# NOAA-OWP/T-Route

Hardware: AMD Instinct MI355X
Metric: segment-timesteps/sec, CONUS NHD 2.7M-seg MC (higher is better)
Workload: dtype f32

## Files before the change

include/trmc.h:

```cpp
#ifndef TRMC_H
#define TRMC_H

#include <stddef.h>
#include <stdint.h>

#ifdef __cplusplus
extern "C" {
#endif

#define TRMC_ABI_VERSION 19

typedef enum trmc_status {
    TRMC_OK = 0,
    TRMC_EINVAL = -1,
    TRMC_ECYCLE = -2,
    TRMC_ENODEVICE = -3,
    TRMC_EHIP = -4,
    TRMC_ENOMEM = -5,
    TRMC_ESTATE = -6,
    TRMC_EUNSUPPORTED = -7
} trmc_status;

enum { TRMC_P_DT = 0, TRMC_P_DX, TRMC_P_BW, TRMC_P_TW, TRMC_P_TWCC, TRMC_P_N,
       TRMC_P_NCC, TRMC_P_CS, TRMC_P_S0, TRMC_NPARAM };

typedef struct trmc_plan trmc_plan;

typedef struct trmc_stats {
    int64_t nseg;
    int64_t nseg_routed;
    int32_t nlevels;
    int32_t nsteps;
    int32_t assume_short_ts;
    int32_t main_launches;
    int64_t segment_steps;
    double ms_prep;
    double ms_main;
    double ms_emit;
    double ms_total;
    int32_t wide_levels, wide_k;
    int32_t wide_launches;
    int32_t mid_levels;
    int64_t wide_segment_steps;
    double ms_wide;
    int32_t mid_k, mid_launches;
    int32_t arithmetic;
    int32_t reserved0;
} trmc_stats;

const char *trmc_last_error(void);
int trmc_abi_version(void);
int trmc_device_count(int *count);

int trmc_plan_create(int64_t nseg, const int64_t *up_ptr, const int64_t *up_idx,
                     const float *params, const uint8_t *boundary, int precision,
                     int device, trmc_plan **out);
int trmc_plan_create_hinted(int64_t nseg, const int64_t *up_ptr, const int64_t *up_idx,
                            const float *params, const uint8_t *boundary, const uint8_t *cost_hint,
                            int precision, int device, trmc_plan **out);
enum { TRMC_ENGINE_AUTO = 0, TRMC_ENGINE_LEVELS = 1, TRMC_ENGINE_FLOW = 2, TRMC_ENGINE_MASK = 3,
       TRMC_PLAN_SHORT_TS = 4, TRMC_PLAN_FULL_TS = 8 };
int trmc_plan_create_ex(int64_t nseg, const int64_t *up_ptr, const int64_t *up_idx,
                        const float *params, const uint8_t *boundary, const uint8_t *cost_hint,
                        int precision, int device, int flags, trmc_plan **out);
enum { TRMC_ARITH_EXACT = 0, TRMC_ARITH_TOLERANCE = 1 };
typedef struct trmc_plan_options {
    int32_t struct_size;
    int32_t arithmetic;
    int64_t wide_min_rows;
    int32_t wide_levels, wide_k;
    int64_t mid_min_rows;
    int32_t mid_levels, mid_k;
    int32_t tile_perm_group;
    int32_t tail_sort;
    int32_t stem_min_rows;
    int32_t sequence_mode;
    int32_t flow_watchdog_ms;
    int32_t flow_overlap;
    int32_t flow_lean;
    int32_t flow_debug;
    int32_t hot_rows;
    int32_t cluster_rows;
    int32_t cluster_late_lag;
    int32_t stream_split;
    int32_t hot_wave_rows;
    int32_t velocity_on_demand;
    int32_t reserved[2];
} trmc_plan_options;
int trmc_plan_create_opt(int64_t nseg, const int64_t *up_ptr, const int64_t *up_idx,
                         const float *params, const uint8_t *boundary, const uint8_t *cost_hint,
                         int precision, int device, int flags, const trmc_plan_options *options, trmc_plan **out);
int trmc_stream_begin(trmc_plan *plan, int nsteps, int qts_subdivisions, int slots, int full_output, int output_stride);
int trmc_stream_push(trmc_plan *plan, const void *qlat, int64_t nq, const void *boundary_q_dev, int32_t rowset, void *hyd_host,
                     void *q0_host, void *fvd_host);
typedef struct trmc_stream_day {
    const void *qlat;
    int64_t nq;
    const void *boundary_q_dev;
    int32_t rowset;
    int32_t reserved0;
    void *hyd_host, *q0_host, *fvd_host;
    int64_t da_ngage;
    int32_t da_nsteps, res_nsteps;
    const uint8_t *da_mode;
    const void *da_a, *da_w;
    void *nudge_host;
    int64_t res_nres;
    void *res_inflow_host;
    const void *da_q0;
    const struct trmc_stream_reservoir_da *reservoir_da;
    void *res_da_state_host, *res_da_tsidx_host;
} trmc_stream_day;
int trmc_stream_set_gages(trmc_plan *plan, int64_t ngage, const int64_t *gage_rows);
int trmc_stream_push_day(trmc_plan *plan, const trmc_stream_day *day);
int trmc_stream_set_packed_forcing(trmc_plan *plan, int64_t nfeat, const int64_t *feat_of_row, const double *pack_a, const double *pack_b);
int trmc_stream_push_day_packed(trmc_plan *plan, const trmc_stream_day *day, const int32_t *raw_a, const int32_t *raw_b);
int trmc_stream_packed_forcing_kernel_ms(trmc_plan *plan, double *ms_out);
enum { TRMC_SUMMARY_PEAK = 1, TRMC_SUMMARY_MEAN = 2, TRMC_SUMMARY_PEAK_DEPTH = 4, TRMC_SUMMARY_TOTAL = 8 };
int trmc_stream_set_summary(trmc_plan *plan, int what);
int trmc_stream_summary_dest(trmc_plan *plan, void *peak_flow_host, int32_t *peak_step_host, void *mean_flow_host);
int trmc_stream_summary_depth_dest(trmc_plan *plan, void *peak_depth_host, int32_t *peak_depth_step_host);
int trmc_stream_summary_total(trmc_plan *plan, void *peak_flow, int64_t *peak_step, void *mean_flow, void *peak_depth,
                              int64_t *peak_depth_step, int64_t *days_out);
int trmc_stream_gather(trmc_plan *plan, int64_t day, int32_t rowset, void *dst_dev, void *stream);
int trmc_stream_boundary(trmc_plan *plan, int64_t day, const void *q_dev, int64_t src_row_stride, const int64_t *index_dev, void *stream);
int trmc_stream_advance(trmc_plan *plan, int ntiles);
int trmc_stream_flush(trmc_plan *plan);
int trmc_stream_wait(trmc_plan *plan, int64_t day);
int trmc_stream_info(const trmc_plan *plan, int32_t *slots, int32_t *tiles_per_day, int32_t *lag_max, int32_t *wide_levels,
                     int32_t *cluster_levels, int64_t *days_pushed, int64_t *days_complete, int64_t *launches);
int trmc_stream_day_ms(trmc_plan *plan, int64_t day, double *ms_out);
int trmc_stream_end(trmc_plan *plan);

int trmc_plan_set_sequence_mode(trmc_plan *plan, int on);
int trmc_plan_arithmetic(const trmc_plan *plan, int32_t *arithmetic);
int trmc_plan_engine(const trmc_plan *plan, int32_t *is_flow);
void trmc_plan_destroy(trmc_plan *plan);

int trmc_topology_levels(int64_t nseg, const int64_t *up_ptr, const int64_t *up_idx,
                         const uint8_t *boundary, int32_t *level_of_row,
                         int64_t *plan_pos_of_row, int32_t *nlevels);

int trmc_topology_levels_hinted(int64_t nseg, const int64_t *up_ptr, const int64_t *up_idx,
                                const uint8_t *boundary, const uint8_t *cost_hint, int32_t *level_of_row,
                                int64_t *plan_pos_of_row, int32_t *nlevels);

int trmc_topology_clusters(int64_t nseg, const int64_t *up_ptr, const int64_t *up_idx, const uint8_t *boundary,
                           const uint8_t *cost_hint, int64_t wide_min_rows, int32_t wide_max_levels, int32_t cluster_rows,
                           int64_t *plan_pos_of_row, int32_t *lag_of_row, int32_t *block_of_row, int32_t *wide_levels,
                           int32_t *cluster_levels, int32_t *cluster_blocks);

int trmc_topology_blocks(int64_t nseg, const int64_t *up_ptr, const int64_t *up_idx,
                         const uint8_t *boundary, const uint8_t *cost_hint, int cost_tiers,
                         int64_t *plan_pos_of_row, int32_t *rank_of_row, int32_t *block_rows, int32_t *nblocks);

int trmc_topology_blocks_general(int64_t nseg, const int64_t *up_ptr, const int64_t *up_idx, const uint8_t *boundary,
                                 int32_t stem_min_rows, int64_t *plan_pos_of_row, int32_t *rank_of_row, int32_t *block_rows,
                                 int32_t *nblocks, int32_t *early_blocks, int32_t early_cap, int32_t *nearly);

int trmc_plan_info(const trmc_plan *plan, int64_t *nseg, int64_t *nseg_routed,
                   int32_t *nlevels, int32_t *precision, int32_t *device);
int trmc_plan_lags(const trmc_plan *plan, int32_t *lag_of_row, int32_t *wide_levels, int32_t *cluster_levels);
int trmc_plan_cluster_blocks(const trmc_plan *plan, int32_t *block_of_row, int32_t *block_width, int32_t *cluster_blocks);
int trmc_plan_levels(const trmc_plan *plan, int32_t *level_of_row, int64_t *plan_pos_of_row);

int trmc_upload_forcing(trmc_plan *plan, int nsteps, const void *qlat, int64_t nq,
                        const void *q0, const void *boundary_fvd);

int trmc_upload_forcing_packed(trmc_plan *plan, int nsteps, int64_t nq, int64_t nfeat, const int32_t *raw_a,
                               const int32_t *raw_b, const double *pack_a, const double *pack_b,
                               const int64_t *feat_of_row, const void *q0, const void *boundary_fvd);

int trmc_set_boundary_flow_device(trmc_plan *plan, int nsteps, const void *q_dev);

int trmc_set_reservoirs(trmc_plan *plan, int64_t nres, const int64_t *res_rows, const void *par,
                        double routing_period);
int trmc_download_reservoir_inflow(trmc_plan *plan, void *inflow_out);

typedef struct trmc_reservoir_da_table {
    int64_t n, ncol;
    const float *obs, *time, *state;
    const int32_t *ipar;
} trmc_reservoir_da_table;
int trmc_set_reservoir_da(trmc_plan *plan, int64_t nres, const int32_t *kind, const int32_t *table_row,
                          const trmc_reservoir_da_table *usgs, const trmc_reservoir_da_table *usace,
                          const trmc_reservoir_da_table *rfc);
int trmc_download_reservoir_da(trmc_plan *plan, float *state_out, int32_t *timeseries_idx_out);
typedef struct trmc_stream_reservoir_da {
    trmc_reservoir_da_table usgs, usace, rfc;
    int32_t rfc_reset_idx;
    int32_t reserved0;
} trmc_stream_reservoir_da;
int trmc_stream_set_reservoir_da(trmc_plan *plan, int on, int64_t usgs_ncol, int64_t usace_ncol, int64_t rfc_ncol);
#define TRMC_RESERVOIR_DA_HYBRID 2
#define TRMC_RESERVOIR_DA_RFC 4
int trmc_reservoir_da_steps(int device, int kind, int64_t n, int64_t ncol, const float *obs, const float *time,
                            const float *fin, const int32_t *iin, float *fout, int32_t *iout);

int trmc_set_nudging(trmc_plan *plan, int nsteps, int64_t ngage, const int64_t *gage_rows,
                     const uint8_t *mode, const void *a, const void *w);
int trmc_set_nudging_successors(trmc_plan *plan, int64_t ngage, const int64_t *successor_rows);
int trmc_download_nudge(trmc_plan *plan, void *nudge_out);

int trmc_route_device(trmc_plan *plan, int nsteps, int qts_subdivisions, int assume_short_ts);

int trmc_route_begin(trmc_plan *plan, int nsteps, int qts_subdivisions, int assume_short_ts);
int trmc_route_advance(trmc_plan *plan, int t_end);
int trmc_route_end(trmc_plan *plan);
int trmc_plan_stream(trmc_plan *plan, void **stream_out);
int trmc_rowset_create(trmc_plan *plan, const int64_t *rows, int64_t nrows, int32_t *id_out);
int trmc_gather_flow_range(trmc_plan *plan, int32_t rowset, int t_begin, int t_end, void *dst_dev,
                           int64_t dst_stride);
int trmc_set_boundary_flow_range(trmc_plan *plan, int t_begin, int t_end, const void *q_dev, int64_t src_stride,
                                 void *stream );
int trmc_set_boundary_flow_range_indexed(trmc_plan *plan, int t_begin, int t_end, const void *q_dev,
// ... 115 lines not shown
```

t-route_amd/_lib.py:

```python
import ctypes as C
import os

import numpy as np

_HERE = os.path.dirname(os.path.abspath(__file__))
LIB_PATH = os.environ.get("TRMC_LIB_PATH") or os.path.join(_HERE, "libtrmc.so")

TRMC_OK, TRMC_EINVAL, TRMC_ECYCLE, TRMC_ENODEVICE, TRMC_EHIP, TRMC_ENOMEM, TRMC_ESTATE = 0, -1, -2, -3, -4, -5, -6
TRMC_EUNSUPPORTED = -7
ENGINE_AUTO, ENGINE_LEVELS, ENGINE_FLOW, PLAN_SHORT_TS, PLAN_FULL_TS = 0, 1, 2, 4, 8
NPARAM = 9
PARAM_COLS = ("dt", "dx", "bw", "tw", "twcc", "n", "ncc", "cs", "s0")


class Stats(C.Structure):
    _fields_ = [
        ("nseg", C.c_int64), ("nseg_routed", C.c_int64), ("nlevels", C.c_int32), ("nsteps", C.c_int32),
        ("assume_short_ts", C.c_int32), ("main_launches", C.c_int32), ("segment_steps", C.c_int64),
        ("ms_prep", C.c_double), ("ms_main", C.c_double), ("ms_emit", C.c_double), ("ms_total", C.c_double),
        ("wide_levels", C.c_int32), ("wide_k", C.c_int32), ("wide_launches", C.c_int32), ("mid_levels", C.c_int32),
        ("wide_segment_steps", C.c_int64), ("ms_wide", C.c_double), ("mid_k", C.c_int32), ("mid_launches", C.c_int32),
        ("arithmetic", C.c_int32), ("reserved0", C.c_int32),
    ]

    def as_dict(self):
        return {k: getattr(self, k) for k, _ in self._fields_}


class PlanOptions(C.Structure):
    _fields_ = [
        ("struct_size", C.c_int32), ("arithmetic", C.c_int32), ("wide_min_rows", C.c_int64), ("wide_levels", C.c_int32),
        ("wide_k", C.c_int32), ("mid_min_rows", C.c_int64), ("mid_levels", C.c_int32), ("mid_k", C.c_int32),
        ("tile_perm_group", C.c_int32), ("tail_sort", C.c_int32), ("stem_min_rows", C.c_int32), ("sequence_mode", C.c_int32),
        ("flow_watchdog_ms", C.c_int32), ("flow_overlap", C.c_int32), ("flow_lean", C.c_int32), ("flow_debug", C.c_int32), ("hot_rows", C.c_int32),
        ("cluster_rows", C.c_int32), ("cluster_late_lag", C.c_int32), ("stream_split", C.c_int32), ("hot_wave_rows", C.c_int32), ("velocity_on_demand", C.c_int32), ("reserved", C.c_int32 * 2),
    ]


ARITH_EXACT, ARITH_TOLERANCE = 0, 1
OPTION_ENV = {
    "TRMC_WIDE_MIN_ROWS": ("wide_min_rows", "off0"), "TRMC_WIDE_LEVELS": ("wide_levels", "int"), "TRMC_WIDE_K": ("wide_k", "int"),
    "TRMC_MID_MIN_ROWS": ("mid_min_rows", "off0"), "TRMC_MID_LEVELS": ("mid_levels", "int"), "TRMC_MID_K": ("mid_k", "int"),
    "TRMC_TILE_PERM": ("tile_perm_group", "off0"), "TRMC_HOT_ROWS": ("hot_rows", "off0"), "TRMC_CLUSTER_ROWS": ("cluster_rows", "int"), "TRMC_STREAM_SPLIT": ("stream_split", "int"), "TRMC_HOT_WAVE_ROWS": ("hot_wave_rows", "int"), "TRMC_VELOCITY_ON_DEMAND": ("velocity_on_demand", "int"), "TRMC_TAIL_SORT": ("tail_sort", "off0"),
    "TRMC_STEM_MIN_ROWS": ("stem_min_rows", "off0"), "TRMC_SETUP_ASIDE": ("sequence_mode", "flag"),
    "TRMC_FLOW_WATCHDOG_MS": ("flow_watchdog_ms", "int"), "TRMC_FLOW_OVERLAP": ("flow_overlap", "flag"),
    "TRMC_FLOW_LEAN": ("flow_lean", "lean"), "TRMC_FLOW_DEBUG": ("flow_debug", "flag"),
}


def plan_options(options=None):
    o = PlanOptions()
    o.struct_size = C.sizeof(PlanOptions)
    for name, (field, how) in OPTION_ENV.items():
        v = os.environ.get(name)
        if v is None or v == "":
            continue
        n = int(v)
        if how == "off0":
            n = -1 if n == 0 else n
        elif how == "flag":
            n = 1 if n == 1 else 0
        elif how == "lean":
            n = 1 if n == 1 else -1
        setattr(o, field, n)
    a = os.environ.get("TRMC_ARITHMETIC")
    if a:
        o.arithmetic = {"exact": ARITH_EXACT, "tolerance": ARITH_TOLERANCE}[a]
    for k, v in (options or {}).items():
        if k == "arithmetic" and isinstance(v, str):
            v = {"exact": ARITH_EXACT, "tolerance": ARITH_TOLERANCE}[v]
        if not hasattr(o, k) or k in ("struct_size", "reserved"):
            raise ValueError(f"unknown plan option {k!r}")
        setattr(o, k, int(v))
    return o


_vp, _i64, _i32, _int = C.c_void_p, C.c_int64, C.c_int32, C.c_int


class ReservoirDaTable(C.Structure):
    _fields_ = [("n", C.c_int64), ("ncol", C.c_int64), ("obs", C.c_void_p), ("time", C.c_void_p), ("state", C.c_void_p),
                ("ipar", C.c_void_p)]


class StreamReservoirDa(C.Structure):
    _fields_ = [("usgs", ReservoirDaTable), ("usace", ReservoirDaTable), ("rfc", ReservoirDaTable), ("rfc_reset_idx", C.c_int32),
                ("reserved0", C.c_int32)]


RESERVOIR_DA_HYBRID, RESERVOIR_DA_RFC = 2, 4
SUMMARY_PEAK, SUMMARY_MEAN = 1, 2
SUMMARY_PEAK_DEPTH, SUMMARY_TOTAL = 4, 8
SUMMARY_NAMES = {"peak": SUMMARY_PEAK, "mean": SUMMARY_MEAN, "peak_depth": SUMMARY_PEAK_DEPTH, "total": SUMMARY_TOTAL}
TRMC_X_FLOW, TRMC_X_VELOCITY, TRMC_X_DEPTH = 0, 1, 2
X_NAMES = {"flow": TRMC_X_FLOW, "velocity": TRMC_X_VELOCITY, "depth": TRMC_X_DEPTH}
_P = C.POINTER
SIGNATURES = {
    "trmc_last_error": (C.c_char_p, []),
    "trmc_abi_version": (_int, []),
    "trmc_device_count": (_int, [_P(_int)]),
    "trmc_plan_create": (_int, [_i64, _vp, _vp, _vp, _vp, _int, _int, _P(_vp)]),
    "trmc_plan_create_hinted": (_int, [_i64, _vp, _vp, _vp, _vp, _vp, _int, _int, _P(_vp)]),
    "trmc_plan_create_ex": (_int, [_i64, _vp, _vp, _vp, _vp, _vp, _int, _int, _int, _P(_vp)]),
    "trmc_plan_create_opt": (_int, [_i64, _vp, _vp, _vp, _vp, _vp, _int, _int, _int, _P(PlanOptions), _P(_vp)]),
    "trmc_plan_set_sequence_mode": (_int, [_vp, _int]),
    "trmc_stream_begin": (_int, [_vp, _int, _int, _int, _int, _int]),
    "trmc_stream_push": (_int, [_vp, _vp, _i64, _vp, _i32, _vp, _vp, _vp]),
    "trmc_stream_set_gages": (_int, [_vp, _i64, _vp]),
    "trmc_stream_push_day": (_int, [_vp, _vp]),
    "trmc_stream_set_reservoir_da": (_int, [_vp, _int, _i64, _i64, _i64]),
    "trmc_stream_set_summary": (_int, [_vp, _int]),
    "trmc_stream_summary_dest": (_int, [_vp, _vp, _vp, _vp]),
    "trmc_stream_summary_depth_dest": (_int, [_vp, _vp, _vp]),
    "trmc_stream_summary_total": (_int, [_vp, _vp, _vp, _vp, _vp, _vp, _vp]),
    "trmc_stream_gather": (_int, [_vp, _i64, _i32, _vp, _vp]),
    "trmc_stream_boundary": (_int, [_vp, _i64, _vp, _i64, _vp, _vp]),
    "trmc_stream_advance": (_int, [_vp, _int]),
    "trmc_stream_flush": (_int, [_vp]),
    "trmc_stream_wait": (_int, [_vp, _i64]),
    "trmc_stream_info": (_int, [_vp, _P(_i32), _P(_i32), _P(_i32), _P(_i32), _P(_i32), _P(_i64), _P(_i64), _P(_i64)]),
    "trmc_stream_day_ms": (_int, [_vp, _i64, _P(C.c_double)]),
    "trmc_stream_end": (_int, [_vp]),
    "trmc_plan_arithmetic": (_int, [_vp, _P(_i32)]),
    "trmc_plan_engine": (_int, [_vp, _P(_i32)]),
    "trmc_plan_destroy": (None, [_vp]),
    "trmc_topology_levels": (_int, [_i64, _vp, _vp, _vp, _vp, _vp, _P(_i32)]),
    "trmc_topology_levels_hinted": (_int, [_i64, _vp, _vp, _vp, _vp, _vp, _vp, _P(_i32)]),
    "trmc_topology_clusters": (_int, [_i64, _vp, _vp, _vp, _vp, _i64, _i32, _i32, _vp, _vp, _vp, _P(_i32), _P(_i32), _P(_i32)]),
    "trmc_topology_blocks": (_int, [_i64, _vp, _vp, _vp, _vp, _int, _vp, _vp, _P(_i32), _P(_i32)]),
    "trmc_topology_blocks_general": (_int, [_i64, _vp, _vp, _vp, _i32, _vp, _vp, _P(_i32), _P(_i32), _vp, _i32, _P(_i32)]),
    "trmc_plan_info": (_int, [_vp, _P(_i64), _P(_i64), _P(_i32), _P(_i32), _P(_i32)]),
    "trmc_plan_levels": (_int, [_vp, _vp, _vp]),
    "trmc_plan_lags": (_int, [_vp, _vp, _P(_i32), _P(_i32)]),
    "trmc_plan_cluster_blocks": (_int, [_vp, _vp, _P(_i32), _P(_i32)]),
    "trmc_upload_forcing": (_int, [_vp, _int, _vp, _i64, _vp, _vp]),
    "trmc_upload_forcing_packed": (_int, [_vp, _int, _i64, _i64, _vp, _vp, _vp, _vp, _vp, _vp, _vp]),
    "trmc_set_boundary_flow_device": (_int, [_vp, _int, _vp]),
    "trmc_set_reservoirs": (_int, [_vp, _i64, _vp, _vp, C.c_double]),
    "trmc_download_reservoir_inflow": (_int, [_vp, _vp]),
    "trmc_set_reservoir_da": (_int, [_vp, _i64, _vp, _vp, _P(ReservoirDaTable), _P(ReservoirDaTable), _P(ReservoirDaTable)]),
    "trmc_download_reservoir_da": (_int, [_vp, _vp, _vp]),
    "trmc_reservoir_da_steps": (_int, [_int, _int, _i64, _i64, _vp, _vp, _vp, _vp, _vp, _vp]),
    "trmc_set_nudging": (_int, [_vp, _int, _i64, _vp, _vp, _vp, _vp]),
    "trmc_set_nudging_successors": (_int, [_vp, C.c_int64, _vp]),
    "trmc_download_nudge": (_int, [_vp, _vp]),
    "trmc_route_device": (_int, [_vp, _int, _int, _int]),
    "trmc_route_begin": (_int, [_vp, _int, _int, _int]),
    "trmc_route_advance": (_int, [_vp, _int]),
    "trmc_route_end": (_int, [_vp]),
    "trmc_plan_stream": (_int, [_vp, _P(_vp)]),
    "trmc_rowset_create": (_int, [_vp, _vp, _i64, _P(_i32)]),
    "trmc_gather_flow_range": (_int, [_vp, _i32, _int, _int, _vp, _i64]),
    "trmc_set_boundary_flow_range": (_int, [_vp, _int, _int, _vp, _i64, _vp]),
    "trmc_set_boundary_flow_range_indexed": (_int, [_vp, _int, _int, _vp, _i64, _vp, _vp]),
    "trmc_plan_set_lag": (_int, [_vp, _vp]),
    "trmc_download_fvd": (_int, [_vp, _vp]),
    "trmc_download_fvd_strided": (_int, [_vp, _int, _vp]),
    "trmc_download_fvd_rowset": (_int, [_vp, _int, C.c_int32, _vp]),
    "trmc_window_summary": (_int, [_vp, _i32, _vp, _vp, _vp, _vp, _vp, _vp, _vp]),
    "trmc_window_summary_tile": (_int, [_int, _P(_i32), _P(_i32)]),
    "trmc_window_summary_kernel_ms": (_int, [_vp, _P(C.c_double)]),
    "trmc_window_courant": (_int, [_vp, _i32, _int, _vp]),
    "trmc_window_courant_summary": (_int, [_vp, _i32, C.c_double, _vp, _vp, _vp]),
    "trmc_window_courant_tile": (_int, [_int, _P(_i32), _P(_i32)]),
    "trmc_window_courant_kernel_ms": (_int, [_vp, _P(C.c_double)]),
    "trmc_plan_set_thresholds": (_int, [_vp, _i32, _vp]),
    "trmc_window_exceedance": (_int, [_vp, _i32, _int, _vp, _vp, _vp, _vp]),
    "trmc_window_exceedance_tile": (_int, [_int, _P(_i32), _P(_i32)]),
    "trmc_window_exceedance_kernel_ms": (_int, [_vp, _P(C.c_double)]),
    "trmc_plan_bankfull_depth": (_int, [_vp, _vp]),
    "trmc_stream_set_exceedance": (_int, [_vp, _int]),
    "trmc_stream_exceedance": (_int, [_vp, _vp, _vp, _vp, _vp, _P(_i64)]),
    "trmc_stream_set_courant": (_int, [_vp, _int, C.c_double]),
    "trmc_stream_courant": (_int, [_vp, _vp, _vp, _vp, _P(_i64)]),
    "trmc_stream_courant_kernel_ms": (_int, [_vp, _P(C.c_double)]),
    "trmc_stream_set_depth_exceedance": (_int, [_vp, _i32, _vp]),
    "trmc_stream_depth_exceedance": (_int, [_vp, _vp, _vp, _vp, _vp, _P(_i64)]),
    "trmc_stream_depth_exceedance_kernel_ms": (_int, [_vp, _P(C.c_double)]),
    "trmc_stream_set_stage": (_int, [_vp, _int]),
    "trmc_stream_stage_dest": (_int, [_vp, _vp]),
    "trmc_stream_set_packed_forcing": (_int, [_vp, _i64, _vp, _vp, _vp]),
    "trmc_stream_push_day_packed": (_int, [_vp, _vp, _vp, _vp]),
    "trmc_stream_packed_forcing_kernel_ms": (_int, [_vp, _P(C.c_double)]),
    "trmc_plan_set_nan_is_zero": (_int, [_vp, _int]),
    "trmc_host_alloc": (_int, [C.c_size_t, C.POINTER(C.c_void_p)]),
    "trmc_host_free": (_int, [_vp]),
    "trmc_download_final_state": (_int, [_vp, _vp]),
    "trmc_download_iterations": (_int, [_vp, _vp]),
    "trmc_plan_collect_cost": (_int, [_vp, _int]),
    "trmc_download_cost": (_int, [_vp, _vp, _P(_i32)]),
    "trmc_gather_flow_rows": (_int, [_vp, _vp, _i64, _vp, _int]),
    "trmc_download_gathered": (_int, [_vp, _vp]),
    "trmc_plan_set_stamps": (_int, [_vp, _vp, _i32]),
    "trmc_plan_set_output_stride": (_int, [_vp, _i32]),
    "trmc_plan_hot_rows": (_int, [_vp, _P(_i64)]),
    "trmc_plan_hot_state": (_int, [_vp, _P(_i32), _P(_i32), _P(_i32), _P(_i32), _P(_i32), _P(_i32)]),
    "trmc_fetch_begin": (_int, [_vp, _i32, _vp, _vp]),
    "trmc_fetch_begin_fvd": (_int, [_vp, _i32, _vp, _vp, _int, _vp]),
    "trmc_fetch_wait": (_int, [_vp]),
    "trmc_get_stats": (_int, [_vp, _P(Stats)]),
    "trmc_route": (_int, [_vp, _int, _int, _int, _vp, _i64, _vp, _vp, _vp]),
    "trmc_segments": (_int, [_int, _int, _i64, _vp, _vp]),
    "trmc_segments_ex": (_int, [_int, _int, _int, _i64, _vp, _vp, _vp]),
    "trmc_muskingcungenwm": (None, [_P(C.c_float)] * 21),
    "trmc_plan_chain_from": (_int, [_vp, _vp]),
# ... 244 lines not shown
```

t-route_amd/csrc/abi.inc:

```

static bool stream_active(const trmc_plan *pl);

const char *trmc_last_error(void) { return g_err.c_str(); }
int trmc_abi_version(void) { return TRMC_ABI_VERSION; }

int trmc_device_count(int *count)
{
    if (!count) return fail(TRMC_EINVAL, "count is NULL");
    int c = 0;
    hipError_t e = hipGetDeviceCount(&c);
    if (e != hipSuccess) {
        *count = 0;
        return fail(TRMC_ENODEVICE, std::string("hipGetDeviceCount: ") + hipGetErrorString(e));
    }
    *count = c;
    return 0;
}

int trmc_topology_levels(int64_t nseg, const int64_t *up_ptr, const int64_t *up_idx, const uint8_t *boundary,
                         int32_t *level_of_row, int64_t *plan_pos_of_row, int32_t *nlevels)
{
    return trmc_topology_levels_hinted(nseg, up_ptr, up_idx, boundary, nullptr, level_of_row, plan_pos_of_row, nlevels);
}

// ... 168 lines not shown

int trmc_plan_create_ex(int64_t nseg, const int64_t *up_ptr, const int64_t *up_idx, const float *params,
                        const uint8_t *boundary, const uint8_t *cost_hint, int precision, int device, int flags,
                        trmc_plan **out)
{
    return trmc_plan_create_opt(nseg, up_ptr, up_idx, params, boundary, cost_hint, precision, device, flags, nullptr, out);
}

static int plan_streams(trmc_plan *pl)
{
    HIP_TRY(hipSetDevice(pl->device));
    int prio_lo = 0, prio_hi = 0;
    HIP_TRY(hipDeviceGetStreamPriorityRange(&prio_lo, &prio_hi));
    if (int rc = pl->stream.ensure(hipStreamNonBlocking, prio_hi)) return rc;
    if (int rc = pl->stream2.ensure(hipStreamNonBlocking, prio_lo)) return rc;
    if (int rc = pl->ev_emit.ensure(false)) return rc;
    if (pl->flow) {
        if (int rc = pl->fstream.ensure(hipStreamNonBlocking, prio_hi)) return rc;
        for (DevEvent &e : pl->ev_chunk)
            if (int rc = e.ensure(false)) return rc;
        if (int rc = pl->ev_ctl.ensure(false)) return rc;
    }
    for (DevEvent &e : pl->ev)
        if (int rc = e.ensure(true)) return rc;
    return 0;
}

int trmc_plan_create_opt(int64_t nseg, const int64_t *up_ptr, const int64_t *up_idx, const float *params,
                         const uint8_t *boundary, const uint8_t *cost_hint, int precision, int device, int flags,
                         const trmc_plan_options *options, trmc_plan **out)
{
    if (!out) return fail(TRMC_EINVAL, "out is NULL");
    trmc_plan_options o{};
    if (options) {
        if (options->struct_size < 8 || options->struct_size > (int32_t)sizeof(trmc_plan_options))
            return fail(TRMC_EINVAL, "trmc_plan_options.struct_size is not the size of a trmc_plan_options this library knows");
        std::memcpy(&o, options, (size_t)options->struct_size);
    }
    if (o.arithmetic != TRMC_ARITH_EXACT && o.arithmetic != TRMC_ARITH_TOLERANCE) return fail(TRMC_EINVAL, "bad trmc_plan_options.arithmetic");
    if (o.arithmetic == TRMC_ARITH_TOLERANCE && precision != 32)
        return fail(TRMC_EINVAL, "TRMC_ARITH_TOLERANCE is an arithmetic of precision-32 plans");
    *out = nullptr;
    if (precision != 32 && precision != 64) return fail(TRMC_EINVAL, "precision must be 32 or 64");
    if (nseg > 0 && !params) return fail(TRMC_EINVAL, "params is NULL");
    if ((flags & ~(TRMC_ENGINE_MASK | TRMC_PLAN_SHORT_TS | TRMC_PLAN_FULL_TS)) || (flags & TRMC_ENGINE_MASK) == 3
        || ((flags & TRMC_PLAN_SHORT_TS) && (flags & TRMC_PLAN_FULL_TS)))
        return fail(TRMC_EINVAL, "bad plan flags");
    int engine = flags & TRMC_ENGINE_MASK;
    if (engine == TRMC_ENGINE_FLOW && precision != 32) return fail(TRMC_EINVAL, "the dataflow engine runs precision-32 plans only");
    if (int rc = check_device(device)) return rc;

    trmc_plan *pl = new (std::nothrow) trmc_plan();
    if (!pl) return fail(TRMC_ENOMEM, "out of host memory");
    pl->sh = std::make_shared<PlanShared>();
    if (engine == TRMC_ENGINE_AUTO) {
        if (precision != 32)
            engine = TRMC_ENGINE_LEVELS;
        else {
            int64_t nb = 0;
            for (int64_t r = 0; boundary && r < nseg; ++r) nb += boundary[r] == 1;
            engine = ((flags & TRMC_PLAN_SHORT_TS) && nseg - nb >= 1000000) ? TRMC_ENGINE_LEVELS : TRMC_ENGINE_FLOW;
        }
    }
    pl->flow = engine == TRMC_ENGINE_FLOW;
    pl->watchdog_ticks = (uint64_t)(o.flow_watchdog_ms > 0 ? o.flow_watchdog_ms : 30000) * 100000ull;
    {
        int ncu = 256;
        if (hipSetDevice(device) == hipSuccess) (void)hipDeviceGetAttribute(&ncu, hipDeviceAttributeMultiprocessorCount, device);
        trmc_plan::Opt &po = pl->opt;
        po.tol = o.arithmetic == TRMC_ARITH_TOLERANCE;
        po.wide_min_rows = o.wide_min_rows < 0 ? 0 : (o.wide_min_rows > 0 ? o.wide_min_rows : (po.tol ? 256L : 288L) * ncu);
        po.wide_levels = (int32_t)std::min<long>(o.wide_levels > 0 ? o.wide_levels : 16, kWideMaxLevels);
        po.wide_k = o.wide_k > 0 ? o.wide_k : 0;
        po.mid_min_rows = o.mid_min_rows < 0 ? 0 : (o.mid_min_rows > 0 ? o.mid_min_rows : kMidDefaultRowsPerCu * (int64_t)ncu);
        po.mid_levels = (int32_t)std::min<long>(o.mid_levels > 0 ? o.mid_levels : 12, kMidMaxLevels);
        po.mid_k = o.mid_k > 0 ? o.mid_k : 4;
        po.tile_perm_group = o.tile_perm_group < 0 ? 0 : (o.tile_perm_group > 0 ? 1 : -1);
        po.hot_rows = o.hot_rows < 0 ? 0 : (o.hot_rows > 0 ? 1 : -1);
        po.cluster_rows = o.cluster_rows > 0 ? std::min<int32_t>(o.cluster_rows, kClusterRowsMax) : 0;
        po.cluster_late_lag = std::max(0, o.cluster_late_lag);
        po.stream_split = std::max(0, o.stream_split);
        po.hot_wave_rows = std::max(0, std::min(64, o.hot_wave_rows));
        po.velocity_on_demand = o.velocity_on_demand;
        po.sequence = o.sequence_mode != 0;
        po.flow_overlap = o.flow_overlap != 0;
        po.flow_lean = o.flow_lean;
        po.flow_debug = o.flow_debug != 0;
    }
    const bool tiers = (flags & TRMC_PLAN_SHORT_TS) != 0;
    std::string err;
    int64_t wide_min_rows = 0, mid_min_rows = 0;
    int32_t wide_max_levels = 0, mid_max_levels = 0;
    if (tiers && !pl->flow && cost_hint && o.tail_sort >= 0) {
        wide_min_rows = pl->opt.wide_min_rows;
        wide_max_levels = pl->opt.wide_levels;
        mid_min_rows = pl->opt.mid_min_rows;
        mid_max_levels = pl->opt.mid_levels;
    }
    int32_t cluster_rows = 0;
    if (tiers && !pl->flow && pl->opt.cluster_rows > 0) {
        cluster_rows = pl->opt.cluster_rows;
        wide_min_rows = pl->opt.wide_min_rows;
        wide_max_levels = pl->opt.wide_levels;
        mid_min_rows = 0;
        mid_max_levels = 0;
        pl->opt.mid_min_rows = 0;
    }
    int32_t stem_min_rows = 0;
    if (pl->flow && (flags & TRMC_PLAN_FULL_TS)) stem_min_rows = o.stem_min_rows < 0 ? 0 : (o.stem_min_rows > 0 ? o.stem_min_rows : 1024);
    const int trc = trmc::build_topology(nseg, up_ptr, up_idx, boundary, pl->sh->topo, err, cost_hint, pl->flow ? kFlowBlock : 0, tiers,
                                         (tiers && !pl->flow) ? kWideMaxLevels : 0, wide_min_rows, wide_max_levels, stem_min_rows,
                                         mid_min_rows, mid_max_levels, cluster_rows, pl->opt.cluster_late_lag, kCtileBlock);
    if (trc) {
        delete pl;
        return fail(trc == -2 ? TRMC_ECYCLE : TRMC_EINVAL, err);
    }
    pl->device = device;
    pl->hinted = cost_hint != nullptr && (!pl->flow || tiers);
    pl->precision = precision;
    pl->esz = precision == 32 ? 4 : 8;
    pl->nseg = nseg;
    pl->nseg_pad = (nseg + 63) / 64 * 64;
    if (pl->nseg_pad == 0) pl->nseg_pad = 64;
    pl->nrouted = nseg - pl->sh->topo.nboundary;
    pl->dt_uniform = true;
    pl->dt = nseg ? params[TRMC_P_DT] : 0.0;
    for (int64_t r = 1; r < nseg; ++r)
        if (params[(size_t)r * TRMC_NPARAM + TRMC_P_DT] != params[TRMC_P_DT]) {
            pl->dt_uniform = false;
            break;
        }

    auto bail = [&](int rc) {
        trmc_plan_destroy(pl);
        return rc;
    };
    int rc = plan_streams(pl);
    if (rc) return bail(rc);
    rc = by_precision(pl, [&](auto t) { return upload_params<decltype(t)>(pl, params); });
    if (rc) return bail(rc);
    std::vector<int32_t> level_plan((size_t)pl->nseg_pad, 0);
    for (int64_t p = 0; p < nseg; ++p) level_plan[p] = pl->sh->topo.level_of_row[pl->sh->topo.row_of_pos[p]];
    if ((rc = upload_i32(pl->sh->level, level_plan, 1))) return bail(rc);
    if (pl->sh->topo.ncl > 0) {
        std::vector<int32_t> lagk(pl->sh->topo.lagk_of_pos);
        lagk.resize((size_t)pl->nseg_pad, 0);
        if ((rc = upload_i32(pl->sh->lagk, lagk, 1))) return bail(rc);
        if ((rc = upload_i32(pl->sh->cblk_ptr, pl->sh->topo.cblk_ptr, 1))) return bail(rc);
    }
    if ((rc = upload_i32(pl->sh->up_ptr, pl->sh->topo.up_ptr, 1))) return bail(rc);
    if ((rc = upload_i32(pl->sh->up_idx, pl->sh->topo.up_idx, 1))) return bail(rc);
    {
        if (nseg >= (int64_t)1 << 30) return bail(fail(TRMC_EINVAL, "more than 2**30 segments in one plan"));
        if ((uint64_t)pl->nseg_pad * pl->esz >= (1ull << 32))
            return bail(fail(TRMC_EINVAL, "too many segments for one plan at this precision (column size reaches 4 GiB)"));
        std::vector<int32_t> up2((size_t)pl->nseg_pad * 2, -1);
        for (int64_t p = 0; p < nseg; ++p) {
            const int32_t k0 = pl->sh->topo.up_ptr[p], k1 = pl->sh->topo.up_ptr[p + 1];
            if (k1 - k0 >= 1) up2[2 * p] = pl->sh->topo.up_idx[k0];
            if (k1 - k0 >= 2) up2[2 * p + 1] = pl->sh->topo.up_idx[k0 + 1] | (k1 - k0 > 2 ? 0x40000000 : 0);
        }
        if ((rc = upload_i32(pl->sh->up2, up2, 2))) return bail(rc);
    }
    if (pl->flow && (rc = upload_i32(pl->sh->rank, pl->sh->topo.rank_of_pos, 1))) return bail(rc);
    if (pl->flow) {
        if ((rc = pl->sh->prio.ensure(pl->sh->topo.prio_of_wave.size() + 1))) return bail(rc);
// ... 27 lines not shown
    *out = pl;
    return 0;
}

void trmc_plan_destroy(trmc_plan *pl)
{
    if (!pl) return;
    (void)hipSetDevice(pl->device);
    delete pl;
}

static int final_state_into(trmc_plan *pl, void *dst, int32_t nsteps_of_window = -1);
static int ensure_copy_stream(trmc_plan *pl);

int trmc_plan_clone(trmc_plan *src, trmc_plan **out)
{
    if (!out) return fail(TRMC_EINVAL, "out is NULL");
    *out = nullptr;
    if (!src) return fail(TRMC_EINVAL, "plan is NULL");
    if (int rc = use_device(src)) return rc;
    trmc_plan *pl = new (std::nothrow) trmc_plan();
    if (!pl) return fail(TRMC_ENOMEM, "out of host memory");
    pl->device = src->device;
    pl->precision = src->precision;
    pl->esz = src->esz;
    pl->nseg = src->nseg;
    pl->nseg_pad = src->nseg_pad;
    pl->nrouted = src->nrouted;
    pl->dt_uniform = src->dt_uniform;
    pl->dt = src->dt;
    pl->hinted = src->hinted;
    pl->params_sane = src->params_sane;
    pl->flow = src->flow;
    pl->watchdog_ticks = src->watchdog_ticks;
    pl->opt = src->opt;
    pl->ncuq = src->ncuq;
    pl->sh = src->sh;
    pl->is_clone = true;
    auto bail = [&](int rc) {
        trmc_plan_destroy(pl);
        return rc;
    };
    if (int rc = plan_streams(pl)) return bail(rc);
    if (src->maxlag > 0) {
        pl->lag_of_row = src->lag_of_row;
        pl->maxlag = src->maxlag;
    }
    if (int rc = pl->it_prev.ensure((size_t)pl->nseg_pad)) return bail(rc);
    if (pl->ncuq > 0)
        if (int rc = pl->cuq_head.ensure((size_t)pl->ncuq * 2 * sizeof(int32_t))) return bail(rc);
    *out = pl;
    return 0;
}

int trmc_stage_forcing(trmc_plan *pl, int nsteps, const void *qlat, int64_t nq)
{
    if (!pl) return fail(TRMC_EINVAL, "plan is NULL");
    const bool busy = pl->run.active;
    if (busy && pl->run.t_done < pl->run.nsteps + (pl->run.short_ts ? pl->maxlag : 0))
        return fail(TRMC_ESTATE, "the window in progress has not been queued to its end (trmc_route_advance)");
    if (busy && (pl->ngage > 0 || pl->nres > 0))
        return fail(TRMC_ESTATE, "a window with nudging tables or reservoirs is in progress: its series are read after trmc_route_end; "
                                 "stage the next forcing then");
    if (nsteps < 1) return fail(TRMC_EINVAL, "nsteps must be >= 1");
    if (nq < 1) return fail(TRMC_EINVAL, "qlat needs at least one column");
    if (pl->nseg > 0 && !qlat) return fail(TRMC_EINVAL, "qlat is NULL");
    if (int rc = use_device(pl)) return rc;
    if (int rc = ensure_copy_stream(pl)) return rc;
    const size_t bytes = (size_t)pl->nseg * nq * pl->esz;
    if (busy && bytes > pl->in_qlat.bytes)
        return fail(TRMC_ESTATE, "the staging area would have to grow while the window in progress may still read it");
    if (int rc = pl->in_qlat.ensure(bytes)) return rc;
    if (int rc = pl->in_q0.ensure((size_t)pl->nseg * 3 * pl->esz)) return rc;
    pl->state_missing = busy || (pl->routed_nsteps < 0 && !pl->q0_staged);
    if (pl->nseg > 0 && !pl->state_missing && pl->routed_nsteps >= 0)
        if (int rc = final_state_into(pl, pl->in_q0.p)) return rc;
    pl->q0_staged = !pl->state_missing;
    if (busy) HIP_TRY(hipStreamWaitEvent(pl->hstream, pl->ev[1], 0));
    if (pl->nseg > 0) HIP_TRY(hipMemcpyAsync(pl->in_qlat.p, qlat, bytes, hipMemcpyHostToDevice, pl->hstream));
    pl->qlat_alt_ready = false;
    if (pl->opt.sequence && !pl->flow && pl->nseg > 0) {
        if (int rc = pl->qlat_alt.ensure((size_t)nq * pl->nseg_pad * pl->esz)) return rc;
        const int32_t n = (int32_t)pl->nseg;
        const dim3 grid((n + 63) / 64, (unsigned)((nq + 31) / 32));
        const int rc = by_precision(pl, [&](auto t) {
            using T = decltype(t);
            hipLaunchKernelGGL((k_prep_qlat<T>), grid, dim3(kBlock), 0, pl->hstream, (const T *)pl->in_qlat.p,
                               (const int32_t *)pl->sh->row_of_pos.p, (T *)pl->qlat_alt.p, n, pl->nseg_pad, (int32_t)nq);
            return launched();
        });
        if (rc) return rc;
        pl->qlat_alt_ready = true;
    }
    if (int rc = pl->mk_forcing.record(pl->hstream)) return rc;
    pl->qlat_direct = false;
    pl->nq = nq;
    pl->have_boundary = pl->sh->topo.nboundary == 0;
    pl->ngage = 0;
    pl->nraw = 0;
    pl->staged_nsteps = nsteps;
    if (!busy) pl->routed_nsteps = -1;
    return 0;
}

int trmc_plan_info(const trmc_plan *pl, int64_t *nseg, int64_t *nseg_routed, int32_t *nlevels, int32_t *precision,
                   int32_t *device)
{
    if (!pl) return fail(TRMC_EINVAL, "plan is NULL");
    if (nseg) *nseg = pl->nseg;
    if (nseg_routed) *nseg_routed = pl->nrouted;
    if (nlevels) *nlevels = pl->sh->topo.nlevels;
    if (precision) *precision = pl->precision;
    if (device) *device = pl->device;
    return 0;
}

int trmc_plan_lags(const trmc_plan *pl, int32_t *lag_of_row, int32_t *wide_levels, int32_t *cluster_levels)
{
    if (!pl) return fail(TRMC_EINVAL, "plan is NULL");
    const trmc::Topology &t = pl->sh->topo;
    if (t.cl_rows <= 0) return fail(TRMC_EINVAL, "the plan is not in cluster order (trmc_plan_options.cluster_rows)");
    for (int64_t r = 0; lag_of_row && r < pl->nseg; ++r)
        lag_of_row[r] = t.level_of_row[r] < 0 ? -1 : t.lagk_of_pos[(size_t)t.pos_of_row[r]];
    if (wide_levels) *wide_levels = t.cl_from_level;
    if (cluster_levels) *cluster_levels = t.ncl;
    return 0;
}

int trmc_plan_cluster_blocks(const trmc_plan *pl, int32_t *block_of_row, int32_t *block_width, int32_t *cluster_blocks)
{
    if (!pl) return fail(TRMC_EINVAL, "plan is NULL");
    const trmc::Topology &t = pl->sh->topo;
    if (t.cl_rows <= 0) return fail(TRMC_EINVAL, "the plan is not in cluster order (trmc_plan_options.cluster_rows)");
    const int32_t nb = t.ncl > 0 ? (int32_t)t.cblk_ptr.size() - 1 : 0;
    if (block_of_row) {
        for (int64_t r = 0; r < pl->nseg; ++r) block_of_row[r] = -1;
        for (int32_t b = 0; b < nb; ++b)
            for (int32_t p = t.cblk_ptr[(size_t)b]; p < t.cblk_ptr[(size_t)b + 1]; ++p) block_of_row[t.row_of_pos[(size_t)p]] = b;
    }
    if (block_width) *block_width = kCtileBlock;
    if (cluster_blocks) *cluster_blocks = nb;
    return 0;
}

int trmc_plan_levels(const trmc_plan *pl, int32_t *level_of_row, int64_t *plan_pos_of_row)
{
    if (!pl) return fail(TRMC_EINVAL, "plan is NULL");
    for (int64_t r = 0; r < pl->nseg; ++r) {
        if (level_of_row) level_of_row[r] = pl->sh->topo.level_of_row[r];
        if (plan_pos_of_row) plan_pos_of_row[r] = pl->sh->topo.pos_of_row[r];
    }
    return 0;
}

static int final_state_into(trmc_plan *pl, void *dst, int32_t nsteps_of_window)
{
    const int32_t n = (int32_t)pl->nseg, T_ = nsteps_of_window >= 0 ? nsteps_of_window : pl->routed_nsteps;
    const size_t plane = (size_t)(T_ + 1) * pl->nseg_pad;
    const int32_t *rop = (const int32_t *)pl->sh->row_of_pos.p;
    int rc;
    if (pl->flow) {
        hipLaunchKernelGGL((k_final_state<float>), dim3(blocks_for(n)), dim3(kBlock), 0, pl->stream, (const float *)pl->tm.p,
                           (const float *)pl->d_state.p, rop, (float *)dst, n, pl->nseg_pad, T_, 2, 0);
        rc = launched();
    } else {
        rc = by_precision(pl, [&](auto t) {
            using T = decltype(t);
            const T *q = (const T *)pl->tm.p;
            hipLaunchKernelGGL((k_final_state<T>), dim3(blocks_for(n)), dim3(kBlock), 0, pl->stream, q, q + 2 * plane, rop, (T *)dst, n,
                               pl->nseg_pad, T_, 1, T_);
            return launched();
// ... 1297 lines not shown
```

t-route_amd/csrc/host_flow.inc:

```
int flow_place_blocks(trmc_plan *pl)
{
    pl->ncuq = 0;
    const int32_t nb = pl->sh->topo.nblocks;
    if (nb <= 0) return 0;
    constexpr int kKeys = 4096;
    DevBuf seen;
    if (int rc = seen.ensure(kKeys)) return rc;
    HIP_TRY(hipMemset(seen.p, 0, kKeys));
    int ncu = 256;
    (void)hipDeviceGetAttribute(&ncu, hipDeviceAttributeMultiprocessorCount, pl->device);
    hipLaunchKernelGGL(k_cu_probe, dim3((unsigned)(64 * ncu)), dim3(64), 0, nullptr, (uint8_t *)seen.p);
    std::vector<uint8_t> hs(kKeys);
    hipError_t e = hipMemcpy(hs.data(), seen.p, kKeys, hipMemcpyDeviceToHost);
    seen.release();
    if (e != hipSuccess) return fail(TRMC_EHIP, std::string("compute-unit probe: ") + hipGetErrorString(e));
    std::vector<int32_t> cu_index(kKeys, -1);
    int32_t Q = 0;
    for (int k = 0; k < kKeys; ++k)
        if (hs[k]) cu_index[k] = Q++;
    if (Q < 2) return 0;
    const std::vector<uint8_t> &wc = pl->sh->topo.cost_of_wave;
    int hi = 0;
    for (const uint8_t c : wc) hi = std::max(hi, (int)c);
    const bool sixteenths = hi > 7;
// ... 83 lines not shown
    a.gran = (unsigned long long *)pl->tm.p;
    a.d_state = (float *)pl->d_state.p;
    a.d_gran = (unsigned long long *)pl->d_gran.p;
    a.out = (float *)pl->out.p;
    a.row_of_pos = (const int32_t *)pl->sh->row_of_pos.p;
    a.it_prev = (uint8_t *)pl->it_prev.p;
    a.it_sum = pl->collect_cost ? (uint16_t *)pl->it_sum.p : nullptr;
    a.sane = pl->params_sane;
    a.out_vec = nsteps % 4 == 0;
    a.res_of_pos = pl->nres > 0 ? (const int32_t *)pl->res_of_pos.p : nullptr;
    a.res_par = (const float *)pl->res_par.p;
    a.res_inflow = (float *)pl->res_inflow.p;
    a.res_dt = (float)pl->res_dt;
    a.res_da = (pl->nres > 0 && pl->res_da_on) ? pl->res_da.p : nullptr;
    const bool da = pl->ngage > 0;
    a.gage_of_pos = da ? (const int32_t *)pl->gage_of_pos.p : nullptr;
    a.da_mode = (const uint8_t *)pl->da_mode.p;
    a.da_a = (const float *)pl->da_a.p;
    a.da_w = (const float *)pl->da_w.p;
    a.da_nudge = (float *)pl->da_nudge.p;
    a.nseg_pad = pl->nseg_pad;
    a.nsteps = nsteps;
    a.qts = qts;
    a.nseg = (int32_t)pl->nseg;
    a.first = (int32_t)pl->sh->topo.nboundary;
    a.tag_base = pl->tag_base;
    a.ticket = (int32_t *)pl->ticket.p;
    a.watchdog_ticks = pl->watchdog_ticks;
    a.dbg = pl->opt.flow_debug ? (unsigned long long *)pl->dbg.p : nullptr;
    a.nblocks_dbg = pl->sh->topo.nblocks;
    a.prio = (const uint8_t *)pl->sh->prio.p;
    a.cuq_ptr = a.cuq_blk = a.cu_index = nullptr;
    a.cuq_perm = nullptr;
    a.cuq_head = nullptr;
    a.ncuq = 0;
    return a;
}

int flow_route_begin(trmc_plan *pl, int nsteps, int qts, int short_ts)
{
    const trmc::Topology &tp = pl->sh->topo;
    const int32_t n = (int32_t)pl->nseg;
    const int64_t np = pl->nseg_pad;
    hipStream_t st = pl->stream;
    if (int rc = pl->tm.ensure((size_t)(nsteps + 1) * np * sizeof(unsigned long long), true)) return rc;
    if (int rc = pl->d_state.ensure((size_t)np * sizeof(float))) return rc;
    if (int rc = pl->d_gran.ensure((size_t)np * sizeof(unsigned long long), true)) return rc;
    if (int rc = pl->ticket.ensure(16 * sizeof(int32_t))) return rc;
    if (pl->opt.flow_debug) {
        if (int rc = pl->dbg.ensure((size_t)(tp.nblocks + 1) * 6 * sizeof(unsigned long long))) return rc;
        HIP_TRY(hipMemsetAsync(pl->dbg.p, 0, pl->dbg.bytes, st));
    }
    if (int rc = pl->qlat_tm.ensure((size_t)pl->nq * np * sizeof(float))) return rc;
    if (int rc = pl->out.ensure((size_t)pl->nseg * nsteps * 3 * sizeof(float))) return rc;
    if (pl->nres > 0)
        if (int rc = pl->res_inflow.ensure((size_t)pl->nres * nsteps * sizeof(float))) return rc;
    if (pl->collect_cost) {
        if (int rc = pl->it_sum.ensure((size_t)np * sizeof(uint16_t))) return rc;
        pl->cost_nsteps = nsteps;
    }
    if ((uint64_t)pl->tag_base + (uint64_t)pl->tag_span + (uint64_t)nsteps + 2 >= 0xffffffffull) {
        HIP_TRY(hipMemsetAsync(pl->tm.p, 0, pl->tm.bytes, st));
        HIP_TRY(hipMemsetAsync(pl->d_gran.p, 0, pl->d_gran.bytes, st));
        pl->tag_base = 1;
        pl->tag_span = 0;
    }
    pl->tag_base += (uint32_t)pl->tag_span;
    pl->tag_span = nsteps + 1;
    const int32_t *row_of_pos = (const int32_t *)pl->sh->row_of_pos.p;
    HIP_TRY(hipEventRecord(pl->ev[0], st));
    pl->q0_staged = false;
    if (int rc = pl->mk_dec.order(st)) return rc;
    if (pl->fstream)
        if (int rc = pl->mk_dec.order(pl->fstream)) return rc;
    pl->mk_dec.settle();
    if (int rc = pl->mk_forcing.order(st)) return rc;
    pl->mk_forcing.settle();
    HIP_TRY(hipMemsetAsync(pl->it_prev.p, 0, (size_t)np, st));
    HIP_TRY(hipMemsetAsync(pl->ticket.p, 0, 16 * sizeof(int32_t), st));
    pl->flow_next = pl->flow_last = 0;
    if (pl->collect_cost) HIP_TRY(hipMemsetAsync(pl->it_sum.p, 0, (size_t)np * sizeof(uint16_t), st));
    if (n > 0) {
        if (!pl->qlat_direct)
            hipLaunchKernelGGL((k_prep_qlat<float>), dim3((n + 63) / 64, (unsigned)((pl->nq + 31) / 32)), dim3(kBlock), 0, st,
                               (const float *)pl->in_qlat.p, row_of_pos, (float *)pl->qlat_tm.p, n, np, (int32_t)pl->nq);
        hipLaunchKernelGGL(k_flow_init, dim3(blocks_for(n)), dim3(kBlock), 0, st, (const float *)pl->in_q0.p, row_of_pos,
                           (unsigned long long *)pl->tm.p, (float *)pl->d_state.p, (unsigned long long *)pl->d_gran.p, n,
                           pl->tag_base);
    }
    RouteRun &r = pl->run;
    r = RouteRun{};
    r.active = true;
    r.nsteps = nsteps;
    r.qts = qts;
    r.short_ts = short_ts ? 1 : 0;
    r.boundary_through = tp.nboundary > 0 ? 0 : nsteps;
    if (tp.nboundary > 0 && pl->have_boundary) {
        hipLaunchKernelGGL(k_flow_boundary, dim3(blocks_for(tp.nboundary * (int64_t)nsteps)), dim3(kBlock), 0, st,
                           (const float *)pl->in_bfvd.p, (unsigned long long *)pl->tm.p, (float *)pl->out.p, row_of_pos,
                           (int32_t)tp.nboundary, nsteps, np, 0, nsteps, (int64_t)nsteps * 3, 3, 3, pl->tag_base, (const int64_t *)nullptr);
        r.boundary_through = nsteps;
    }
    HIP_TRY(hipEventRecord(pl->ev[1], st));
    HIP_TRY(hipStreamWaitEvent(pl->fstream, pl->ev[1], 0));
    HIP_TRY(hipGetLastError());
    pl->routed_nsteps = -1;
    return 0;
}

static bool flow_lean(const trmc_plan *pl, int nsteps)
{
    int ncu = 256;
    (void)hipDeviceGetAttribute(&ncu, hipDeviceAttributeMultiprocessorCount, pl->device);
    const int32_t force = pl->opt.flow_lean;
    return (uint64_t)pl->nseg * (uint64_t)nsteps * 3ull < (1ull << 32)
           && (force ? force > 0 : pl->sh->topo.nblocks <= TRMC_LEAN_WAVES * (256 / kFlowBlock) * ncu);
}
static bool flow_overlap(const trmc_plan *pl)
{
    return pl->opt.flow_overlap && pl->run.short_ts && flow_lean(pl, pl->run.nsteps);
}
static hipStream_t flow_stream(const trmc_plan *pl, int which) { return which ? pl->fstream : pl->stream; }

int flow_route_advance(trmc_plan *pl, int t_end)
{
    RouteRun &r = pl->run;
    if (pl->nrouted > 0 && t_end > r.t_done) {
        const bool lean = r.short_ts && flow_lean(pl, r.nsteps);
        const int which = flow_overlap(pl) ? pl->flow_next : 0;
        hipStream_t st = flow_stream(pl, which);
        FlowArgs a = flow_args(pl, r.nsteps, r.qts, r.short_ts != 0);
        a.ticket += 8 * which;
        HIP_TRY(hipMemsetAsync(a.ticket, 0, sizeof(int32_t), st));
        if (lean && pl->ncuq > 0) {
            a.cuq_ptr = (const int32_t *)pl->sh->cuq_ptr.p;
            a.cuq_blk = (const int32_t *)pl->sh->cuq_blk.p;
            a.cu_index = (const int32_t *)pl->sh->cu_index.p;
            a.cuq_perm = (const uint8_t *)pl->sh->cuq_perm.p;
            a.cuq_head = (int32_t *)pl->cuq_head.p + (size_t)pl->ncuq * which;
            a.ncuq = pl->ncuq;
            HIP_TRY(hipMemsetAsync(a.cuq_head, 0, (size_t)pl->ncuq * sizeof(int32_t), st));
        }
        const dim3 grid((unsigned)pl->sh->topo.nblocks), block(kFlowBlock);
        if (a.res_da) {
            if (lean && a.lag) hipLaunchKernelGGL((k_mc_flow_lean_rda<true>), grid, block, 0, st, a, r.t_done, t_end);
            else if (lean) hipLaunchKernelGGL((k_mc_flow_lean_rda<false>), grid, block, 0, st, a, r.t_done, t_end);
            else if (r.short_ts) hipLaunchKernelGGL((k_mc_flow_rda<true>), grid, block, 0, st, a, r.t_done, t_end);
            else hipLaunchKernelGGL((k_mc_flow_rda<false>), grid, block, 0, st, a, r.t_done, t_end);
        } else if (pl->opt.tol) {
            if (lean && a.lag)
                hipLaunchKernelGGL((k_mc_flow_lean<true, true>), grid, block, 0, st, a, r.t_done, t_end);
            else if (lean)
                hipLaunchKernelGGL((k_mc_flow_lean<false, true>), grid, block, 0, st, a, r.t_done, t_end);
            else if (r.short_ts)
                hipLaunchKernelGGL((k_mc_flow<true, true>), grid, block, 0, st, a, r.t_done, t_end);
            else
                hipLaunchKernelGGL((k_mc_flow<false, true>), grid, block, 0, st, a, r.t_done, t_end);
        } else if (lean && a.lag)
            hipLaunchKernelGGL((k_mc_flow_lean<true>), grid, block, 0, st, a, r.t_done, t_end);
        else if (lean)
            hipLaunchKernelGGL((k_mc_flow_lean<false>), grid, block, 0, st, a, r.t_done, t_end);
        else if (r.short_ts)
            hipLaunchKernelGGL((k_mc_flow<true>), grid, block, 0, st, a, r.t_done, t_end);
        else
            hipLaunchKernelGGL((k_mc_flow<false>), grid, block, 0, st, a, r.t_done, t_end);
        HIP_TRY(hipEventRecord(pl->ev_chunk[which], st));
        pl->flow_last = which;
        if (flow_overlap(pl)) pl->flow_next = 1 - which;
// ... 107 lines not shown
```

t-route_amd/csrc/host_levels.inc:

```

int quot_selfcheck(int device, bool *ok);

template <class T> T *col(trmc_plan *pl, int c) { return (T *)pl->sh->params.p + (size_t)c * pl->nseg_pad; }

template <class T> int upload_params(trmc_plan *pl, const float *params)
{
    const int64_t n = pl->nseg, np = pl->nseg_pad;
    std::vector<T> host((size_t)TRMC_NPARAM * np, T(0));
    const size_t all_cols = (size_t)kTotalCols * np;
    bool sane = true;
    auto in_range = [](float v) { return v >= 0x1p-14f && v <= 0x1p17f; };
    auto within = [](float v, float lo, float hi) { return v >= lo && v <= hi; };
    for (int64_t p = 0; p < n; ++p) {
        const float *src = params + (size_t)pl->sh->topo.row_of_pos[p] * TRMC_NPARAM;
        for (int c = 0; c < TRMC_NPARAM; ++c) host[(size_t)c * np + p] = (T)src[c];
        const float cs = src[TRMC_P_CS];
        sane = sane && in_range(src[TRMC_P_BW]) && in_range(src[TRMC_P_N]) && (cs == 0.0f || in_range(cs))
               && (src[TRMC_P_TWCC] == 0.0f || in_range(src[TRMC_P_TWCC])) && (src[TRMC_P_NCC] == 0.0f || in_range(src[TRMC_P_NCC]))
               && within(src[TRMC_P_DT], 0x1p-20f, 0x1p40f) && within(src[TRMC_P_DX], 0x1p-10f, 0x1p19f)
               && within(src[TRMC_P_S0], 0x1p-30f, 0x1p10f);
    }
    bool quot_ok = false;
    if (int rc = quot_selfcheck(pl->device, &quot_ok)) return rc;
    pl->params_sane = sane && quot_ok && sizeof(T) == 4;
// ... 261 lines not shown
        if constexpr (rda()) hipLaunchKernelGGL((k_mc_ctile_rda<dec()>), grid, block, 0, st, a, cblk_ptr, b0, tile, K);
        else if (dpl && tile_carries(a)) {
            if (pk_d) hipLaunchKernelGGL((k_mc_ctile_dpl<T, tl(), dec(), true>), grid, block, 0, st, a, cblk_ptr, b0, tile, K, pk_d, pk_at);
            else hipLaunchKernelGGL((k_mc_ctile_dpl<T, tl(), dec(), false>), grid, block, 0, st, a, cblk_ptr, b0, tile, K, pk_d, pk_at);
        } else if (pk_d && tile_carries(a)) hipLaunchKernelGGL((k_mc_ctile_pkd<T, tl(), dec()>), grid, block, 0, st, a, cblk_ptr, b0, tile, K, pk_d, pk_at);
        else hipLaunchKernelGGL((k_mc_ctile<T, tl(), dec(), lazy()>), grid, block, 0, st, a, cblk_ptr, b0, tile, K);
    });
}

template <class T> int emit_tiles_through(trmc_plan *pl, int32_t t_complete)
{
    constexpr int32_t kTile = TRMC_EMIT_TILE;
    RouteRun &r = pl->run;
    const int32_t n = (int32_t)pl->nseg, nsteps = r.nsteps;
    const int32_t ntiles = (nsteps + kTile - 1) / kTile;
    const size_t plane = (size_t)(nsteps + 1) * pl->nseg_pad;
    const T *q_tm = (const T *)pl->tm.p;
    while (r.tiles_done < ntiles && ((r.tiles_done + 1) * kTile <= t_complete || t_complete >= nsteps)) {
        HIP_TRY(hipEventRecord(pl->tile_ev[r.tiles_done], (r.wide > 0 && !r.tail_active) ? pl->wstream : pl->stream));
        HIP_TRY(hipStreamWaitEvent(pl->stream2, pl->tile_ev[r.tiles_done], 0));
        const int32_t skip_lo = (r.wide > 0 || r.cl) ? pl->sh->topo.lvl_ptr[0] : 0;
        const int32_t skip_hi = r.cl ? pl->sh->topo.lvl_ptr[pl->sh->topo.nlevels] : (r.wide > 0 ? pl->sh->topo.lvl_ptr[r.wide + r.mid] : 0);
        const int32_t shift_from = (skip_lo + 63) / 64 * 64, shift = std::max(0, (skip_hi - shift_from) / 64 * 64);
        const int32_t n_emit = n - shift;
        if (n_emit > 0) {
            const int32_t tb = r.tiles_done * kTile, te = min(nsteps, tb + kTile);
            hipLaunchKernelGGL((k_emit<T>), dim3((n_emit + 63) / 64, (unsigned)((te - tb + kEmitSteps - 1) / kEmitSteps)),
                               dim3(kBlock), 0, pl->stream2, q_tm, q_tm + plane, q_tm + 2 * plane,
                               (const int32_t *)pl->sh->row_of_pos.p, (T *)pl->out.p, n, pl->nseg_pad, nsteps, tb, te, shift_from, shift,
                               skip_lo, skip_hi);
        }
        ++r.tiles_done;
    }
    return 0;
}

template <class T> int route_begin_t(trmc_plan *pl, int nsteps, int qts, int short_ts)
{
    const trmc::Topology &tp = pl->sh->topo;
    const int32_t n = (int32_t)pl->nseg;
    const int64_t np = pl->nseg_pad;
    hipStream_t st = pl->stream;
    const size_t plane = (size_t)(nsteps + 1) * np;
    if (int rc = pl->tm.ensure(3 * plane * sizeof(T))) return rc;
    const bool qlat_early = pl->qlat_alt_ready;
    if (qlat_early) std::swap(pl->qlat_tm, pl->qlat_alt);
    pl->qlat_alt_ready = false;
    if (int rc = pl->qlat_tm.ensure((size_t)pl->nq * np * sizeof(T))) return rc;
    if (int rc = pl->out.ensure((size_t)pl->nseg * nsteps * 3 * sizeof(T))) return rc;
    if (pl->nres > 0)
        if (int rc = pl->res_inflow.ensure((size_t)pl->nres * nsteps * sizeof(T))) return rc;
    if (pl->collect_cost) {
        if (int rc = pl->it_sum.ensure((size_t)np * sizeof(uint16_t))) return rc;
        pl->cost_nsteps = nsteps;
    }
    StepArgs<T> a = step_args<T>(pl, nsteps, qts);
    const int32_t *row_of_pos = (const int32_t *)pl->sh->row_of_pos.p;
    constexpr int32_t kTile = TRMC_EMIT_TILE;
    const int32_t ntiles = (nsteps + kTile - 1) / kTile;
    if (int rc = ensure_events(pl->tile_ev, (size_t)std::max(0, ntiles), false)) return rc;

    for (DevMark &m : pl->mk_released) {
        if (int rc = m.order(st)) return rc;
        if (pl->wstream)
            if (int rc = m.order(pl->wstream)) return rc;
        m.settle();
    }
    HIP_TRY(hipEventRecord(pl->ev[0], st));
    const bool setup_aside = pl->opt.sequence && short_ts && pl->wstream != nullptr;
    hipStream_t const plan_st = st;
    if (setup_aside) {
        st = pl->wstream;
        if (int rc = pl->mk_gather.order(st)) return rc;
    }
    pl->mk_gather.settle();
    if (int rc = pl->mk_dec.order(st)) return rc;
    pl->mk_dec.settle();
    if (int rc = pl->mk_forcing.order(st)) return rc;
    pl->mk_forcing.settle();
    HIP_TRY(hipMemsetAsync(pl->it_prev.p, 0, (size_t)np, st));
    if (pl->collect_cost) HIP_TRY(hipMemsetAsync(pl->it_sum.p, 0, (size_t)np * sizeof(uint16_t), st));
    if (n > 0) {
        if (!pl->qlat_direct && !qlat_early)
            hipLaunchKernelGGL((k_prep_qlat<T>), dim3((n + 63) / 64, (unsigned)((pl->nq + 31) / 32)), dim3(kBlock), 0, st,
                               (const T *)pl->in_qlat.p, row_of_pos, (T *)pl->qlat_tm.p, n, np, (int32_t)pl->nq);
        if (!pl->chain_staged)
            hipLaunchKernelGGL((k_init_state<T>), dim3(blocks_for(n)), dim3(kBlock), 0, st, (const T *)pl->in_q0.p,
                               row_of_pos, a.q_tm, a.v_tm, a.d_tm, n);
    }
    pl->chain_staged = false;
    pl->q0_staged = false;
    pl->row0_replaced = false;
    RouteRun &r = pl->run;
    r = RouteRun{};
    r.active = true;
    r.nsteps = nsteps;
    r.qts = qts;
    r.short_ts = short_ts ? 1 : 0;
    if (pl->stamps) ++pl->stamp_seq;
    r.boundary_through = tp.nboundary > 0 ? 0 : nsteps;
    if (tp.nboundary > 0 && pl->have_boundary) {
        hipLaunchKernelGGL((k_fill_boundary<T>), dim3(blocks_for(tp.nboundary * (int64_t)nsteps)), dim3(kBlock), 0, st,
                           (const T *)pl->in_bfvd.p, a.q_tm, a.v_tm, a.d_tm, (int32_t)tp.nboundary, nsteps, np);
        r.boundary_through = nsteps;
    }
    HIP_TRY(hipEventRecord(pl->ev[1], st));
    if (setup_aside) {
        st = plan_st;
        HIP_TRY(hipStreamWaitEvent(st, pl->ev[1], 0));
    }
    if (pl->wide_safe_pos < 0) {
        int64_t first = pl->nseg;
        for (int64_t p = tp.nboundary; p < pl->nseg && first == pl->nseg; ++p) {
            bool unsafe = pl->maxlag > 0 && !pl->lag_of_row.empty() && pl->lag_of_row[(size_t)tp.row_of_pos[p]] != 0;
            for (int32_t k = tp.up_ptr[p]; !unsafe && k < tp.up_ptr[p + 1]; ++k) unsafe = tp.up_idx[k] < tp.nboundary;
            if (unsafe) first = p;
        }
        pl->wide_safe_pos = first;
    }
    if (short_ts && pl->nrouted > 0) {
        const int64_t min_rows = pl->opt.wide_min_rows;
        int32_t W = 0, M = 0;
        const bool all_in_place = pl->maxlag == 0 && r.boundary_through == nsteps;
        const int32_t level_cap = tp.ncl > 0 ? tp.cl_from_level : (tp.tail_from_level > 0 ? tp.tail_from_level : tp.nlevels);
        auto level_ok = [&](int32_t l, int64_t need) {
            return l < level_cap && tp.lvl_ptr[l + 1] - tp.lvl_ptr[l] >= need && (all_in_place || (int64_t)tp.lvl_ptr[l + 1] <= pl->wide_safe_pos);
        };
        if (min_rows > 0)
            while (W < std::min<int32_t>(pl->opt.wide_levels, kWideMaxLevels) && level_ok(W, min_rows)) ++W;
        if (W > 0 && pl->opt.mid_min_rows > 0)
            while (M < pl->opt.mid_levels && level_ok(W + M, pl->opt.mid_min_rows)) ++M;
        if (tp.ncl > 0 && all_in_place) {
            r.cl = true;
            W = tp.cl_from_level;
            M = 0;
        }
        if (W > 0 || r.cl) {
            r.wide = W;
            r.wide_k = std::max(1, std::min(nsteps, pl->opt.wide_k > 0 ? pl->opt.wide_k : std::max(1, std::min(16, nsteps / 8))));
            r.mid = M;
            r.mid_k = M > 0 ? std::max(1, std::min(r.wide_k, pl->opt.mid_k)) : 0;
            r.cl_next = W;
            if (int rc = ensure_tile_stream(pl)) return rc;
            HIP_TRY(hipStreamWaitEvent(pl->wstream, pl->ev[1], 0));
            const size_t ntile = (size_t)std::max(1, (nsteps + r.wide_k - 1) / r.wide_k + W - 1);
            if (int rc = ensure_events(pl->wide_t0, ntile, true)) return rc;
            if (int rc = ensure_events(pl->wide_t1, ntile, true)) return rc;
        }
    }
    HIP_TRY(hipGetLastError());
    pl->routed_nsteps = -1;
    return 0;
}

template <class T> int route_end_queue(trmc_plan *pl)
{
    RouteRun &r = pl->run;
    if (r.end_queued) return 0;
    hipStream_t st = pl->stream;
    stamp(pl, st, 3);
    HIP_TRY(hipEventRecord(pl->ev[2], st));
    if (int rc = emit_tiles_through<T>(pl, r.nsteps)) return rc;
    HIP_TRY(hipEventRecord(pl->ev_emit, pl->stream2));
    HIP_TRY(hipStreamWaitEvent(st, pl->ev_emit, 0));
    HIP_TRY(hipEventRecord(pl->ev[3], st));
    HIP_TRY(hipGetLastError());
    r.end_queued = true;
    return 0;
// ... 209 lines not shown
```

t-route_amd/csrc/k_mc_ctile.inc:

```
#ifndef TRMC_CTILE_BLOCK
#define TRMC_CTILE_BLOCK 512
#endif
constexpr int kCtileBlock = TRMC_CTILE_BLOCK;
constexpr int kClusterRowsMax = 128;
static_assert(kCtileBlock % 64 == 0 && kCtileBlock >= kClusterRowsMax && kCtileBlock <= 1024,
              "TRMC_CTILE_BLOCK: whole wavefronts, at least one cluster, at most one workgroup");
constexpr int kCtileStage = kCtileBlock > 512 ? kTileStage / 2 : kTileStage;
template <class T, bool TOL, bool DEC, bool LAZYV, bool RDA, bool PKD = false, bool DPL = false>
__device__ __forceinline__ void mc_ctile_rows(const StepArgs<T> &a, const int32_t *__restrict__ cblk_ptr, int32_t cb0, int32_t tile, int32_t K,
                                              T *pk_d = nullptr, int32_t *pk_at = nullptr);
template <class T, bool TOL = false, bool DEC = false, bool LAZYV = false>
__global__ void __launch_bounds__(kCtileBlock, sizeof(T) == 4 ? (LAZYV ? TRMC_TILE_WAVES_LAZY : TRMC_TILE_WAVES) : 1)
k_mc_ctile(const StepArgs<T> a, const int32_t *__restrict__ cblk_ptr, const int32_t cb0, const int32_t tile, const int32_t K)
{
    mc_ctile_rows<T, TOL, DEC, LAZYV, false>(a, cblk_ptr, cb0, tile, K);
}
template <bool DEC>
__global__ void __launch_bounds__(kCtileBlock, TRMC_TILE_WAVES)
k_mc_ctile_rda(const StepArgs<float> a, const int32_t *__restrict__ cblk_ptr, const int32_t cb0, const int32_t tile, const int32_t K)
{
    mc_ctile_rows<float, false, DEC, false, true>(a, cblk_ptr, cb0, tile, K);
}
template <class T, bool TOL = false, bool DEC = false>
__global__ void __launch_bounds__(kCtileBlock, sizeof(T) == 4 ? TRMC_TILE_WAVES_LAZY : 1)
k_mc_ctile_pkd(const StepArgs<T> a, const int32_t *__restrict__ cblk_ptr, const int32_t cb0, const int32_t tile, const int32_t K,
               T *const pk_d, int32_t *const pk_at)
{
    mc_ctile_rows<T, TOL, DEC, true, false, true>(a, cblk_ptr, cb0, tile, K, pk_d, pk_at);
}
template <class T, bool TOL = false, bool DEC = false, bool PKD = false>
__global__ void __launch_bounds__(kCtileBlock, sizeof(T) == 4 ? TRMC_TILE_WAVES_LAZY : 1)
k_mc_ctile_dpl(const StepArgs<T> a, const int32_t *__restrict__ cblk_ptr, const int32_t cb0, const int32_t tile, const int32_t K,
               T *const pk_d, int32_t *const pk_at)
{
    mc_ctile_rows<T, TOL, DEC, true, false, PKD, true>(a, cblk_ptr, cb0, tile, K, pk_d, pk_at);
}
template <class T, bool TOL, bool DEC, bool LAZYV, bool RDA, bool PKD, bool DPL>
__device__ __forceinline__ void mc_ctile_rows(const StepArgs<T> &a, const int32_t *__restrict__ cblk_ptr, const int32_t cb0,
                                              const int32_t tile, const int32_t K, T *const pk_d, int32_t *const pk_at)
{
    using M = typename DevMath<T, TOL>::type;
    const ColdArgs<StepArgs<T>> cold = cold_args<StepArgs<T>>();
    __shared__ uint64_t s_tab[TRMC_POW_TAB_WORDS];
    __shared__ T s_out[(DEC || !LAZYV) ? 3 * kCtileStage * kCtileBlock : 1];
    __shared__ T s_x[2 * kCtileBlock];
    M m{stage_pow_tables(s_tab), false};
    m.sane = a.sane;

    const int32_t cb = cb0 + (int32_t)blockIdx.x;
    const int32_t lo = cblk_ptr[cb], hi = cblk_ptr[cb + 1];
    int32_t behind, slot, slot_next;
    const bool in_range = seq_locate(a, tile, a.level[lo], behind, slot, slot_next);
    const int32_t t_lo = behind * K + 1, t_hi = min(behind * K + K, a.nsteps);
    if (!in_range || t_lo > t_hi) return;

    int32_t s = lo + (int32_t)threadIdx.x;
    bool active = s < hi;
    if (a.cls_last) {
        const int32_t c = active ? (int32_t)(a.cls_last[s] & 0x7f) : 0x80;
        const int32_t key = (c & 0x80) ? 8 : 7 - min(c, 7);
        bool none;
        s = lo + block_partition_by_class<kCtileBlock>(key, none);
        active = !none;
    }
    if (a.cls_last) {
        const int32_t cp = active ? (int32_t)(a.cls_last[s] & 0x7f) : 0;
        if (__any(cp >= 3)) __builtin_amdgcn_s_setprio(3);
        else if (__any(cp == 2)) __builtin_amdgcn_s_setprio(2);
        else __builtin_amdgcn_s_setprio(1);
    } else
        __builtin_amdgcn_s_setprio(2);
    const uint32_t su = (uint32_t)(active ? s : lo);
    const uint32_t sl = su - (uint32_t)lo;
    uint32_t ob = su * (uint32_t)sizeof(T);
    const size_t np = (size_t)a.nseg_pad;
    trmc::ChannelParams<T> p;
    trmc::ChannelConst<T> c;
    load_row_params(a, ob, p, c);
    int2 u = a.up2[su];
    if (!active) u.x = u.y = -1;
    const int32_t uy = u.y >= 0 ? (u.y & 0x3fffffff) : -1;
    const int32_t in0 = (u.x >= lo && u.x < hi) ? (u.x - lo) * (int32_t)sizeof(T) : -1;
    const int32_t in1 = (uy >= lo && uy < hi) ? (uy - lo) * (int32_t)sizeof(T) : -1;
    const int32_t ri = (active && a.res_of_pos) ? a.res_of_pos[su] : -1;
    const int32_t gi = (active && a.gage_of_pos) ? a.gage_of_pos[su] : -1;

    T *const q_tm = a.q_tm + (size_t)slot * (size_t)a.slot_tm;
    const size_t ql_base = (size_t)slot * (size_t)a.slot_qlat;
    T q_prev = at(q_tm + (size_t)(t_lo - 1) * np, ob);
    T d_prev = at(a.d_tm + (size_t)slot * (size_t)a.slot_tm + (size_t)(t_lo - 1) * np, ob);
    T *const out_row = a.out + (size_t)slot * (size_t)a.slot_out + (size_t)a.row_of_pos[su] * (size_t)a.nsteps * 3;
    int32_t ql_col = (t_lo - 1) / a.qts, ql_left = a.qts - (t_lo - 1) % a.qts;
    T ql = at(a.qlat_tm + ql_base + (size_t)ql_col * np, ob);
    m.coef_ok = coef_guard(p.dt, ql);
    const bool count_cost = a.it_sum != nullptr;
    int32_t it_acc = 0, it_last = 0, staged = 0;
    bool over_last = false;
    if (active) s_x[(size_t)((t_lo - 1) & 1) * kCtileBlock + sl] = q_prev;
    __syncthreads();
    T *q_up = q_tm + (size_t)(t_lo - 1) * np;
    const ptrdiff_t d_of_q = DPL ? a.d_tm - a.q_tm : 0;
    const int32_t v_every = (LAZYV && DEC) ? cold->v_every : 0;
    int32_t v_left = v_every > 0 ? (v_every - 1) - ((t_lo - 1) % v_every) : 0;
    T dmax = T(0);
    int32_t dmax_at = 1;
    if constexpr (PKD) {
        if (t_lo != 1) {
            const size_t col = (size_t)slot * np + (size_t)su;
            dmax = pk_d[col];
            dmax_at = pk_at[col];
        }
    }
    for (int32_t t = t_lo; t <= t_hi; ++t, q_up += np) {
        bool want_v = false;
        if constexpr (LAZYV && DEC) {
            want_v = v_every > 0 && v_left == 0;
            if (v_every > 0) v_left = v_left == 0 ? v_every - 1 : v_left - 1;
        }
        if (active) {
            if (ql_left == 0) {
                ++ql_col;
                ql = at(cold->qlat_tm + ql_base + (size_t)ql_col * np, ob);
                m.coef_ok = coef_guard(p.dt, ql);
                ql_left = cold->qts;
            }
            --ql_left;
            const T *const sx = s_x + (size_t)((t - 1) & 1) * kCtileBlock;
            T qup = T(0);
            if (u.x >= 0) qup += in0 >= 0 ? at(sx, (uint32_t)in0) : at(q_up, (uint32_t)u.x * (uint32_t)sizeof(T));
            if (uy >= 0) qup += in1 >= 0 ? at(sx, (uint32_t)in1) : at(q_up, (uint32_t)uy * (uint32_t)sizeof(T));
            if (uy >= 0) {
                if (u.y & 0x40000000) {
                    const int32_t *const up_ptr = cold->up_ptr, *const up_idx = cold->up_idx;
                    const int32_t k1 = up_ptr[su + 1];
                    for (int32_t k = up_ptr[su] + 2; k < k1; ++k) {
                        const int32_t uk = up_idx[k];
                        qup += (uk >= lo && uk < hi) ? sx[uk - lo] : at(q_up, (uint32_t)uk * (uint32_t)sizeof(T));
                    }
                }
            }
            T q_new, v_new, d_new;
            if (ri >= 0) {
                reservoir_row<T, M, RDA>(cold, m, slot, ri, t, qup, d_prev, q_new, v_new, d_new);
                it_last = 0;
            } else {
                trmc::Inflow<T> f;
                f.qup = qup;
                f.quc = qup;
                f.qdp = q_prev;
                f.ql = ql;
                const trmc::StepResult<T> r = trmc::mc_segment_step<T, M>(p, c, f, d_prev, m, !LAZYV);
                q_new = r.qdc;
                v_new = r.velc;
                d_new = r.depthc;
                it_last = r.iters;
                over_last = r.over;
                if (count_cost) it_acc += min(r.iters, 3) + (r.over ? 4 : 0);
                if (gi >= 0) nudge_row<T>(cold, slot, gi, t, q_new);
            }
            asm volatile("" : "+v"(ob));
            at(q_up + np, ob) = q_new;
            if constexpr (DPL) {
                if (t != t_hi) at(q_up + np + d_of_q, ob) = d_new;
            }
            s_x[(size_t)(t & 1) * kCtileBlock + sl] = q_new;
            hand_on_row<T>(cold, slot, slot_next, ob, np, t, t_hi, q_new, d_new);
            q_prev = q_new;
            d_prev = d_new;
            if constexpr (PKD) {
                if (t == 1 || d_new > dmax) {
                    dmax = d_new;
                    dmax_at = t;
                }
            }
            if (LAZYV && want_v && it_last > 0) v_new = trmc::step_velocity<T, M>(p, c, d_new, m);
// ... 50 lines not shown
```

t-route_amd/csrc/k_tile_row.inc:

```

template <class T>
__device__ __forceinline__ void load_row_params(const StepArgs<T> &a, uint32_t &ob, trmc::ChannelParams<T> &p, trmc::ChannelConst<T> &c)
{
    p.dt = a.dt_col ? at(a.dt_col, ob) : a.dt;
    asm volatile("" : "+v"(ob));
    p.dx = at(a.dx, ob);
    p.bw = at(a.bw, ob);
    p.twcc = at(a.twcc, ob);
    p.n = at(a.n, ob);
    p.ncc = at(a.ncc, ob);
    p.s0 = at(a.s0, ob);
    p.tw = p.cs = T(0);
    c.z = at(a.z, ob);
    c.bfd = at(a.bfd, ob);
    c.sqrt_s0 = at(a.sqrt_s0, ob);
    c.sq1pz2 = at(a.sq1pz2, ob);
    c.s0_n = at(a.s0_n, ob);
    c.s0_ncc = at(a.s0_ncc, ob);
    c.inv_n = at(a.inv_n, ob);
    trmc::derive_const(c, p);
}

template <class T, class M, bool RDA>
__device__ __forceinline__ void reservoir_row(ColdArgs<StepArgs<T>> cold, const M &m, int32_t slot, int32_t ri, int32_t t, T qup, T d_prev, T &q_new, T &v_new, T &d_new)
{
    const T *rp = cold->res_par + (size_t)ri * 9;
    const trmc::LevelPoolParams<T> lp{rp[0], rp[1], rp[2], rp[3], rp[4], rp[5], rp[6], rp[7], rp[8]};
    T H = d_prev;
    q_new = trmc::levelpool_step<T, M>(qup, T(0), cold->res_dt, H, lp, m);
    if constexpr (RDA) {
        void *const da = cold->res_da;
        trmc::ResDaState *const carry = (trmc::ResDaState *)cold->res_da_carry;
        const trmc::ResDaResult r =
            carry ? trmc::reservoir_da_row_day((char *)da + (size_t)slot * (size_t)cold->slot_rda, carry, ri, t, cold->nsteps, cold->res_t_end,
                                               qup, d_prev, cold->res_dt, rp, q_new, H)
                  : trmc::reservoir_da_row(da, ri, t, qup, d_prev, cold->res_dt, rp, q_new, H);
        q_new = r.outflow;
        H = r.water_elevation;
    }
    v_new = T(0);
    d_new = H;
    cold->res_inflow[(size_t)slot * (size_t)cold->slot_res + (size_t)ri * (size_t)cold->nsteps + (size_t)(t - 1)] = qup;
}

template <class T>
__device__ __forceinline__ void nudge_row(ColdArgs<StepArgs<T>> cold, int32_t slot, int32_t gi, int32_t t, T &q_new)
{
    const size_t e = (size_t)slot * (size_t)cold->slot_da + (size_t)gi * (size_t)cold->nsteps + (size_t)(t - 1);
    const T *const da_a = cold->da_a;
    const uint8_t mode = cold->da_mode[e];
    T nudge = T(0);
    if (mode == 1) {
        nudge = da_a[e] - q_new;
        q_new = da_a[e];
    } else if (mode == 2) {
        nudge = (da_a[e] - q_new) * cold->da_w[e];
        q_new = q_new + nudge;
    }
    cold->da_nudge[e] = nudge;
}

template <class T>
__device__ __forceinline__ void hand_on_row(ColdArgs<StepArgs<T>> cold, int32_t slot, int32_t slot_next, uint32_t ob, size_t np, int32_t t, int32_t t_hi, T q_new, T d_new)
{
    if (t == t_hi) {
        at(cold->d_tm + (size_t)slot * (size_t)cold->slot_tm + (size_t)t * np, ob) = d_new;
        if (cold->seq_slots > 1 && t == cold->nsteps) {
            at(cold->q_tm + (size_t)slot_next * (size_t)cold->slot_tm, ob) = q_new;
            at(cold->d_tm + (size_t)slot_next * (size_t)cold->slot_tm, ob) = d_new;
        }
    }
}
```

t-route_amd/csrc/kernels_levels.inc:

```
template <class A> using ColdArgs = const __attribute__((address_space(4))) A *;
template <class A> __device__ __forceinline__ ColdArgs<A> cold_args()
{
    ColdArgs<A> p = (ColdArgs<A>)__builtin_amdgcn_kernarg_segment_ptr();
    asm volatile("" : "+s"(p));
    return p;
}
template <class T> struct StepArgs {
    const T *dx, *bw, *twcc, *n, *ncc, *s0;
    const T *z, *bfd, *sqrt_s0, *sq1pz2, *s0_n, *s0_ncc, *inv_n;
    const T *dt_col;
    T dt;
    const int32_t *up_ptr, *up_idx, *level;
    const int2 *up2;
    const int32_t *lag;
    const T *qlat_tm;
    T *q_tm, *v_tm, *d_tm;
    uint8_t *it_prev;
    uint16_t *it_sum;
    bool sane;
    const int32_t *res_of_pos;
    const T *res_par;
    T *res_inflow;
    T res_dt;
    void *res_da;
// ... 215 lines not shown
}
template <class T, bool TOL = false, bool DEC = false>
__global__ void __launch_bounds__(kTileBlock, sizeof(T) == 4 ? TRMC_TILE_WAVES_LAZY : 1)
k_mc_tile_pkd(const StepArgs<T> a, const int32_t s_begin, const int32_t s_end, const int32_t tile, const int32_t K, T *const pk_d,
              int32_t *const pk_at)
{
    mc_tile_rows<T, TOL, DEC, true, false, true>(a, s_begin, s_end, tile, K, pk_d, pk_at);
}
template <class T, bool TOL = false, bool DEC = false, bool PKD = false>
__global__ void __launch_bounds__(kTileBlock, sizeof(T) == 4 ? TRMC_TILE_WAVES_LAZY : 1)
k_mc_tile_dpl(const StepArgs<T> a, const int32_t s_begin, const int32_t s_end, const int32_t tile, const int32_t K, T *const pk_d,
              int32_t *const pk_at)
{
    mc_tile_rows<T, TOL, DEC, true, false, PKD, true>(a, s_begin, s_end, tile, K, pk_d, pk_at);
}
template <class T, bool TOL, bool DEC, bool LAZYV, bool RDA, bool PKD, bool DPL>
__device__ __forceinline__ void mc_tile_rows(const StepArgs<T> &a, const int32_t s_begin, const int32_t s_end, const int32_t tile,
                                             const int32_t K, T *const pk_d, int32_t *const pk_at)
{
    using M = typename DevMath<T, TOL>::type;
    const ColdArgs<StepArgs<T>> cold = cold_args<StepArgs<T>>();
    __shared__ uint64_t s_tab[TRMC_POW_TAB_WORDS];
    __shared__ T s_out[(DEC || !LAZYV) ? 3 * kTileStage * kTileBlock : 1];
    M m{stage_pow_tables(s_tab), false};
    m.sane = a.sane;

    int32_t s;
    bool from_hot = false;
    int32_t *const hot_list = a.cls_last ? cold->hot_list : nullptr;
    const int32_t hot_blocks = hot_list ? cold->hot_home : 0;
    if ((int32_t)blockIdx.x < hot_blocks) {
        const int32_t cur = cold->hot_cur, cap = cold->hot_cap, H = cold->hot_wave_rows;
        const int32_t lane = (int32_t)(threadIdx.x & 63u), wave = (int32_t)blockIdx.x * (kTileBlock / 64) + (int32_t)(threadIdx.x >> 6);
        const int32_t i = wave * H + lane;
        const int32_t nlist = min(cold->hot_cnt[cur], cap);
        if (lane >= H || i >= nlist) return;
        if (lane == 0) atomicAdd(&cold->hot_cnt[3], min(nlist - i, H));
        s = hot_list[(size_t)cur * (size_t)cap + (size_t)i];
        from_hot = true;
        if (s < s_begin || s >= s_end) return;
    } else {
        const int32_t home = (int32_t)blockIdx.x - hot_blocks;
        const int32_t s_mine = s_begin + home * kTileBlock + (int32_t)threadIdx.x;
        s = s_mine;
        if (a.cls_last) {
            if (hot_list && home == 0 && threadIdx.x == 0) cold->hot_cnt[(cold->hot_cur + 2) % 3] = 0;
            int32_t c = s_mine < s_end ? (int32_t)(a.cls_last[s_mine] & 0x7f) : 0x80;
            if (hot_list && s_mine < s_end) {
                const int32_t n = cold->hot_seq;
                if (hot_list[(size_t)3 * (size_t)cold->hot_cap + (size_t)(n & 1) * (size_t)a.nseg_pad + (size_t)s_mine] == n) c = 0x80;
            }
            const int32_t key = (c & 0x80) ? 8 : 7 - min(c, 7);
            bool none;
            s = s_begin + home * kTileBlock + block_partition_by_class<kTileBlock>(key, none);
            if (none) return;
        }
        if (s >= s_end) return;
    }
    int32_t behind, slot, slot_next;
    const bool in_range = seq_locate(a, tile, a.level[s], behind, slot, slot_next);
    const int32_t t_lo = behind * K + 1, t_hi = min(behind * K + K, a.nsteps);
    if (!in_range || t_lo > t_hi) return;
    if (a.cls_last) {
        const int32_t cp = from_hot ? 7 : (int32_t)(a.cls_last[s] & 0x7f);
        if (__any(cp >= 3)) __builtin_amdgcn_s_setprio(3);
        else if (__any(cp == 2)) __builtin_amdgcn_s_setprio(1);
    }

    const uint32_t su = (uint32_t)s;
    uint32_t ob = su * (uint32_t)sizeof(T);
    const size_t np = (size_t)a.nseg_pad;
    trmc::ChannelParams<T> p;
    trmc::ChannelConst<T> c;
    load_row_params(a, ob, p, c);
    const int2 u = a.up2[su];
    const int32_t ri = a.res_of_pos ? a.res_of_pos[s] : -1;
    const int32_t gi = a.gage_of_pos ? a.gage_of_pos[s] : -1;

    T *const q_tm = a.q_tm + (size_t)slot * (size_t)a.slot_tm;
    const size_t ql_base = (size_t)slot * (size_t)a.slot_qlat;
    T q_prev = at(q_tm + (size_t)(t_lo - 1) * np, ob);
    T d_prev = at(a.d_tm + (size_t)slot * (size_t)a.slot_tm + (size_t)(t_lo - 1) * np, ob);
    T *const out_row = a.out + (size_t)slot * (size_t)a.slot_out + (size_t)a.row_of_pos[su] * (size_t)a.nsteps * 3;
    int32_t ql_col = (t_lo - 1) / a.qts, ql_left = a.qts - (t_lo - 1) % a.qts;
    T ql = at(a.qlat_tm + ql_base + (size_t)ql_col * np, ob);
    m.coef_ok = coef_guard(p.dt, ql);
    const bool count_cost = a.it_sum != nullptr;
    int32_t it_acc = 0, it_last = 0, staged = 0;
    bool over_last = false;
    T *q_up = q_tm + (size_t)(t_lo - 1) * np;
    const ptrdiff_t d_of_q = DPL ? a.d_tm - a.q_tm : 0;
    const int32_t v_every = (LAZYV && DEC) ? cold->v_every : 0;
    int32_t v_left = v_every > 0 ? (v_every - 1) - ((t_lo - 1) % v_every) : 0;
    T dmax = T(0);
    int32_t dmax_at = 1;
    if constexpr (PKD) {
        if (t_lo != 1) {
            const size_t col = (size_t)slot * np + (size_t)su;
            dmax = pk_d[col];
            dmax_at = pk_at[col];
        }
    }
    for (int32_t t = t_lo; t <= t_hi; ++t, q_up += np) {
        bool want_v = false;
        if constexpr (LAZYV && DEC) {
            want_v = v_every > 0 && v_left == 0;
            if (v_every > 0) v_left = v_left == 0 ? v_every - 1 : v_left - 1;
        }
        if (ql_left == 0) {
            ++ql_col;
            ql = at(cold->qlat_tm + ql_base + (size_t)ql_col * np, ob);
            m.coef_ok = coef_guard(p.dt, ql);
            ql_left = cold->qts;
        }
        --ql_left;
        T qup = T(0);
        if (u.x >= 0) qup += at(q_up, (uint32_t)u.x * (uint32_t)sizeof(T));
        if (u.y >= 0) {
            qup += at(q_up, (uint32_t)(u.y & 0x3fffffff) * (uint32_t)sizeof(T));
            if (u.y & 0x40000000) {
                const int32_t *const up_ptr = cold->up_ptr, *const up_idx = cold->up_idx;
                const int32_t k1 = up_ptr[su + 1];
                for (int32_t k = up_ptr[su] + 2; k < k1; ++k) qup += at(q_up, (uint32_t)up_idx[k] * (uint32_t)sizeof(T));
            }
        }
        T q_new, v_new, d_new;
        if (ri >= 0) {
            reservoir_row<T, M, RDA>(cold, m, slot, ri, t, qup, d_prev, q_new, v_new, d_new);
            it_last = 0;
        } else {
            trmc::Inflow<T> f;
            f.qup = qup;
            f.quc = qup;
            f.qdp = q_prev;
            f.ql = ql;
            const trmc::StepResult<T> r = trmc::mc_segment_step<T, M>(p, c, f, d_prev, m, !LAZYV);
            q_new = r.qdc;
            v_new = r.velc;
            d_new = r.depthc;
            it_last = r.iters;
            over_last = r.over;
            if (count_cost) it_acc += min(r.iters, 3) + (r.over ? 4 : 0);
            if (gi >= 0) nudge_row<T>(cold, slot, gi, t, q_new);
        }
        asm volatile("" : "+v"(ob));
        at(q_up + np, ob) = q_new;
        if constexpr (DPL) {
            if (t != t_hi) at(q_up + np + d_of_q, ob) = d_new;
        }
        hand_on_row<T>(cold, slot, slot_next, ob, np, t, t_hi, q_new, d_new);
        q_prev = q_new;
        d_prev = d_new;
        if constexpr (PKD) {
            if (t == 1 || d_new > dmax) {
                dmax = d_new;
                dmax_at = t;
            }
        }
        if (LAZYV && want_v && it_last > 0) v_new = trmc::step_velocity<T, M>(p, c, d_new, m);
        if (DEC || (!LAZYV && a.out)) {
            T *so = s_out + (size_t)(staged * 3) * kTileBlock + threadIdx.x;
            so[0] = q_new;
            so[kTileBlock] = v_new;
            so[2 * kTileBlock] = d_new;
            ++staged;
            if (staged == kTileStage || t == t_hi) {
                T *dst = out_row + (size_t)(t - staged) * 3;
// ... 1 lines not shown
                if (LAZYV || !a.out) {
                } else if (a.out_vec && (staged & 3) == 0) {
                    for (int j = 0; j < 3 * staged / 4; ++j) {
                        float4 v;
                        v.x = (float)si[(4 * j + 0) * kTileBlock];
                        v.y = (float)si[(4 * j + 1) * kTileBlock];
                        v.z = (float)si[(4 * j + 2) * kTileBlock];
                        v.w = (float)si[(4 * j + 3) * kTileBlock];
                        reinterpret_cast<float4 *>(dst)[j] = v;
                    }
                } else {
                    for (int32_t e = 0; e < 3 * staged; ++e) dst[e] = si[e * kTileBlock];
                }
                if constexpr (DEC) {
                    const int32_t ds = cold->dec_stride;
                    for (int32_t k = t / ds; k >= 1 && k * ds > t - staged; --k) {
                        if (k > cold->dec_keep) continue;
                        const int32_t kslot = k * ds - (t - staged) - 1;
                        T *dd = cold->dec + (size_t)slot * (size_t)cold->slot_dec + ((size_t)cold->row_of_pos[su] * (size_t)cold->dec_keep + (size_t)(k - 1)) * 3;
                        dd[0] = si[(kslot * 3 + 0) * kTileBlock];
                        dd[1] = si[(kslot * 3 + 1) * kTileBlock];
                        dd[2] = si[(kslot * 3 + 2) * kTileBlock];
                    }
                }
                staged = 0;
            }
        }
    }
    if constexpr (PKD) {
        const size_t col = (size_t)slot * np + (size_t)su;
        pk_d[col] = dmax;
        pk_at[col] = dmax_at;
    }
    if (t_hi == cold->nsteps) cold->it_prev[su] = (uint8_t)min(it_last, 255);
    if (uint8_t *const cls = cold->cls_last) {
        uint8_t c = (uint8_t)(min(it_last, 3) + (over_last ? 4 : 0));
        const bool hot = hot_list && c >= 3 && (t_hi < cold->nsteps || cold->seq_slots > 1);
        if (hot && (from_hot || __builtin_popcountll(__ballot(hot)) < TRMC_HOT_WAVE_MAX)) {
            const int32_t nxt = (cold->hot_cur + 1) % 3, cap = cold->hot_cap;
            const int32_t i = atomicAdd(&cold->hot_cnt[nxt], 1);
            if (i < cap) {
                hot_list[(size_t)nxt * (size_t)cap + (size_t)i] = s;
                const int32_t n = cold->hot_seq + 1;
                hot_list[(size_t)3 * (size_t)cap + (size_t)(n & 1) * (size_t)a.nseg_pad + (size_t)su] = n;
            }
        }
        cls[su] = c;
    }
    if (uint16_t *const it_sum = cold->it_sum) it_sum[su] = (uint16_t)min(65535, (int)it_sum[su] + it_acc);
}

#include "k_mc_ctile.inc"

constexpr int kConstCols = 7, kTotalCols = TRMC_NPARAM + kConstCols;
template <class T>
__global__ void __launch_bounds__(kBlock)
k_make_const(T *cols, int32_t nseg, int64_t nseg_pad)
{
    using M = typename DevMath<T>::type;
    const int32_t s = blockIdx.x * kBlock + threadIdx.x;
    if (s >= nseg) return;
    const M m{nullptr, false};
    trmc::ChannelParams<T> p;
    p.dt = cols[(size_t)TRMC_P_DT * nseg_pad + s];
    p.dx = cols[(size_t)TRMC_P_DX * nseg_pad + s];
    p.bw = cols[(size_t)TRMC_P_BW * nseg_pad + s];
    p.tw = cols[(size_t)TRMC_P_TW * nseg_pad + s];
    p.twcc = cols[(size_t)TRMC_P_TWCC * nseg_pad + s];
    p.n = cols[(size_t)TRMC_P_N * nseg_pad + s];
    p.ncc = cols[(size_t)TRMC_P_NCC * nseg_pad + s];
    p.cs = cols[(size_t)TRMC_P_CS * nseg_pad + s];
    p.s0 = cols[(size_t)TRMC_P_S0 * nseg_pad + s];
    const trmc::ChannelConst<T> c = trmc::make_const<T, M>(p, m);
    T *o = cols + (size_t)TRMC_NPARAM * nseg_pad + s;
    o[0 * nseg_pad] = c.z;
    o[1 * nseg_pad] = c.bfd;
    o[2 * nseg_pad] = c.sqrt_s0;
    o[3 * nseg_pad] = c.sq1pz2;
    o[4 * nseg_pad] = c.s0_n;
    o[5 * nseg_pad] = c.s0_ncc;
    o[6 * nseg_pad] = c.inv_n;
}

template <class T>
__global__ void __launch_bounds__(kBlock)
k_prep_qlat(const T *__restrict__ in, const int32_t *__restrict__ row_of_pos, T *__restrict__ qlat_tm,
            int32_t nseg, int64_t nseg_pad, int32_t nq)
{
    __shared__ T tile[32][65];
    const int32_t p0 = blockIdx.x * 64;
    const int32_t j0 = blockIdx.y * 32;
    const int32_t nj = min(32, nq - j0);
    for (int32_t i = threadIdx.x; i < 64 * 32; i += kBlock) {
        const int32_t pl = i / 32, jl = i % 32;
        const int32_t p = p0 + pl;
        if (p < nseg && jl < nj) tile[jl][pl] = in[(size_t)row_of_pos[p] * nq + j0 + jl];
    }
    __syncthreads();
    for (int32_t i = threadIdx.x; i < 64 * 32; i += kBlock) {
        const int32_t jl = i / 64, pl = i % 64;
        const int32_t p = p0 + pl;
        if (p < nseg && jl < nj) qlat_tm[(size_t)(j0 + jl) * nseg_pad + p] = tile[jl][pl];
    }
}

struct PackSpec {
    double scale, offset;
    int32_t fill1, fill2, vmin, vmax;
    int32_t use1, use2;
};
__device__ __forceinline__ double unpack_cf(int32_t raw, const PackSpec &k)
{
    if ((k.use1 && raw == k.fill1) || (k.use2 && raw == k.fill2) || raw < k.vmin || raw > k.vmax) return 0.0;
    return (double)raw * k.scale + k.offset;
}
template <class T>
__device__ __forceinline__ T ingest_packed_at(const int32_t *__restrict__ raw_a, const int32_t *__restrict__ raw_b, const PackSpec &ka,
                                              const PackSpec &kb, int32_t f, size_t col)
{
    double v = 0.0;
    if (f >= 0) {
        v = unpack_cf(raw_a[col + (size_t)f], ka);
        if (raw_b) v = v + unpack_cf(raw_b[col + (size_t)f], kb);
    }
    return (T)(float)v;
}
template <class T>
__global__ void __launch_bounds__(kBlock)
k_ingest_packed(const int32_t *__restrict__ raw_a, const int32_t *__restrict__ raw_b, const PackSpec ka, const PackSpec kb,
                const int32_t *__restrict__ feat_of_pos, T *__restrict__ qlat_tm, int32_t nseg, int64_t nseg_pad, int32_t nq,
                int64_t nfeat)
{
    const int32_t p = blockIdx.x * kBlock + threadIdx.x;
    if (p >= nseg) return;
    const int32_t f = feat_of_pos[p];
    for (int32_t j = 0; j < nq; ++j)
        qlat_tm[(size_t)j * nseg_pad + p] = ingest_packed_at<T>(raw_a, raw_b, ka, kb, f, (size_t)j * (size_t)nfeat);
}
constexpr int32_t kIngestCols = 4;
template <class T>
__global__ void __launch_bounds__(kBlock)
k_ingest_packed_day(const int32_t *__restrict__ raw_a, const int32_t *__restrict__ raw_b, const PackSpec ka, const PackSpec kb,
                    const int32_t *__restrict__ feat_of_pos, T *__restrict__ qlat_tm, int32_t nseg, int64_t nseg_pad, int32_t nq,
                    int64_t nfeat)
{
    const int32_t p = blockIdx.x * kBlock + threadIdx.x;
    if (p >= nseg) return;
    const int32_t f = feat_of_pos[p];
    const int32_t j0 = (int32_t)blockIdx.y * kIngestCols;
    T v[kIngestCols];
#pragma unroll
    for (int32_t k = 0; k < kIngestCols; ++k)
        v[k] = j0 + k < nq ? ingest_packed_at<T>(raw_a, raw_b, ka, kb, f, (size_t)(j0 + k) * (size_t)nfeat) : T(0);
#pragma unroll
    for (int32_t k = 0; k < kIngestCols; ++k)
        if (j0 + k < nq) qlat_tm[(size_t)(j0 + k) * nseg_pad + p] = v[k];
}

template <class T>
__global__ void __launch_bounds__(kBlock)
k_init_state(const T *__restrict__ q0, const int32_t *__restrict__ row_of_pos, T *q_tm, T *v_tm, T *d_tm,
             int32_t nseg)
{
    const int32_t p = blockIdx.x * kBlock + threadIdx.x;
    if (p >= nseg) return;
    const size_t r = (size_t)row_of_pos[p] * 3;
    q_tm[p] = q0[r + 0];
    v_tm[p] = q0[r + 1];
    d_tm[p] = q0[r + 2];
}

template <class T>
__global__ void __launch_bounds__(kBlock)
k_fill_boundary(const T *__restrict__ bfvd, T *q_tm, T *v_tm, T *d_tm, int32_t nboundary, int32_t nsteps,
                int64_t nseg_pad)
{
    const int64_t i = (int64_t)blockIdx.x * kBlock + threadIdx.x;
    if (i >= (int64_t)nboundary * nsteps) return;
    const int32_t b = (int32_t)(i / nsteps), t = (int32_t)(i % nsteps) + 1;
    const size_t src = ((size_t)b * nsteps + (t - 1)) * 3;
    const size_t dst = (size_t)t * nseg_pad + b;
    q_tm[dst] = bfvd[src + 0];
    v_tm[dst] = bfvd[src + 1];
    d_tm[dst] = bfvd[src + 2];
}

// ... 251 lines not shown
```

t-route_amd/csrc/stream.inc:

```
extern "C++" {
enum : int {
    P_HYD,
    P_Q0,
    P_FVD,
    P_NUDGE,
    P_RES,
    P_RDA,
    P_RDA_IDX,
    P_PEAK,
    P_STEP,
    P_MEAN,
    P_PD,
    P_PDS,
    P_N
};
enum : int {
    P_STAGE = P_N,
    P_ALL
};
struct StreamProdRow {
    bool on = false;
    size_t bytes = 0;
    size_t stride = 0;
    char *base = nullptr;
    DevBuf buf;
    void *next = nullptr;
};
struct StreamProd {
    int64_t day = -1;
    void *host[P_ALL] = {};
    int32_t rowset = -1;
    bool queued = false;
    DevEvent ev_done;
};
struct StreamRun {
    DevStream fst;
    DevEvent ev_begin, ev_gat;
    DevMark mk_bnd;
    DevEvent ev_total;
    DevEvent ev_exc;
    DevEvent ev_cou0, ev_cou;
    DevEvent ev_dex0, ev_dex;
    DevEvent ev_pk0, ev_pk1;
    std::vector<DevEvent> ev_slab;
    std::vector<DevEvent> ev_free;
    std::vector<DevEvent> ev_ready;
    std::vector<DevEvent> ev_forcing;
    std::vector<DevEvent> ev_t0, ev_t1;
    std::vector<StreamProd> prod;
    HostBlock rda_stage;
    bool active = false;
    int32_t nsteps = 0, qts = 1, K = 0, tpd = 0, slots = 0, W = 0, C = 0, lmax = 0;
    int64_t nq = 0;
    int64_t days_pushed = 0, day_min = 0, days_complete = 0, g_done = -1, launches = 0;
    size_t plane = 0, slot_tm = 0, slot_qlat = 0, slot_out = 0, slot_dec = 0;
    bool want_out = false;
    int32_t dec_stride = 0, dec_keep = 0;
    int32_t rowset = -1;
    DevBuf tm, qlat, out, dec;
    StreamProdRow tab[P_ALL];
    size_t slot_res = 0, slot_da = 0;
    DevBuf da_mode, da_a, da_w;
    DevBuf da_q0;
    DevBuf gage_of_pos, gage_pos_dev;
    std::vector<int32_t> gage_pos;
    int64_t ngage = 0;
    bool rda_want = false, rda = false;
    int64_t rda_cap_want[3] = {0, 0, 0}, rda_cap[3] = {0, 0, 0};
    int64_t rda_off[3] = {0, 0, 0}, rda_time_off[3] = {0, 0, 0};
    size_t slot_rda = 0;
    float t_end = 0.0f;
    DevBuf rda_tab, rda_carry;
    int32_t sum_want = 0, sum = 0;
    bool carry = false;
    DevBuf pkd_d, pkd_at;
    bool stage_want = false, stage = false, dpl = false;
    bool cou_want = false, cou = false, cou_ms_ok = false;
    double cou_limit_want = 0.0, cou_limit = 0.0;
    DevBuf cou_peak, cou_step, cou_count, cou_rows;
    int64_t cou_days = 0;
    DevBuf tot[P_N - P_PEAK];
    int64_t tot_days = 0;
    int32_t exc_want = -1, exc = -1, exc_K = 0, exc_KP = 0;
    DevBuf exc_acc, exc_rows;
    int64_t exc_days = 0;
    int32_t dex_K_want = 0, dex_KP_want = 0, dex_K = 0, dex_KP = 0;
    bool dex_ms_ok = false;
    DevBuf dex_th, dex_acc, dex_rows;
    int64_t dex_days = 0;
    int64_t pk_nfeat = 0;
    bool pk_two = false, pk_ms_ok = false;
    PackSpec pk_a{}, pk_b{};
    DevBuf pk_feat_of_pos;
};

}
trmc_plan::trmc_plan() = default;
trmc_plan::~trmc_plan() = default;

extern "C++" {
namespace {

constexpr int kSlabEvents = 8;

inline size_t stream_raw_bytes(const StreamRun &S, bool two) { return (two ? 2 : 1) * (size_t)S.nq * (size_t)S.pk_nfeat * sizeof(int32_t); }

template <class T>
__global__ void __launch_bounds__(kBlock)
k_stream_boundary(const T *__restrict__ q_dev, T *__restrict__ q_plane, int32_t nboundary, int32_t nsteps, int64_t nseg_pad)
{
    const int64_t i = (int64_t)blockIdx.x * kBlock + threadIdx.x;
    if (i >= (int64_t)nboundary * nsteps) return;
    const int32_t b = (int32_t)(i / nsteps), t = (int32_t)(i % nsteps) + 1;
    q_plane[(size_t)t * nseg_pad + b] = q_dev[i];
}
template <class T>
__global__ void __launch_bounds__(kBlock)
k_stream_boundary_idx(const T *__restrict__ q_dev, int64_t src_stride, const int64_t *__restrict__ index, T *__restrict__ q_plane,
                      int32_t nboundary, int32_t nsteps, int64_t nseg_pad)
{
    const int64_t i = (int64_t)blockIdx.x * kBlock + threadIdx.x;
    if (i >= (int64_t)nboundary * nsteps) return;
    const int32_t b = (int32_t)(i / nsteps), t = (int32_t)(i % nsteps) + 1;
    const int64_t r = index ? index[b] : b;
    q_plane[(size_t)t * nseg_pad + b] = q_dev[(size_t)r * (size_t)src_stride + (size_t)(t - 1)];
}

template <class T>
__global__ void __launch_bounds__(kBlock)
k_stream_first_obs(const int32_t *__restrict__ gage_pos, const int32_t *__restrict__ gage_of_pos, const int32_t *__restrict__ lagk,
                   const T *__restrict__ da_q0, T *__restrict__ q_tm, int32_t ngage, int32_t p0, int32_t p1, int64_t g, int32_t tpd,
                   int32_t slots, int64_t day_min, int64_t days, int64_t slot_tm)
{
    const int32_t gi = (int32_t)blockIdx.x * kBlock + (int32_t)threadIdx.x;
    if (gi >= ngage) return;
    const int32_t p = gage_pos[gi];
    if (p < p0 || p >= p1 || gage_of_pos[p] != gi) return;
    const int64_t i = g - lagk[p];
    if (i < 0 || i % tpd != 0) return;
    const int64_t day = i / tpd;
    if (day < day_min || day >= days) return;
    const int32_t slot = (int32_t)(day % slots);
    const T v = da_q0[(size_t)slot * (size_t)ngage + (size_t)gi];
    if (v == v) q_tm[(size_t)slot * (size_t)slot_tm + (size_t)p] = v;
}

__global__ void __launch_bounds__(kBlock) k_stream_rda_state(const trmc::ResDaRec *__restrict__ rec, float *__restrict__ state,
                                                             int32_t *__restrict__ tsidx, int32_t nres)
{
    const int32_t i = (int32_t)blockIdx.x * kBlock + (int32_t)threadIdx.x;
    if (i >= nres) return;
    const trmc::ResDaState s = rec[i].st;
    state[4 * i + 0] = s.update_time;
    state[4 * i + 1] = s.prev_persisted;
    state[4 * i + 2] = s.persistence_index;
    state[4 * i + 3] = s.persistence_update_time;
    tsidx[i] = s.timeseries_idx;
}

inline void stream_rda_image(const trmc_plan *pl, const StreamRun &S, const trmc_stream_reservoir_da &d, float *img)
{
    std::memset(img, 0, S.slot_rda);
    const trmc_reservoir_da_table *tab[3] = {&d.usgs, &d.usace, &d.rfc};
    for (int k = 0; k < 3; ++k) {
        if (tab[k]->n <= 0) continue;
        std::memcpy(img + S.rda_off[k], tab[k]->obs, (size_t)(tab[k]->n * tab[k]->ncol) * sizeof(float));
        if (k < 2) std::memcpy(img + S.rda_time_off[k], tab[k]->time, (size_t)tab[k]->ncol * sizeof(float));
    }
    trmc::ResDaRec *rec = reinterpret_cast<trmc::ResDaRec *>(img);
    for (int64_t i = 0; i < pl->nres; ++i) {
        trmc::ResDaRec r{};
        r.kind = pl->res_da_kind[(size_t)i];
        if (r.kind != 0) {
            const int k = r.kind == 2 ? 0 : (r.kind == 3 ? 1 : 2);
            const trmc_reservoir_da_table &t = *tab[k];
            const int64_t j = pl->res_da_trow[(size_t)i];
            r.ncol = (int32_t)t.ncol;
            r.obs_off = S.rda_off[k] + j * t.ncol;
            r.time_off = S.rda_time_off[k];
            if (k == 2) {
                const int32_t *ip = t.ipar + 5 * j;
                r.st.timeseries_idx = ip[0];
                r.total_counts = ip[1];
                r.use_forecast = ip[2];
                r.da_timestep = ip[3];
                r.persist_days = ip[4];
                r.reset_idx = d.rfc_reset_idx != 0;
// ... 129 lines not shown
        }
        HIP_TRY(hipEventRecord(S.ev_exc, pst));
        S.exc_days = e + 1;
    }
    if (S.cou && pl->nseg > 0) {
        StreamCourantArgs<T> c;
        c.par = (const T *)pl->sh->params.p;
        c.nseg_pad = pl->nseg_pad;
        c.up_ptr = (const int32_t *)pl->sh->up_ptr.p;
        c.up_idx = (const int32_t *)pl->sh->up_idx.p;
        c.res_of_pos = pl->nres > 0 ? (const int32_t *)pl->res_of_pos.p : nullptr;
        c.q_tm = q;
        c.d0 = d;
        if (S.dpl) {
            c.row_of_pos = nullptr;
            c.d1 = d + (size_t)pl->nseg_pad;
            c.d_row = 1;
            c.d_step = pl->nseg_pad;
        } else {
            c.row_of_pos = (const int32_t *)pl->sh->row_of_pos.p;
            c.d1 = (const T *)S.out.p + (size_t)slot * S.slot_out + 2;
            c.d_row = 3 * (int64_t)S.nsteps;
            c.d_step = 3;
        }
        c.qlat = (const T *)S.qlat.p + (size_t)slot * S.slot_qlat;
        c.peak = (T *)S.cou_peak.p;
        c.step = (int32_t *)S.cou_step.p;
        c.count = (int32_t *)S.cou_count.p;
        c.nseg = (int32_t)pl->nseg;
        c.nboundary = (int32_t)pl->sh->topo.nboundary;
        c.nsteps = S.nsteps;
        c.qts = S.qts;
        c.t0 = (int32_t)(e * S.nsteps);
        c.sane = pl->params_sane ? 1 : 0;
        c.limit = (T)S.cou_limit;
        HIP_TRY(hipEventRecord(S.ev_cou0, pst));
        bool tol = false;
        if constexpr (std::is_same<T, float>::value) {
            tol = pl->opt.tol;
            if (tol) hipLaunchKernelGGL((k_stream_courant<float, true>), dim3(blocks_for(pl->nseg)), dim3(kBlock), 0, pst, c);
        }
        if (!tol) hipLaunchKernelGGL((k_stream_courant<T, false>), dim3(blocks_for(pl->nseg)), dim3(kBlock), 0, pst, c);
        HIP_TRY(hipEventRecord(S.ev_cou, pst));
        S.cou_days = e + 1;
        S.cou_ms_ok = true;
    }
    if (S.dex_K > 0 && pl->nseg > 0) {
        const int32_t t0 = (int32_t)(e * S.nsteps);
        const T *const d1 = S.dpl ? d + (size_t)pl->nseg_pad : (const T *)S.out.p + (size_t)slot * S.slot_out + 2;
        const int64_t d_row = S.dpl ? 1 : 3 * (int64_t)S.nsteps, d_step = S.dpl ? pl->nseg_pad : 3;
        auto fold = [&](auto kp) {
            hipLaunchKernelGGL((k_stream_exceed_depth<T, decltype(kp)::value>), dim3(blocks_for(pl->nseg)), dim3(kBlock), 0, pst, d1,
                               (const int32_t *)pl->sh->row_of_pos.p, (const T *)S.dex_th.p, (int32_t *)S.dex_acc.p, (int32_t)pl->nseg,
                               pl->nseg_pad, S.nsteps, t0, S.dpl ? 0 : 1, d_row, d_step);
        };
        HIP_TRY(hipEventRecord(S.ev_dex0, pst));
        switch (S.dex_KP) {
        case 1: fold(std::integral_constant<int, 1>{}); break;
        case 2: fold(std::integral_constant<int, 2>{}); break;
        case 4: fold(std::integral_constant<int, 4>{}); break;
        default: return fail(TRMC_ESTATE, "internal: the stream's depth exceedance has no threshold table");
        }
        HIP_TRY(hipEventRecord(S.ev_dex, pst));
        S.dex_days = e + 1;
        S.dex_ms_ok = true;
    }
    HIP_TRY(hipGetLastError());
    if (!any) {
        HIP_TRY(hipEventRecord(S.ev_free[(size_t)slot], pst));
        HIP_TRY(hipEventRecord(p.ev_done, pst));
        p.queued = true;
        return 0;
    }
    HIP_TRY(hipEventRecord(S.ev_ready[(size_t)slot], pst));
    HIP_TRY(hipStreamWaitEvent(pl->cstream, S.ev_ready[(size_t)slot], 0));
    for (int k = 0; k < P_ALL; ++k)
        if (bytes[k]) HIP_TRY(hipMemcpyAsync(p.host[k], at(k), bytes[k], hipMemcpyDeviceToHost, pl->cstream));
    HIP_TRY(hipEventRecord(S.ev_free[(size_t)slot], pl->cstream));
    HIP_TRY(hipEventRecord(p.ev_done, pl->cstream));
    p.queued = true;
    return 0;
}

template <class T> int stream_launch(trmc_plan *pl, StreamRun &S, int64_t g_from, int64_t g_to, int64_t days)
{
    const trmc::Topology &tp = pl->sh->topo;
    const bool tol = pl->opt.tol;
    const int32_t split = (pl->opt.stream_split > 0 && pl->opt.stream_split < S.W) ? pl->opt.stream_split : S.W;
    const int32_t w0 = tp.lvl_ptr[0], w1 = tp.lvl_ptr[split], w2 = tp.lvl_ptr[S.W];
    hipStream_t wst = pl->wstream, cst = pl->stream;
    hipStream_t pst = stream_last(pl, S);
    const int32_t ncblk = S.C > 0 ? (int32_t)tp.cblk_ptr.size() - 1 : 0;
    StepArgs<T> as = stream_args<T>(pl, S, days);
    tile_args(pl, S.W, as);
    StepArgs<T> a = as;
    a.hot_list = a.hot_cnt = nullptr;
    T *const pk_d = S.carry ? (T *)S.pkd_d.p : nullptr;
    int32_t *const pk_at = S.carry ? (int32_t *)S.pkd_at.p : nullptr;
    for (int64_t g = g_from + 1; g <= g_to; ++g) {
        a.seq_day = as.seq_day = (int32_t)(g / S.tpd);
        const int32_t tile = (int32_t)(g % S.tpd);
        auto first_obs = [&](hipStream_t st, int32_t p0, int32_t p1) {
            if (S.ngage > 0 && p1 > p0)
                hipLaunchKernelGGL((k_stream_first_obs<T>), dim3(blocks_for(S.ngage)), dim3(kBlock), 0, st, (const int32_t *)S.gage_pos_dev.p,
                                   (const int32_t *)S.gage_of_pos.p, a.level, (const T *)S.da_q0.p, (T *)S.tm.p, (int32_t)S.ngage, p0, p1, g, S.tpd,
                                   S.slots, S.day_min, days, (int64_t)S.slot_tm);
        };
        if (S.W > 0 && w1 > w0) {
            first_obs(wst, w0, w1);
            if (as.hot_list) tile_turn(pl, as);
            launch_tile<T>(wst, as, w0, w1, tile, S.K, tol, pk_d, pk_at, S.dpl);
            HIP_TRY(hipEventRecord(S.ev_slab[(size_t)(g % kSlabEvents)], wst));
            ++S.launches;
        }
        if (ncblk > 0 || w2 > w1) {
            if (S.W > 0 && g >= 1) HIP_TRY(hipStreamWaitEvent(cst, S.ev_slab[(size_t)((g - 1) % kSlabEvents)], 0));
            first_obs(cst, w1, (int32_t)pl->nseg_pad);
            if (w2 > w1) {
                launch_tile<T>(cst, a, w1, w2, tile, S.K, tol, pk_d, pk_at, S.dpl);
                ++S.launches;
            }
            if (ncblk > 0) {
                launch_ctile<T>(cst, a, (const int32_t *)pl->sh->cblk_ptr.p, 0, ncblk, tile, S.K, tol, pk_d, pk_at, S.dpl);
                ++S.launches;
            }
        }
        HIP_TRY(hipGetLastError());
        S.g_done = g;
        const int64_t i_last = g - S.lmax;
        if (i_last >= 0 && (i_last + 1) % S.tpd == 0) {
            const int64_t e = (i_last + 1) / S.tpd - 1;
            if (e >= S.days_complete && e < days)
                if (int rc = stream_complete_day<T>(pl, S, e, pst)) return rc;
        }
    }
    return 0;
}

template <class T> int stream_begin_t(trmc_plan *pl, int nsteps, int qts, int slots, int full_output, int output_stride)
{
    const trmc::Topology &tp = pl->sh->topo;
    if (!pl->seq) pl->seq = std::make_unique<StreamRun>();
    StreamRun &S = *pl->seq;
    const int32_t K = pl->opt.wide_k > 0 ? pl->opt.wide_k : 16;
    if (nsteps % K != 0) return fail(TRMC_EINVAL, "a stream of windows needs nsteps to be a multiple of the plan's wide_k (" + std::to_string(K) + ")");
    S.nsteps = nsteps;
    S.qts = qts;
    S.K = K;
    S.tpd = nsteps / K;
    S.W = tp.ncl > 0 ? tp.cl_from_level : tp.nlevels;
    S.C = tp.ncl;
    S.lmax = std::max(0, S.W + S.C - 1);
    const int32_t need = 2 + (S.lmax + 1 + S.tpd - 1) / S.tpd;
    S.slots = std::max(need, slots);
    S.nq = pl->nq;
    const size_t np = (size_t)pl->nseg_pad;
    S.plane = (size_t)(nsteps + 1) * np;
    S.slot_tm = 2 * S.plane;
    S.slot_qlat = (size_t)S.nq * np;
    S.want_out = full_output != 0;
    S.slot_out = S.want_out ? (size_t)pl->nseg * nsteps * 3 : 0;
    S.dec_stride = output_stride > 0 ? output_stride : 0;
    S.dec_keep = S.dec_stride > 0 ? nsteps / S.dec_stride : 0;
    if (S.dec_stride > 0 && S.dec_keep < 1) return fail(TRMC_EINVAL, "output_stride exceeds nsteps");
    S.slot_dec = (size_t)pl->nseg * S.dec_keep * 3;
    if (int rc = S.tm.ensure((size_t)S.slots * S.slot_tm * sizeof(T))) return rc;
    if (int rc = S.qlat.ensure((size_t)S.slots * S.slot_qlat * sizeof(T))) return rc;
    if (int rc = pl->in_qlat.ensure(std::max((size_t)pl->nseg * (size_t)S.nq * sizeof(T), stream_raw_bytes(S, S.pk_two)))) return rc;
    S.pk_ms_ok = false;
    if (S.pk_nfeat > 0)
        for (DevEvent *e : {&S.ev_pk0, &S.ev_pk1})
            if (int rc = e->ensure(true)) return rc;
    if (S.want_out)
        if (int rc = S.out.ensure((size_t)S.slots * S.slot_out * sizeof(T))) return rc;
    if (S.dec_stride > 0)
        if (int rc = S.dec.ensure((size_t)S.slots * S.slot_dec * sizeof(T))) return rc;
    S.slot_res = (size_t)pl->nres * (size_t)nsteps;
    S.slot_da = (size_t)S.ngage * (size_t)nsteps;
    if (S.slot_da > 0) {
        if (int rc = S.da_mode.ensure((size_t)S.slots * S.slot_da)) return rc;
        for (DevBuf *b : {&S.da_a, &S.da_w})
            if (int rc = b->ensure((size_t)S.slots * S.slot_da * sizeof(T))) return rc;
        if (int rc = S.da_q0.ensure((size_t)S.slots * (size_t)S.ngage * sizeof(T))) return rc;
    }
    S.sum = S.sum_want;
    const bool pd = (S.sum & TRMC_SUMMARY_PEAK_DEPTH) != 0;
    S.carry = pd && !S.want_out;
    if (S.carry && pl->opt.velocity_on_demand < 0)
        return fail(TRMC_EUNSUPPORTED, "the peak depth of a stream without full_output is carried by the tile kernels' on-demand-velocity instances: "
                                       "not with trmc_plan_options.velocity_on_demand < 0");
    S.rda = pl->nres > 0 && pl->res_da_on && S.rda_want;
    if (S.rda && pd)
        return fail(TRMC_EUNSUPPORTED, "the peak depth of the day (TRMC_SUMMARY_PEAK_DEPTH) is not supported in a stream with reservoir data "
                                       "assimilation: the _rda tile instances do not carry it");
    for (DevBuf *b : {&S.pkd_d, &S.pkd_at})
        if (!S.carry) b->release();
    if (S.carry) {
        if (int rc = S.pkd_d.ensure((size_t)S.slots * np * sizeof(T))) return rc;
        if (int rc = S.pkd_at.ensure((size_t)S.slots * np * sizeof(int32_t))) return rc;
    }
    S.stage = S.stage_want;
    S.cou = S.cou_want;
    S.cou_limit = S.cou_limit_want;
    S.cou_days = 0;
    S.cou_ms_ok = false;
    S.dex_K = S.dex_K_want;
    S.dex_KP = S.dex_KP_want;
    S.dex_days = 0;
    S.dex_ms_ok = false;
    S.dpl = (S.stage || S.cou || S.dex_K > 0) && !S.want_out;
    if (S.dpl && pl->opt.velocity_on_demand < 0)
        return fail(TRMC_EUNSUPPORTED, "the stage, and the depths the Courant number and the depth exceedance are formed from, of a stream without "
                                       "full_output are written by the tile kernels' on-demand-velocity instances: not with "
                                       "trmc_plan_options.velocity_on_demand < 0");
    if (S.rda && S.stage)
        return fail(TRMC_EUNSUPPORTED, "stage hydrographs (trmc_stream_set_stage) are not supported in a stream with reservoir data "
                                       "assimilation: the _rda tile instances do not write the depth plane");
    if (S.rda && S.cou)
        return fail(TRMC_EUNSUPPORTED, "the Courant number over the days (trmc_stream_set_courant) is not supported in a stream with reservoir "
                                       "data assimilation: the _rda tile instances do not write the depth plane");
    if (S.rda && S.dex_K > 0)
        return fail(TRMC_EUNSUPPORTED, "the depth exceedance over the days (trmc_stream_set_depth_exceedance) is not supported in a stream with "
                                       "reservoir data assimilation: the _rda tile instances do not write the depth plane");
    if (S.dpl && tp.nboundary > 0)
        HIP_TRY(hipMemset2DAsync((T *)S.tm.p + S.plane, S.slot_tm * sizeof(T), 0, S.plane * sizeof(T), (size_t)S.slots, pl->stream));
    if ((pd || S.stage || S.dex_K > 0) && S.want_out && tp.nboundary > 0) HIP_TRY(hipMemsetAsync(S.out.p, 0, (size_t)S.slots * S.slot_out * sizeof(T), pl->stream));
    const size_t row = (size_t)pl->nseg * sizeof(T), irow = (size_t)pl->nseg * sizeof(int32_t), lrow = (size_t)pl->nseg * sizeof(int64_t);
    const size_t fvd = (S.dec_stride > 0 ? S.slot_dec : S.slot_out) * sizeof(T), da = S.slot_da * sizeof(T), res = S.slot_res * sizeof(T);
    const size_t rda4 = (size_t)pl->nres * 4 * sizeof(float), rda1 = (size_t)pl->nres * sizeof(int32_t);
    const bool peak = (S.sum & TRMC_SUMMARY_PEAK) != 0, mean = (S.sum & TRMC_SUMMARY_MEAN) != 0;
    const struct { bool on; size_t bytes, stride; bool own; size_t total; } rows[] = {
         {true, 0, 0, true, 0},
         {true, 3 * row, 3 * row, true, 0},
         {S.dec_stride > 0 || S.want_out, fvd, fvd, false, 0},
         {S.slot_da > 0, da, da, true, 0},
         {S.slot_res > 0, res, res, true, 0},
         {S.rda, rda4, rda4 + rda1, true, 0},
         {S.rda, rda1, rda4 + rda1, false, 0},
// ... 13 lines not shown
        t.bytes = rows[k].bytes;
        t.stride = rows[k].stride;
        t.next = nullptr;
        if (k >= P_PEAK && !t.on) t.buf.release();
        if (rows[k].own && t.on)
            if (int rc = t.buf.ensure((size_t)S.slots * t.stride)) return rc;
        t.base = (char *)t.buf.p;
        if (k < P_PEAK || k >= P_N) continue;
        DevBuf &b = S.tot[k - P_PEAK];
        if (!(tot && t.on)) b.release();
        else if (int rc = b.ensure(rows[k].total)) return rc;
    }
    S.tab[P_FVD].base = (char *)(S.dec_stride > 0 ? S.dec.p : S.out.p);
    if (S.rda) S.tab[P_RDA_IDX].base = S.tab[P_RDA].base + rda4;
    if (tot)
        if (int rc = S.ev_total.ensure(false)) return rc;
    S.exc = S.exc_want;
    S.exc_days = 0;
    if (S.exc >= 0 && pl->th_levels < 1)
        return fail(TRMC_ESTATE, "the streams of this plan were told to form an exceedance (trmc_stream_set_exceedance), but its thresholds have been "
                                 "cleared since (trmc_plan_set_thresholds)");
    S.exc_K = S.exc >= 0 ? pl->th_levels : 0;
    S.exc_KP = S.exc >= 0 ? pl->th_pad : 0;
    const size_t exc_bytes = (size_t)kStreamExceedFields * (size_t)S.exc_KP * np * sizeof(int32_t);
    if (S.exc < 0) {
        S.exc_acc.release();
        S.exc_rows.release();
    } else {
        if (int rc = S.exc_acc.ensure(exc_bytes)) return rc;
        if (int rc = S.exc_rows.ensure(4 * (size_t)pl->nseg * (size_t)S.exc_K * sizeof(int64_t))) return rc;
        if (int rc = S.ev_exc.ensure(false)) return rc;
    }
    const size_t cou_off = ((size_t)pl->nseg * sizeof(T) + 255) / 256 * 256;
    if (!S.cou) {
        for (DevBuf *b : {&S.cou_peak, &S.cou_step, &S.cou_count, &S.cou_rows}) b->release();
    } else {
        if (int rc = S.cou_peak.ensure(np * sizeof(T))) return rc;
        if (int rc = S.cou_step.ensure(np * sizeof(int32_t))) return rc;
        if (int rc = S.cou_count.ensure(np * sizeof(int32_t))) return rc;
        if (int rc = S.cou_rows.ensure(cou_off + 2 * (size_t)pl->nseg * sizeof(int64_t))) return rc;
        for (DevEvent *e : {&S.ev_cou0, &S.ev_cou})
            if (int rc = e->ensure(true)) return rc;
    }
    const size_t dex_bytes = (size_t)kStreamExceedFields * (size_t)S.dex_KP * np * sizeof(int32_t);
    if (S.dex_K < 1) {
        S.dex_acc.release();
        S.dex_rows.release();
    } else {
        if (int rc = S.dex_acc.ensure(dex_bytes)) return rc;
        if (int rc = S.dex_rows.ensure(4 * (size_t)pl->nseg * (size_t)S.dex_K * sizeof(int64_t))) return rc;
        for (DevEvent *e : {&S.ev_dex0, &S.ev_dex})
            if (int rc = e->ensure(true)) return rc;
    }
    S.slot_rda = 0;
    if (S.rda) {
        int64_t floats = pl->nres * (int64_t)(sizeof(trmc::ResDaRec) / sizeof(float));
        for (int k = 0; k < 3; ++k) {
            const int64_t n = pl->res_da_n[k];
            S.rda_cap[k] = n > 0 ? std::max(S.rda_cap_want[k], pl->res_da_ncol[k]) : 0;
            S.rda_off[k] = floats;
            floats += n * S.rda_cap[k];
            S.rda_time_off[k] = floats;
            if (k < 2) floats += S.rda_cap[k];
        }
        S.slot_rda = ((size_t)floats * sizeof(float) + 63) / 64 * 64;
        S.t_end = (float)nsteps * (float)pl->res_dt;
        if (int rc = S.rda_tab.ensure((size_t)S.slots * S.slot_rda)) return rc;
        if (int rc = S.rda_carry.ensure((size_t)pl->nres * sizeof(trmc::ResDaState))) return rc;
        if (int rc = S.rda_stage.ensure((size_t)S.slots * S.slot_rda)) return rc;
        HIP_TRY(hipStreamSynchronize(pl->stream));
        std::vector<trmc::ResDaRec> rec((size_t)pl->nres);
        HIP_TRY(hipMemcpy(rec.data(), pl->res_da.p, rec.size() * sizeof(trmc::ResDaRec), hipMemcpyDeviceToHost));
        std::vector<trmc::ResDaState> carry((size_t)pl->nres);
        for (size_t i = 0; i < rec.size(); ++i) carry[i] = rec[i].st;
        HIP_TRY(hipMemcpy(S.rda_carry.p, carry.data(), carry.size() * sizeof(trmc::ResDaState), hipMemcpyHostToDevice));
    }
    if (int rc = ensure_copy_stream(pl)) return rc;
    if (int rc = ensure_tile_stream(pl)) return rc;
    if (int rc = ensure_events(S.ev_slab, kSlabEvents, false)) return rc;
    for (auto *v : {&S.ev_free, &S.ev_ready, &S.ev_forcing})
        if (int rc = ensure_events(*v, (size_t)S.slots, false)) return rc;
    for (auto *v : {&S.ev_t0, &S.ev_t1})
        if (int rc = ensure_events(*v, (size_t)S.slots, true)) return rc;
    S.prod.resize((size_t)S.slots);
    for (StreamProd &p : S.prod) {
        if (int rc = p.ev_done.ensure(false)) return rc;
        p.day = -1;
        p.queued = false;
    }
    for (DevEvent *e : {&S.ev_begin, &S.ev_gat})
        if (int rc = e->ensure(false)) return rc;
    S.mk_bnd.settle();
    S.days_pushed = S.day_min = S.days_complete = 0;
    S.g_done = -1;
    S.launches = 0;
    hipStream_t st = pl->stream;
    if (int rc = pl->mk_forcing.order(st)) return rc;
    pl->mk_forcing.settle();
    HIP_TRY(hipMemsetAsync(pl->it_prev.p, 0, (size_t)np, st));
    if (S.exc >= 0 && exc_bytes > 0) HIP_TRY(hipMemsetAsync(S.exc_acc.p, 0, exc_bytes, st));
    if (S.dex_K > 0 && dex_bytes > 0) HIP_TRY(hipMemsetAsync(S.dex_acc.p, 0, dex_bytes, st));
    if (S.cou && np > 0) {
        HIP_TRY(hipMemsetAsync(S.cou_peak.p, 0, np * sizeof(T), st));
        HIP_TRY(hipMemsetAsync(S.cou_step.p, 0, np * sizeof(int32_t), st));
        HIP_TRY(hipMemsetAsync(S.cou_count.p, 0, np * sizeof(int32_t), st));
    }
    if (pl->collect_cost) {
        if (int rc = pl->it_sum.ensure(np * sizeof(uint16_t))) return rc;
        HIP_TRY(hipMemsetAsync(pl->it_sum.p, 0, np * sizeof(uint16_t), st));
        pl->cost_nsteps = 0;
    }
    if (pl->nseg > 0) {
        T *q = (T *)S.tm.p;
        hipLaunchKernelGGL((k_init_state<T>), dim3(blocks_for(pl->nseg)), dim3(kBlock), 0, st, (const T *)pl->in_q0.p,
                           (const int32_t *)pl->sh->row_of_pos.p, q, q + S.plane ,
                           q + S.plane, (int32_t)pl->nseg);
    }
    if (int rc = tile_setup(pl, st, S.W)) return rc;
    if (!tile_partition_on(pl)) pl->cls_last.release();
    HIP_TRY(hipEventRecord(S.ev_begin, st));
    HIP_TRY(hipStreamWaitEvent(pl->wstream, S.ev_begin, 0));
    if (int rc = S.fst.ensure(hipStreamNonBlocking)) return rc;
    HIP_TRY(hipStreamWaitEvent(S.fst, S.ev_begin, 0));
    HIP_TRY(hipStreamWaitEvent(pl->hstream, S.ev_begin, 0));
    HIP_TRY(hipGetLastError());
    pl->q0_staged = false;
    pl->routed_nsteps = -1;
    S.active = true;
    return 0;
}

template <class T> int stream_push_t(trmc_plan *pl, const trmc_stream_day &day, const int32_t *raw_a, const int32_t *raw_b)
{
    StreamRun &S = *pl->seq;
    const void *const qlat = day.qlat, *const boundary_q_dev = day.boundary_q_dev;
    const int32_t rowset = day.rowset;
    const trmc::Topology &tp = pl->sh->topo;
    const int64_t d = S.days_pushed;
    const int32_t slot = (int32_t)(d % S.slots);
    const size_t np = (size_t)pl->nseg_pad;
    hipStream_t hst = S.fst;
    if (d >= S.slots && S.days_complete <= d - S.slots)
        return fail(TRMC_ESTATE, "internal: the slot of the new day still belongs to a day that has not been queued to its end");
    if ((S.exc >= 0 || S.cou || S.dex_K > 0) && (d + 1) * (int64_t)S.nsteps > (int64_t)INT32_MAX)
        return fail(TRMC_EUNSUPPORTED, "the exceedance and the Courant number over the days of a stream count its steps in 32 bits on the device: this "
                                       "day would take the stream past 2^31 - 1 steps -- begin a new stream");
    StreamProd &p = S.prod[(size_t)slot];
    if (S.rda && p.day >= 0) HIP_TRY(hipEventSynchronize(S.ev_forcing[(size_t)slot]));
    if (p.day >= 0 && p.queued) HIP_TRY(hipStreamWaitEvent(hst, S.ev_free[(size_t)slot], 0));
    for (const int k : {(int)P_HYD, (int)P_STAGE}) {
        if (!(k == P_HYD ? day.hyd_host != nullptr : S.tab[P_STAGE].next != nullptr) || rowset < 0) continue;
        StreamProdRow &h = S.tab[k];
        const size_t hb = (size_t)pl->rowset_n[(size_t)rowset] * S.nsteps * sizeof(T);
        if (hb > h.stride) {
            if (d > S.day_min || S.days_complete < d) {
                if (h.stride > 0) return fail(TRMC_ESTATE, "a larger row set than the stream's first one: begin a new stream");
            }
            h.stride = hb;
            if (int rc = h.buf.ensure((size_t)S.slots * hb)) return rc;
            h.base = (char *)h.buf.p;
        }
    }
    p.day = d;
    p.queued = false;
    p.rowset = rowset;
    void *const from_day[P_PEAK] = {day.hyd_host, day.q0_host, day.fvd_host, day.nudge_host, day.res_inflow_host, day.res_da_state_host,
                                    day.res_da_tsidx_host};
    for (int k = 0; k < P_ALL; ++k) {
        p.host[k] = k < P_PEAK ? from_day[k] : S.tab[k].next;
        S.tab[k].next = nullptr;
    }
    const size_t bytes = raw_a ? stream_raw_bytes(S, raw_b != nullptr) : (size_t)pl->nseg * S.nq * sizeof(T);
    if (int rc = pl->in_qlat.ensure(bytes)) return rc;
    if (pl->nseg > 0 && raw_a) {
        const size_t one = stream_raw_bytes(S, false);
        int32_t *const da = (int32_t *)pl->in_qlat.p, *const db = raw_b ? da + (size_t)S.nq * (size_t)S.pk_nfeat : nullptr;
        if (one > 0) HIP_TRY(hipMemcpyAsync(da, raw_a, one, hipMemcpyHostToDevice, hst));
        if (one > 0 && raw_b) HIP_TRY(hipMemcpyAsync(db, raw_b, one, hipMemcpyHostToDevice, hst));
        const int32_t n = (int32_t)pl->nseg;
        HIP_TRY(hipEventRecord(S.ev_pk0, hst));
        hipLaunchKernelGGL((k_ingest_packed_day<T>), dim3(blocks_for(n), (unsigned)((S.nq + kIngestCols - 1) / kIngestCols)), dim3(kBlock), 0, hst,
                           (const int32_t *)da, (const int32_t *)db, S.pk_a, S.pk_b, (const int32_t *)S.pk_feat_of_pos.p,
                           (T *)S.qlat.p + (size_t)slot * S.slot_qlat, n, pl->nseg_pad, (int32_t)S.nq, S.pk_nfeat);
        HIP_TRY(hipEventRecord(S.ev_pk1, hst));
        S.pk_ms_ok = true;
    } else if (pl->nseg > 0) {
        HIP_TRY(hipMemcpyAsync(pl->in_qlat.p, qlat, bytes, hipMemcpyHostToDevice, hst));
        const int32_t n = (int32_t)pl->nseg;
        hipLaunchKernelGGL((k_prep_qlat<T>), dim3((n + 63) / 64, (unsigned)((S.nq + 31) / 32)), dim3(kBlock), 0, hst, (const T *)pl->in_qlat.p,
                           (const int32_t *)pl->sh->row_of_pos.p, (T *)S.qlat.p + (size_t)slot * S.slot_qlat, n, pl->nseg_pad, (int32_t)S.nq);
    }
    if (S.slot_da > 0) {
        const size_t n = S.slot_da, o = (size_t)slot * S.slot_da;
        HIP_TRY(hipMemcpyAsync((uint8_t *)S.da_mode.p + o, day.da_mode, n, hipMemcpyHostToDevice, hst));
        HIP_TRY(hipMemcpyAsync((T *)S.da_a.p + o, day.da_a, n * sizeof(T), hipMemcpyHostToDevice, hst));
        HIP_TRY(hipMemcpyAsync((T *)S.da_w.p + o, day.da_w, n * sizeof(T), hipMemcpyHostToDevice, hst));
        HIP_TRY(hipMemsetAsync((T *)S.tab[P_NUDGE].base + o, 0, n * sizeof(T), hst));
        T *const q0o = (T *)S.da_q0.p + (size_t)slot * (size_t)S.ngage;
        if (day.da_q0) HIP_TRY(hipMemcpyAsync(q0o, day.da_q0, (size_t)S.ngage * sizeof(T), hipMemcpyHostToDevice, hst));
        else HIP_TRY(hipMemsetAsync(q0o, 0xff, (size_t)S.ngage * sizeof(T), hst));
    }
    if (S.rda) {
        float *const img = (float *)((char *)S.rda_stage.p + (size_t)slot * S.slot_rda);
        stream_rda_image(pl, S, *day.reservoir_da, img);
        HIP_TRY(hipMemcpyAsync((char *)S.rda_tab.p + (size_t)slot * S.slot_rda, img, S.slot_rda, hipMemcpyHostToDevice, hst));
    }
    if (int rc = S.mk_bnd.order(hst)) return rc;
    S.mk_bnd.settle();
    if (tp.nboundary > 0 && boundary_q_dev) {
        T *q = (T *)S.tm.p + (size_t)slot * S.slot_tm;
        if (d > 0) {
            const T *qp = (const T *)S.tm.p + (size_t)((d - 1) % S.slots) * S.slot_tm + (size_t)S.nsteps * np;
            HIP_TRY(hipMemcpyAsync(q, qp, (size_t)tp.nboundary * sizeof(T), hipMemcpyDeviceToDevice, hst));
        }
        hipLaunchKernelGGL((k_stream_boundary<T>), dim3(blocks_for(tp.nboundary * (int64_t)S.nsteps)), dim3(kBlock), 0, hst,
                           (const T *)boundary_q_dev, q, (int32_t)tp.nboundary, S.nsteps, pl->nseg_pad);
    }
    HIP_TRY(hipGetLastError());
    HIP_TRY(hipEventRecord(S.ev_forcing[(size_t)slot], hst));
    HIP_TRY(hipStreamWaitEvent(pl->wstream, S.ev_forcing[(size_t)slot], 0));
    HIP_TRY(hipStreamWaitEvent(pl->stream, S.ev_forcing[(size_t)slot], 0));
    if (S.cou && S.cou_days > 0) HIP_TRY(hipStreamWaitEvent(pl->wstream, S.ev_cou, 0));
    if (S.dex_K > 0 && S.dex_days > 0) HIP_TRY(hipStreamWaitEvent(pl->wstream, S.ev_dex, 0));
    S.days_pushed = d + 1;
    hipStream_t tst = S.W > 0 ? pl->wstream : pl->stream;
    HIP_TRY(hipEventRecord(S.ev_t0[(size_t)slot], tst));
    const int rc = stream_launch<T>(pl, S, d * S.tpd - 1, (d + 1) * S.tpd - 1, d + 1);
    if (!rc) HIP_TRY(hipEventRecord(S.ev_t1[(size_t)slot], tst));
    return rc;
}

}
}

static bool stream_active(const trmc_plan *pl) { return pl && pl->seq && pl->seq->active; }

static int stream_gages_check(trmc_plan *pl, const std::vector<int32_t> &gage_pos)
{
    if (pl->nres == 0 || gage_pos.empty()) return 0;
    if (int rc = use_device(pl)) return rc;
    std::vector<int32_t> res_of_pos((size_t)pl->nseg_pad);
    HIP_TRY(hipMemcpy(res_of_pos.data(), pl->res_of_pos.p, res_of_pos.size() * sizeof(int32_t), hipMemcpyDeviceToHost));
    for (const int32_t p : gage_pos)
        if (res_of_pos[(size_t)p] >= 0)
            return fail(TRMC_EINVAL, "a gage on a reservoir row is not supported (row " + std::to_string(pl->sh->topo.row_of_pos[(size_t)p]) + ")");
    return 0;
}

static int stream_check(trmc_plan *pl, bool want_active)
{
    if (!pl) return fail(TRMC_EINVAL, "plan is NULL");
    const bool act = pl->seq && pl->seq->active;
    if (want_active && !act) return fail(TRMC_ESTATE, "no stream of windows in progress (trmc_stream_begin)");
    if (!want_active && act) return fail(TRMC_ESTATE, "a stream of windows is in progress (trmc_stream_end it first)");
    return use_device(pl);
}

int trmc_stream_begin(trmc_plan *pl, int nsteps, int qts_subdivisions, int slots, int full_output, int output_stride)
{
    if (int rc = stream_check(pl, false)) return rc;
    if (pl->flow) return fail(TRMC_EINVAL, "a stream of windows runs on the level engine");
    if (pl->run.active) return fail(TRMC_ESTATE, "a routing window is in progress");
    const trmc::Topology &tp = pl->sh->topo;
    if (!(tp.ncl > 0 || (tp.cl_rows > 0 && tp.cl_from_level == tp.nlevels)))
        return fail(TRMC_EINVAL, "a stream of windows needs a plan in cluster order (TRMC_PLAN_SHORT_TS on the level engine, "
                                 "trmc_plan_options.cluster_rows >= 0): every row is then routed in tiles");
    if (pl->maxlag > 0) return fail(TRMC_EINVAL, "rows with a lag (trmc_plan_set_lag) have no place in a stream of windows: every row has its tile lag");
    if (pl->nres > 0 && pl->res_da_on) {
        if (!(pl->seq && pl->seq->rda_want))
            return fail(TRMC_EINVAL, "reservoir data assimilation (reservoir types 2-5, trmc_set_reservoir_da) is routed window by window "
                                     "unless the plan's streams were told to carry it (trmc_stream_set_reservoir_da)");
        if (int rc = reservoir_da_plan_check(pl)) return rc;
    }
    if (pl->ngage > 0 && !(pl->seq && pl->seq->ngage > 0))
        return fail(TRMC_EINVAL, "the nudging tables of trmc_set_nudging belong to one window: declare a stream's gage rows with "
                                 "trmc_stream_set_gages, its tables arrive with every day (trmc_stream_push_day)");
    if (pl->seq && pl->seq->ngage > 0)
        if (int rc = stream_gages_check(pl, pl->seq->gage_pos)) return rc;
    if (settle_deferred_state(pl)) return TRMC_ESTATE;
    if (pl->staged_nsteps < 0) return fail(TRMC_ESTATE, "trmc_upload_forcing (the state, and the shape of the forcing) must precede trmc_stream_begin");
    if (nsteps < 1 || qts_subdivisions < 1) return fail(TRMC_EINVAL, "nsteps and qts_subdivisions must be >= 1");
    if ((int64_t)(nsteps - 1) / qts_subdivisions >= pl->nq)
        return fail(TRMC_EINVAL, "Number of columns (timesteps) in Qlat is incorrect: need " + std::to_string((nsteps - 1) / qts_subdivisions + 1)
                                     + ", got " + std::to_string(pl->nq));
    if (output_stride < 0 || slots < 0) return fail(TRMC_EINVAL, "slots and output_stride must be >= 0");
    const int rc = by_precision(pl, [&](auto t) { return stream_begin_t<decltype(t)>(pl, nsteps, qts_subdivisions, slots, full_output, output_stride); });
    if (rc && pl->seq) pl->seq->active = false;
    return rc;
}

int trmc_stream_set_gages(trmc_plan *pl, int64_t ngage, const int64_t *gage_rows)
{
    if (int rc = stream_check(pl, false)) return rc;
    if (pl->flow) return fail(TRMC_EINVAL, "a stream of windows runs on the level engine");
    if (ngage < 0) return fail(TRMC_EINVAL, "ngage < 0");
    if (ngage > 0 && !gage_rows) return fail(TRMC_EINVAL, "gage_rows is NULL");
    if (!pl->seq) pl->seq = std::make_unique<StreamRun>();
    StreamRun &S = *pl->seq;
    S.ngage = 0;
    S.gage_pos.clear();
    if (ngage == 0) return 0;
    std::vector<int32_t> g_of_pos((size_t)pl->nseg_pad, -1), pos((size_t)ngage);
    for (int64_t g = 0; g < ngage; ++g) {
        const int64_t r = gage_rows[g];
// ... 470 lines not shown

int trmc_stream_gather(trmc_plan *pl, int64_t day, int32_t rowset, void *dst_dev, void *stream)
{
    if (int rc = stream_check(pl, true)) return rc;
    StreamRun &S = *pl->seq;
    if (rowset < 0 || rowset >= (int32_t)pl->rowsets.size()) return fail(TRMC_EINVAL, "unknown row set");
    if (!dst_dev) return fail(TRMC_EINVAL, "dst_dev is NULL");
    if (day < 0 || day >= S.days_pushed) return fail(TRMC_EINVAL, "the day has not been pushed");
    if (S.prod[(size_t)(day % S.slots)].day != day) return fail(TRMC_ESTATE, "the day's slot has been reused");
    if (S.g_done < (day + 1) * S.tpd - 1 + pl->rowset_lagk[(size_t)rowset])
        return fail(TRMC_ESTATE, "the rows of the set have not been queued through day " + std::to_string(day) + " yet (they run up to "
                                     + std::to_string(pl->rowset_lagk[(size_t)rowset]) + " tiles behind)");
    const int64_t nrows = pl->rowset_n[(size_t)rowset];
    if (nrows == 0) return 0;
    hipStream_t pst = stream_last(pl, S);
    hipStream_t st = stream ? (hipStream_t)stream : pst;
    if (st != pst) {
        HIP_TRY(hipEventRecord(S.ev_gat, pst));
        HIP_TRY(hipStreamWaitEvent(st, S.ev_gat, 0));
    }
    if (S.W > 0 && st != pl->wstream) {
        HIP_TRY(hipEventRecord(S.ev_gat, pl->wstream));
        HIP_TRY(hipStreamWaitEvent(st, S.ev_gat, 0));
    }
    const int32_t slot = (int32_t)(day % S.slots);
    return by_precision(pl, [&](auto t) -> int {
        using T = decltype(t);
        hipLaunchKernelGGL((k_gather_rows<T>), dim3(blocks_for(nrows * S.nsteps)), dim3(kBlock), 0, st, (const T *)S.tm.p + (size_t)slot * S.slot_tm,
                           (const int32_t *)pl->rowsets[(size_t)rowset].p, (T *)dst_dev, nrows, pl->nseg_pad, S.nsteps, 1);
        HIP_TRY(hipGetLastError());
        return 0;
    });
}

int trmc_stream_advance(trmc_plan *pl, int ntiles)
{
    if (int rc = stream_check(pl, true)) return rc;
    StreamRun &S = *pl->seq;
    if (ntiles < 0) return fail(TRMC_EINVAL, "ntiles < 0");
    const int64_t g_last = S.days_pushed * S.tpd - 1 + S.lmax;
    const int64_t g_from = std::max<int64_t>(S.g_done, S.days_pushed * S.tpd - 1);
    const int64_t g_to = std::min<int64_t>(g_last, g_from + ntiles);
    int rc = 0;
    if (S.days_complete < S.days_pushed && g_to > g_from) {
        if (int rc = S.mk_bnd.order(pl->wstream)) return rc;
        if (int rc = S.mk_bnd.order(pl->stream)) return rc;
        S.mk_bnd.settle();
        rc = by_precision(pl, [&](auto t) { return stream_launch<decltype(t)>(pl, S, g_from, g_to, S.days_pushed); });
    }
    if (!rc && S.days_complete >= S.days_pushed) S.day_min = S.days_pushed;
    return rc;
}

int trmc_stream_flush(trmc_plan *pl) { return trmc_stream_advance(pl, 1 << 30); }

int trmc_stream_wait(trmc_plan *pl, int64_t day)
{
    if (int rc = stream_check(pl, true)) return rc;
    StreamRun &S = *pl->seq;
    if (day < 0 || day >= S.days_pushed) return fail(TRMC_EINVAL, "no such day in the stream");
    StreamProd &p = S.prod[(size_t)(day % S.slots)];
    if (p.day != day) return fail(TRMC_ESTATE, "the day's slot has been reused: its products were handed over long ago");
    if (!p.queued)
        return fail(TRMC_ESTATE, "day " + std::to_string(day) + " has not been queued to its end: its last rows run " + std::to_string(S.lmax)
                                     + " tiles behind its first -- push further days or trmc_stream_flush");
    HIP_TRY(hipEventSynchronize(p.ev_done));
    return 0;
}

int trmc_stream_day_ms(trmc_plan *pl, int64_t day, double *ms_out)
{
    if (int rc = stream_check(pl, true)) return rc;
    StreamRun &S = *pl->seq;
    if (!ms_out) return fail(TRMC_EINVAL, "ms_out is NULL");
    if (day < 0 || day >= S.days_pushed || S.prod[(size_t)(day % S.slots)].day != day) return fail(TRMC_EINVAL, "no such day in the ring");
    const size_t slot = (size_t)(day % S.slots);
    HIP_TRY(hipEventSynchronize(S.ev_t1[slot]));
    float ms = 0;
    HIP_TRY(hipEventElapsedTime(&ms, S.ev_t0[slot], S.ev_t1[slot]));
    *ms_out = ms;
    return 0;
}

int trmc_stream_info(const trmc_plan *pl, int32_t *slots, int32_t *tiles_per_day, int32_t *lag_max, int32_t *wide_levels,
                     int32_t *cluster_levels, int64_t *days_pushed, int64_t *days_complete, int64_t *launches)
{
    if (!pl || !pl->seq) return fail(TRMC_ESTATE, "no stream of windows was begun on this plan");
    const StreamRun &S = *pl->seq;
    if (slots) *slots = S.slots;
    if (tiles_per_day) *tiles_per_day = S.tpd;
    if (lag_max) *lag_max = S.lmax;
    if (wide_levels) *wide_levels = S.W;
    if (cluster_levels) *cluster_levels = S.C;
    if (days_pushed) *days_pushed = S.days_pushed;
    if (days_complete) *days_complete = S.days_complete;
    if (launches) *launches = S.launches;
    return 0;
}

int trmc_stream_end(trmc_plan *pl)
{
    if (int rc = stream_check(pl, true)) return rc;
    StreamRun &S = *pl->seq;
    if (int rc = trmc_stream_flush(pl)) return rc;
    if (S.days_pushed > 0 && pl->nseg > 0) {
        const int32_t slot = (int32_t)((S.days_pushed - 1) % S.slots);
        if (int rc = pl->in_q0.ensure((size_t)pl->nseg * 3 * pl->esz)) return rc;
        hipStream_t pst = stream_last(pl, S);
        const int rc = by_precision(pl, [&](auto t) -> int {
            using T = decltype(t);
            const T *q = (const T *)S.tm.p + (size_t)slot * S.slot_tm;
            hipLaunchKernelGGL((k_final_state<T>), dim3(blocks_for(pl->nseg)), dim3(kBlock), 0, pst, q, q + S.plane, (const int32_t *)pl->sh->row_of_pos.p,
                               (T *)pl->in_q0.p, (int32_t)pl->nseg, pl->nseg_pad, S.nsteps, 1, S.nsteps);
            HIP_TRY(hipGetLastError());
            return 0;
        });
        if (rc) return rc;
        pl->q0_staged = true;
        pl->state_missing = false;
    }
    HIP_TRY(hipStreamSynchronize(pl->wstream));
    HIP_TRY(hipStreamSynchronize(pl->stream));
    HIP_TRY(hipStreamSynchronize(pl->hstream));
    if (S.fst) HIP_TRY(hipStreamSynchronize(S.fst));
    HIP_TRY(hipStreamSynchronize(pl->cstream));
    if (pl->collect_cost) pl->cost_nsteps = (int32_t)std::min<int64_t>(S.days_pushed * S.nsteps, 1 << 30);
    for (StreamProdRow &t : S.tab) t.next = nullptr;
    S.active = false;
    return 0;
}
```

t-route_amd/csrc/trmc.hip:

```cpp
#include <hip/hip_runtime.h>

#include <cmath>
#include <cstdint>
#include <cstdio>
#include <cstdlib>
#include <cstring>
#include <algorithm>
#include <limits>
#include <memory>
#include <mutex>
#include <new>
#include <string>
#include <type_traits>
#include <utility>
#include <vector>

#include "../../include/trmc.h"
#include "det_pow.h"
#include "det_pow64.h"
#include "mc_segment.hpp"
#include "levelpool.hpp"
#include "reservoir_da.hpp"
#include "topology.hpp"
#include "internal.hpp"
// ... 100 lines not shown
    std::vector<DevEvent> wide_t0, wide_t1;
    std::vector<DevEvent> tile_ev;
    DevEvent ev_emit;
    DevEvent ev_chain[4];
    DevMark mk_released[2];
    DevStream fstream;
    DevEvent ev_chunk[2];
    DevEvent ev_ctl;
    DevMark mk_dec;
    DevStream cstream;
    DevStream hstream;
    DevEvent ev_fetch_ready;
    DevMark mk_fetch_done;
    DevMark mk_gather;
    KernelTimer t_wsum;
    KernelTimer t_cour;
    KernelTimer t_wexc;
    DevMark mk_forcing;
    std::shared_ptr<PlanShared> sh;
    bool is_clone = false;
    int device = 0;
    int precision = 32;
    size_t esz = 4;
    int64_t nseg = 0, nseg_pad = 0, nrouted = 0;
    bool dt_uniform = true;
    double dt = 0.0;
    DevBuf it_prev;
    DevBuf it_sum;
    bool collect_cost = false;
    bool hinted = false;
    bool params_sane = false;
    int32_t cost_nsteps = -1;
    int32_t maxlag = 0;
    int64_t wide_safe_pos = -1;
    bool chain_staged = false;
    std::vector<int32_t> lag_of_row;
    DevBuf gage_of_pos, da_mode, da_a, da_w, da_nudge;
    DevBuf res_of_pos, res_par, res_inflow;
    int64_t nres = 0;
    double res_dt = 0.0;
    std::vector<int64_t> res_rows;
    DevBuf thresholds;
    int32_t th_levels = 0, th_pad = 0;
    DevBuf res_da;
    bool res_da_on = false;
    std::vector<int32_t> res_da_kind, res_da_trow;
    int64_t res_da_n[3] = {0, 0, 0}, res_da_ncol[3] = {0, 0, 0};
    int64_t ngage = 0;
    int64_t nraw = 0;
    DevBuf raw_of_pos, da_raw;
    int32_t da_nsteps = -1;
    DevBuf in_qlat, in_q0, in_bfvd, qlat_tm, tm, out, scratch, gathered;
    size_t gathered_bytes = 0;
    int64_t nq = 0;
    bool qlat_direct = false;
    DevBuf qlat_alt;
    bool qlat_alt_ready = false;
    bool have_boundary = true;
    int32_t staged_nsteps = -1;
    int32_t routed_nsteps = -1;
    bool flow = false;
    uint32_t tag_base = 1;
    int32_t tag_span = 0;
    DevBuf d_gran;
    int flow_next = 0;
    int flow_last = 0;
    DevBuf d_state, ticket, dbg;
    DevBuf cuq_head;
    int32_t ncuq = 0;
    uint64_t watchdog_ticks = 3000000000ull;
    struct Opt {
        bool tol = false;
        int64_t wide_min_rows = 0;
        int32_t wide_levels = 16, wide_k = 16;
        int64_t mid_min_rows = 0;
        int32_t mid_levels = 12, mid_k = 4;
        int32_t tile_perm_group = -1;
        int32_t hot_rows = -1;
        int32_t cluster_rows = 0;
        int32_t cluster_late_lag = 0;
        int32_t stream_split = 0;
        int32_t hot_wave_rows = 0;
        int32_t velocity_on_demand = 0;
        bool sequence = false;
        bool flow_overlap = false;
        int32_t flow_lean = 0;
        bool flow_debug = false;
    } opt;
    trmc_stats stats{};
    RouteRun run;
    int32_t out_stride = 0;
    DevBuf dec;
    int32_t dec_stride_done = 0, dec_keep_done = 0, dec_nsteps_done = 0, dec_lo_done = 0, dec_hi_done = 0;
    unsigned long long *stamps = nullptr;
    int32_t nstamp_windows = 0;
    int64_t stamp_seq = -1;
    DevBuf fetch_hyd, fetch_q0, fetch_fvd;
    bool row0_replaced = false;
    bool state_missing = false;
    bool q0_staged = false;
    DevBuf hot_list, hot_cnt;
    int32_t hot_cap = 0;
    bool nan_is_zero = false;
    int64_t tile_seq = 0;
    DevBuf cls_last;
    std::vector<DevBuf> rowsets;
    std::vector<int64_t> rowset_n;
    std::vector<int32_t> rowset_lag;
    std::vector<int32_t> rowset_lagk;
    std::unique_ptr<StreamRun> seq;
};

namespace {
#include "host_levels.inc"
#include "host_flow.inc"
#include "host_misc.inc"
}

extern "C" {
#include "abi.inc"
#include "stream.inc"

}
```

Before: 71.19 billion.

## Split lateral-inflow forcing upload into column groups with per-tile event waits

Adds an optional forcing_groups setting that splits each day's host-to-device qlat copy and transpose into column groups, recording an event per group, so routing tiles wait only for the forcing columns they need instead of the whole day. The prep_qlat transpose kernel is generalized to a variable column-width tile with pitch and column offset. Some DA, reservoir and boundary uploads are moved ahead of the forcing copy. The default group count is 1, so the grouped path is off unless the option is set, but the reworked transpose kernel with different tile shapes runs by default.

After: 71.16 billion. No clear change (-0.0%).

```diff
diff --git a/include/trmc.h b/include/trmc.h
--- a/include/trmc.h
+++ b/include/trmc.h
@@ -85,7 +85,8 @@
     int32_t stream_split;
     int32_t hot_wave_rows;
     int32_t velocity_on_demand;
-    int32_t reserved[2];
+    int32_t forcing_groups;
+    int32_t reserved[1];
 } trmc_plan_options;
 int trmc_plan_create_opt(int64_t nseg, const int64_t *up_ptr, const int64_t *up_idx,
                          const float *params, const uint8_t *boundary, const uint8_t *cost_hint,
@@ -131,6 +132,7 @@
                      int32_t *cluster_levels, int64_t *days_pushed, int64_t *days_complete, int64_t *launches);
 int trmc_stream_day_ms(trmc_plan *plan, int64_t day, double *ms_out);
 int trmc_stream_end(trmc_plan *plan);
+int trmc_stream_forcing_group(int nsteps, int64_t nq, int tile_steps, int groups, int tile);
 
 int trmc_plan_set_sequence_mode(trmc_plan *plan, int on);
 int trmc_plan_arithmetic(const trmc_plan *plan, int32_t *arithmetic);
diff --git a/t-route_amd/_lib.py b/t-route_amd/_lib.py
--- a/t-route_amd/_lib.py
+++ b/t-route_amd/_lib.py
@@ -33,7 +33,7 @@
         ("wide_k", C.c_int32), ("mid_min_rows", C.c_int64), ("mid_levels", C.c_int32), ("mid_k", C.c_int32),
         ("tile_perm_group", C.c_int32), ("tail_sort", C.c_int32), ("stem_min_rows", C.c_int32), ("sequence_mode", C.c_int32),
         ("flow_watchdog_ms", C.c_int32), ("flow_overlap", C.c_int32), ("flow_lean", C.c_int32), ("flow_debug", C.c_int32), ("hot_rows", C.c_int32),
-        ("cluster_rows", C.c_int32), ("cluster_late_lag", C.c_int32), ("stream_split", C.c_int32), ("hot_wave_rows", C.c_int32), ("velocity_on_demand", C.c_int32), ("reserved", C.c_int32 * 2),
+        ("cluster_rows", C.c_int32), ("cluster_late_lag", C.c_int32), ("stream_split", C.c_int32), ("hot_wave_rows", C.c_int32), ("velocity_on_demand", C.c_int32), ("forcing_groups", C.c_int32), ("reserved", C.c_int32 * 1),
     ]
 
 
@@ -41,7 +41,7 @@
 OPTION_ENV = {
     "TRMC_WIDE_MIN_ROWS": ("wide_min_rows", "off0"), "TRMC_WIDE_LEVELS": ("wide_levels", "int"), "TRMC_WIDE_K": ("wide_k", "int"),
     "TRMC_MID_MIN_ROWS": ("mid_min_rows", "off0"), "TRMC_MID_LEVELS": ("mid_levels", "int"), "TRMC_MID_K": ("mid_k", "int"),
-    "TRMC_TILE_PERM": ("tile_perm_group", "off0"), "TRMC_HOT_ROWS": ("hot_rows", "off0"), "TRMC_CLUSTER_ROWS": ("cluster_rows", "int"), "TRMC_STREAM_SPLIT": ("stream_split", "int"), "TRMC_HOT_WAVE_ROWS": ("hot_wave_rows", "int"), "TRMC_VELOCITY_ON_DEMAND": ("velocity_on_demand", "int"), "TRMC_TAIL_SORT": ("tail_sort", "off0"),
+    "TRMC_TILE_PERM": ("tile_perm_group", "off0"), "TRMC_HOT_ROWS": ("hot_rows", "off0"), "TRMC_CLUSTER_ROWS": ("cluster_rows", "int"), "TRMC_STREAM_SPLIT": ("stream_split", "int"), "TRMC_HOT_WAVE_ROWS": ("hot_wave_rows", "int"), "TRMC_VELOCITY_ON_DEMAND": ("velocity_on_demand", "int"), "TRMC_FORCING_GROUPS": ("forcing_groups", "int"), "TRMC_TAIL_SORT": ("tail_sort", "off0"),
     "TRMC_STEM_MIN_ROWS": ("stem_min_rows", "off0"), "TRMC_SETUP_ASIDE": ("sequence_mode", "flag"),
     "TRMC_FLOW_WATCHDOG_MS": ("flow_watchdog_ms", "int"), "TRMC_FLOW_OVERLAP": ("flow_overlap", "flag"),
     "TRMC_FLOW_LEAN": ("flow_lean", "lean"), "TRMC_FLOW_DEBUG": ("flow_debug", "flag"),
@@ -121,6 +121,7 @@
     "trmc_stream_info": (_int, [_vp, _P(_i32), _P(_i32), _P(_i32), _P(_i32), _P(_i32), _P(_i64), _P(_i64), _P(_i64)]),
     "trmc_stream_day_ms": (_int, [_vp, _i64, _P(C.c_double)]),
     "trmc_stream_end": (_int, [_vp]),
+    "trmc_stream_forcing_group": (_int, [_int, _i64, _int, _int, _int]),
     "trmc_plan_arithmetic": (_int, [_vp, _P(_i32)]),
     "trmc_plan_engine": (_int, [_vp, _P(_i32)]),
     "trmc_plan_destroy": (None, [_vp]),
diff --git a/t-route_amd/csrc/abi.inc b/t-route_amd/csrc/abi.inc
--- a/t-route_amd/csrc/abi.inc
+++ b/t-route_amd/csrc/abi.inc
@@ -274,6 +274,7 @@
         po.stream_split = std::max(0, o.stream_split);
         po.hot_wave_rows = std::max(0, std::min(64, o.hot_wave_rows));
         po.velocity_on_demand = o.velocity_on_demand;
+        po.forcing_groups = std::max(0, o.forcing_groups);
         po.sequence = o.sequence_mode != 0;
         po.flow_overlap = o.flow_overlap != 0;
         po.flow_lean = o.flow_lean;
@@ -467,11 +468,10 @@
     if (pl->opt.sequence && !pl->flow && pl->nseg > 0) {
         if (int rc = pl->qlat_alt.ensure((size_t)nq * pl->nseg_pad * pl->esz)) return rc;
         const int32_t n = (int32_t)pl->nseg;
-        const dim3 grid((n + 63) / 64, (unsigned)((nq + 31) / 32));
         const int rc = by_precision(pl, [&](auto t) {
             using T = decltype(t);
-            hipLaunchKernelGGL((k_prep_qlat<T>), grid, dim3(kBlock), 0, pl->hstream, (const T *)pl->in_qlat.p,
-                               (const int32_t *)pl->sh->row_of_pos.p, (T *)pl->qlat_alt.p, n, pl->nseg_pad, (int32_t)nq);
+            prep_qlat_launch<T>(pl->hstream, (const T *)pl->in_qlat.p, (const int32_t *)pl->sh->row_of_pos.p, (T *)pl->qlat_alt.p, n, pl->nseg_pad,
+                                (int32_t)nq, 0, (int32_t)nq);
             return launched();
         });
         if (rc) return rc;
diff --git a/t-route_amd/csrc/host_flow.inc b/t-route_amd/csrc/host_flow.inc
--- a/t-route_amd/csrc/host_flow.inc
+++ b/t-route_amd/csrc/host_flow.inc
@@ -189,8 +189,7 @@
     if (pl->collect_cost) HIP_TRY(hipMemsetAsync(pl->it_sum.p, 0, (size_t)np * sizeof(uint16_t), st));
     if (n > 0) {
         if (!pl->qlat_direct)
-            hipLaunchKernelGGL((k_prep_qlat<float>), dim3((n + 63) / 64, (unsigned)((pl->nq + 31) / 32)), dim3(kBlock), 0, st,
-                               (const float *)pl->in_qlat.p, row_of_pos, (float *)pl->qlat_tm.p, n, np, (int32_t)pl->nq);
+            prep_qlat_launch<float>(st, (const float *)pl->in_qlat.p, row_of_pos, (float *)pl->qlat_tm.p, n, np, (int32_t)pl->nq, 0, (int32_t)pl->nq);
         hipLaunchKernelGGL(k_flow_init, dim3(blocks_for(n)), dim3(kBlock), 0, st, (const float *)pl->in_q0.p, row_of_pos,
                            (unsigned long long *)pl->tm.p, (float *)pl->d_state.p, (unsigned long long *)pl->d_gran.p, n,
                            pl->tag_base);
diff --git a/t-route_amd/csrc/host_levels.inc b/t-route_amd/csrc/host_levels.inc
--- a/t-route_amd/csrc/host_levels.inc
+++ b/t-route_amd/csrc/host_levels.inc
@@ -367,8 +367,7 @@
     if (pl->collect_cost) HIP_TRY(hipMemsetAsync(pl->it_sum.p, 0, (size_t)np * sizeof(uint16_t), st));
     if (n > 0) {
         if (!pl->qlat_direct && !qlat_early)
-            hipLaunchKernelGGL((k_prep_qlat<T>), dim3((n + 63) / 64, (unsigned)((pl->nq + 31) / 32)), dim3(kBlock), 0, st,
-                               (const T *)pl->in_qlat.p, row_of_pos, (T *)pl->qlat_tm.p, n, np, (int32_t)pl->nq);
+            prep_qlat_launch<T>(st, (const T *)pl->in_qlat.p, row_of_pos, (T *)pl->qlat_tm.p, n, np, (int32_t)pl->nq, 0, (int32_t)pl->nq);
         if (!pl->chain_staged)
             hipLaunchKernelGGL((k_init_state<T>), dim3(blocks_for(n)), dim3(kBlock), 0, st, (const T *)pl->in_q0.p,
                                row_of_pos, a.q_tm, a.v_tm, a.d_tm, n);
diff --git a/t-route_amd/csrc/k_mc_ctile.inc b/t-route_amd/csrc/k_mc_ctile.inc
--- a/t-route_amd/csrc/k_mc_ctile.inc
+++ b/t-route_amd/csrc/k_mc_ctile.inc
@@ -90,7 +90,7 @@
     T q_prev = at(q_tm + (size_t)(t_lo - 1) * np, ob);
     T d_prev = at(a.d_tm + (size_t)slot * (size_t)a.slot_tm + (size_t)(t_lo - 1) * np, ob);
     T *const out_row = a.out + (size_t)slot * (size_t)a.slot_out + (size_t)a.row_of_pos[su] * (size_t)a.nsteps * 3;
-    int32_t ql_col = (t_lo - 1) / a.qts, ql_left = a.qts - (t_lo - 1) % a.qts;
+    int32_t ql_col = TRMC_FORCING_COL_OF_STEP(t_lo, a.qts), ql_left = a.qts - (t_lo - 1) % a.qts;
     T ql = at(a.qlat_tm + ql_base + (size_t)ql_col * np, ob);
     m.coef_ok = coef_guard(p.dt, ql);
     const bool count_cost = a.it_sum != nullptr;
diff --git a/t-route_amd/csrc/k_tile_row.inc b/t-route_amd/csrc/k_tile_row.inc
--- a/t-route_amd/csrc/k_tile_row.inc
+++ b/t-route_amd/csrc/k_tile_row.inc
@@ -1,3 +1,6 @@
+
+#define TRMC_FORCING_COL_OF_STEP(t, qts) (((t) - 1) / (qts))
+__host__ __device__ constexpr int32_t forcing_col_of_step(int32_t t, int32_t qts) { return TRMC_FORCING_COL_OF_STEP(t, qts); }
 
 template <class T>
 __device__ __forceinline__ void load_row_params(const StepArgs<T> &a, uint32_t &ob, trmc::ChannelParams<T> &p, trmc::ChannelConst<T> &c)
diff --git a/t-route_amd/csrc/kernels_levels.inc b/t-route_amd/csrc/kernels_levels.inc
--- a/t-route_amd/csrc/kernels_levels.inc
+++ b/t-route_amd/csrc/kernels_levels.inc
@@ -321,7 +321,7 @@
     T q_prev = at(q_tm + (size_t)(t_lo - 1) * np, ob);
     T d_prev = at(a.d_tm + (size_t)slot * (size_t)a.slot_tm + (size_t)(t_lo - 1) * np, ob);
     T *const out_row = a.out + (size_t)slot * (size_t)a.slot_out + (size_t)a.row_of_pos[su] * (size_t)a.nsteps * 3;
-    int32_t ql_col = (t_lo - 1) / a.qts, ql_left = a.qts - (t_lo - 1) % a.qts;
+    int32_t ql_col = TRMC_FORCING_COL_OF_STEP(t_lo, a.qts), ql_left = a.qts - (t_lo - 1) % a.qts;
     T ql = at(a.qlat_tm + ql_base + (size_t)ql_col * np, ob);
     m.coef_ok = coef_guard(p.dt, ql);
     const bool count_cost = a.it_sum != nullptr;
@@ -489,26 +489,38 @@
     o[6 * nseg_pad] = c.inv_n;
 }
 
+constexpr int32_t kPrepTile = 2048;
 template <class T>
 __global__ void __launch_bounds__(kBlock)
 k_prep_qlat(const T *__restrict__ in, const int32_t *__restrict__ row_of_pos, T *__restrict__ qlat_tm,
-            int32_t nseg, int64_t nseg_pad, int32_t nq)
-{
-    __shared__ T tile[32][65];
-    const int32_t p0 = blockIdx.x * 64;
-    const int32_t j0 = blockIdx.y * 32;
-    const int32_t nj = min(32, nq - j0);
-    for (int32_t i = threadIdx.x; i < 64 * 32; i += kBlock) {
-        const int32_t pl = i / 32, jl = i % 32;
+            int32_t nseg, int64_t nseg_pad, int32_t pitch, int32_t c0, int32_t cnt, int32_t cs)
+{
+    __shared__ T tile[kPrepTile + 32];
+    const int32_t cw = 1 << cs, np = kPrepTile >> cs;
+    const int32_t p0 = blockIdx.x * np;
+    const int32_t j0 = blockIdx.y * cw;
+    const int32_t nj = min(cw, cnt - j0);
+    for (int32_t i = threadIdx.x; i < kPrepTile; i += kBlock) {
+        const int32_t pl = i >> cs, jl = i & (cw - 1);
         const int32_t p = p0 + pl;
-        if (p < nseg && jl < nj) tile[jl][pl] = in[(size_t)row_of_pos[p] * nq + j0 + jl];
+        if (p < nseg && jl < nj) tile[jl * (np + 1) + pl] = in[(size_t)row_of_pos[p] * pitch + j0 + jl];
     }
     __syncthreads();
-    for (int32_t i = threadIdx.x; i < 64 * 32; i += kBlock) {
-        const int32_t jl = i / 64, pl = i % 64;
+    for (int32_t i = threadIdx.x; i < kPrepTile; i += kBlock) {
+        const int32_t jl = i >> (11 - cs), pl = i & (np - 1);
         const int32_t p = p0 + pl;
-        if (p < nseg && jl < nj) qlat_tm[(size_t)(j0 + jl) * nseg_pad + p] = tile[jl][pl];
-    }
+        if (p < nseg && jl < nj) qlat_tm[(size_t)(c0 + j0 + jl) * nseg_pad + p] = tile[jl * (np + 1) + pl];
+    }
+}
+template <class T>
+inline void prep_qlat_launch(hipStream_t st, const T *in, const int32_t *row_of_pos, T *qlat_tm, int32_t n, int64_t nseg_pad, int32_t pitch,
+                             int32_t c0, int32_t cnt)
+{
+    int32_t cs = 0;
+    while (cs < 5 && (1 << cs) < cnt) ++cs;
+    const int32_t np = kPrepTile >> cs;
+    hipLaunchKernelGGL((k_prep_qlat<T>), dim3((unsigned)((n + np - 1) / np), (unsigned)((cnt + (1 << cs) - 1) >> cs)), dim3(kBlock), 0, st, in,
+                       row_of_pos, qlat_tm, n, nseg_pad, pitch, c0, cnt, cs);
 }
 
 struct PackSpec {
diff --git a/t-route_amd/csrc/stream.inc b/t-route_amd/csrc/stream.inc
--- a/t-route_amd/csrc/stream.inc
+++ b/t-route_amd/csrc/stream.inc
@@ -46,12 +46,16 @@
     std::vector<DevEvent> ev_free;
     std::vector<DevEvent> ev_ready;
     std::vector<DevEvent> ev_forcing;
+    std::vector<DevEvent> ev_fgroup;
     std::vector<DevEvent> ev_t0, ev_t1;
     std::vector<StreamProd> prod;
     HostBlock rda_stage;
     bool active = false;
     int32_t nsteps = 0, qts = 1, K = 0, tpd = 0, slots = 0, W = 0, C = 0, lmax = 0;
     int64_t nq = 0;
+    int32_t fgroups = 1, fg_done = -1;
+    std::vector<int32_t> fg_n;
+    int64_t fg_day = -1;
     int64_t days_pushed = 0, day_min = 0, days_complete = 0, g_done = -1, launches = 0;
     size_t plane = 0, slot_tm = 0, slot_qlat = 0, slot_out = 0, slot_dec = 0;
     bool want_out = false;
@@ -103,6 +107,25 @@
 
 constexpr int kSlabEvents = 8;
 
+constexpr int32_t kForcingGroupsDefault = 1;
+
+inline int32_t forcing_groups_of(int64_t nq, int32_t G) { return (int32_t)std::max<int64_t>(1, std::min<int64_t>(G, nq)); }
+inline void forcing_group_cols(int64_t nq, int32_t n, int32_t i, int32_t &first, int32_t &count)
+{
+    const int32_t w = (int32_t)(nq / n);
+    first = i * w;
+    count = i == n - 1 ? (int32_t)nq - first : w;
+}
+inline int stream_forcing_group(int nsteps, int64_t nq, int K, int groups, int tile)
+{
+    if (nsteps < 1 || nq < 1 || K < 1 || tile < 0 || (int64_t)tile * K >= nsteps) return -1;
+    const int32_t qts = (int32_t)((nsteps - 1) / nq) + 1;
+    const int32_t t_last = (int32_t)std::min<int64_t>((int64_t)K * (tile + 1), nsteps);
+    const int64_t col = std::min<int64_t>(forcing_col_of_step(t_last, qts), nq - 1);
+    const int32_t n = forcing_groups_of(nq, groups);
+    return (int)std::min<int64_t>(col / (nq / n), n - 1);
+}
+
 inline size_t stream_raw_bytes(const StreamRun &S, bool two) { return (two ? 2 : 1) * (size_t)S.nq * (size_t)S.pk_nfeat * sizeof(int32_t); }
 
 template <class T>
@@ -398,6 +421,23 @@
     return 0;
 }
 
+inline int stream_forcing_wait(trmc_plan *pl, StreamRun &S, int64_t day, int32_t tile, int64_t days)
+{
+    if (day >= days) return 0;
+    const size_t slot = (size_t)(day % S.slots);
+    const int32_t n = S.fg_n[slot];
+    if (n <= 1) return 0;
+    const int need = stream_forcing_group(S.nsteps, S.nq, S.K, n, tile);
+    if (need < 0) return fail(TRMC_ESTATE, "internal: a tile launch outside its day");
+    if (day == S.fg_day && need <= S.fg_done) return 0;
+    hipEvent_t ev = S.ev_fgroup[slot * (size_t)S.fgroups + (size_t)need];
+    HIP_TRY(hipStreamWaitEvent(pl->wstream, ev, 0));
+    HIP_TRY(hipStreamWaitEvent(pl->stream, ev, 0));
+    S.fg_day = day;
+    S.fg_done = need;
+    return 0;
+}
+
 template <class T> int stream_launch(trmc_plan *pl, StreamRun &S, int64_t g_from, int64_t g_to, int64_t days)
 {
     const trmc::Topology &tp = pl->sh->topo;
@@ -416,6 +456,7 @@
     for (int64_t g = g_from + 1; g <= g_to; ++g) {
         a.seq_day = as.seq_day = (int32_t)(g / S.tpd);
         const int32_t tile = (int32_t)(g % S.tpd);
+        if (int rc = stream_forcing_wait(pl, S, g / S.tpd, tile, days)) return rc;
         auto first_obs = [&](hipStream_t st, int32_t p0, int32_t p1) {
             if (S.ngage > 0 && p1 > p0)
                 hipLaunchKernelGGL((k_stream_first_obs<T>), dim3(blocks_for(S.ngage)), dim3(kBlock), 0, st, (const int32_t *)S.gage_pos_dev.p,
@@ -470,6 +511,7 @@
     const int32_t need = 2 + (S.lmax + 1 + S.tpd - 1) / S.tpd;
     S.slots = std::max(need, slots);
     S.nq = pl->nq;
+    S.fgroups = S.nq < 2 ? 1 : forcing_groups_of(S.nq, pl->opt.forcing_groups > 0 ? pl->opt.forcing_groups : kForcingGroupsDefault);
     const size_t np = (size_t)pl->nseg_pad;
     S.plane = (size_t)(nsteps + 1) * np;
     S.slot_tm = 2 * S.plane;
@@ -649,6 +691,11 @@
         if (int rc = ensure_events(*v, (size_t)S.slots, false)) return rc;
     for (auto *v : {&S.ev_t0, &S.ev_t1})
         if (int rc = ensure_events(*v, (size_t)S.slots, true)) return rc;
+    if (S.fgroups > 1)
+        if (int rc = ensure_events(S.ev_fgroup, (size_t)S.slots * (size_t)S.fgroups, false)) return rc;
+    S.fg_n.assign((size_t)S.slots, 1);
+    S.fg_day = -1;
+    S.fg_done = -1;
     S.prod.resize((size_t)S.slots);
     for (StreamProd &p : S.prod) {
         if (int rc = p.ev_done.ensure(false)) return rc;
@@ -737,8 +784,41 @@
         p.host[k] = k < P_PEAK ? from_day[k] : S.tab[k].next;
         S.tab[k].next = nullptr;
     }
+    if (S.slot_da > 0) {
+        const size_t n = S.slot_da, o = (size_t)slot * S.slot_da;
+        HIP_TRY(hipMemcpyAsync((uint8_t *)S.da_mode.p + o, day.da_mode, n, hipMemcpyHostToDevice, hst));
+        HIP_TRY(hipMemcpyAsync((T *)S.da_a.p + o, day.da_a, n * sizeof(T), hipMemcpyHostToDevice, hst));
+        HIP_TRY(hipMemcpyAsync((T *)S.da_w.p + o, day.da_w, n * sizeof(T), hipMemcpyHostToDevice, hst));
+        HIP_TRY(hipMemsetAsync((T *)S.tab[P_NUDGE].base + o, 0, n * sizeof(T), hst));
+        T *const q0o = (T *)S.da_q0.p + (size_t)slot * (size_t)S.ngage;
+        if (day.da_q0) HIP_TRY(hipMemcpyAsync(q0o, day.da_q0, (size_t)S.ngage * sizeof(T), hipMemcpyHostToDevice, hst));
+        else HIP_TRY(hipMemsetAsync(q0o, 0xff, (size_t)S.ngage * sizeof(T), hst));
+    }
+    if (S.rda) {
+        float *const img = (float *)((char *)S.rda_stage.p + (size_t)slot * S.slot_rda);
+        stream_rda_image(pl, S, *day.reservoir_da, img);
+        HIP_TRY(hipMemcpyAsync((char *)S.rda_tab.p + (size_t)slot * S.slot_rda, img, S.slot_rda, hipMemcpyHostToDevice, hst));
+    }
+    if (int rc = S.mk_bnd.order(hst)) return rc;
+    S.mk_bnd.settle();
+    if (tp.nboundary > 0 && boundary_q_dev) {
+        T *q = (T *)S.tm.p + (size_t)slot * S.slot_tm;
+        if (d > 0) {
+            const T *qp = (const T *)S.tm.p + (size_t)((d - 1) % S.slots) * S.slot_tm + (size_t)S.nsteps * np;
+            HIP_TRY(hipMemcpyAsync(q, qp, (size_t)tp.nboundary * sizeof(T), hipMemcpyDeviceToDevice, hst));
+        }
+        hipLaunchKernelGGL((k_stream_boundary<T>), dim3(blocks_for(tp.nboundary * (int64_t)S.nsteps)), dim3(kBlock), 0, hst,
+                           (const T *)boundary_q_dev, q, (int32_t)tp.nboundary, S.nsteps, pl->nseg_pad);
+    }
     const size_t bytes = raw_a ? stream_raw_bytes(S, raw_b != nullptr) : (size_t)pl->nseg * S.nq * sizeof(T);
     if (int rc = pl->in_qlat.ensure(bytes)) return rc;
+    int32_t ng = 1;
+    if (S.fgroups > 1 && !raw_a && pl->nseg > 0) {
+        hipPointerAttribute_t pa{};
+        if (hipPointerGetAttributes(&pa, qlat) == hipSuccess) ng = pa.type == hipMemoryTypeHost ? S.fgroups : 1;
+        else (void)hipGetLastError();
+    }
+    S.fg_n[(size_t)slot] = ng;
     if (pl->nseg > 0 && raw_a) {
         const size_t one = stream_raw_bytes(S, false);
         int32_t *const da = (int32_t *)pl->in_qlat.p, *const db = raw_b ? da + (size_t)S.nq * (size_t)S.pk_nfeat : nullptr;
@@ -751,42 +831,31 @@
                            (T *)S.qlat.p + (size_t)slot * S.slot_qlat, n, pl->nseg_pad, (int32_t)S.nq, S.pk_nfeat);
         HIP_TRY(hipEventRecord(S.ev_pk1, hst));
         S.pk_ms_ok = true;
+    } else if (pl->nseg > 0 && ng > 1) {
+        const int32_t n = (int32_t)pl->nseg;
+        for (int32_t i = 0; i < ng; ++i) {
+            int32_t c0, cnt;
+            forcing_group_cols(S.nq, ng, i, c0, cnt);
+            T *const stage = (T *)pl->in_qlat.p + (size_t)pl->nseg * (size_t)c0;
+            HIP_TRY(hipMemcpy2DAsync(stage, (size_t)cnt * sizeof(T), (const T *)qlat + c0, (size_t)S.nq * sizeof(T), (size_t)cnt * sizeof(T),
+                                     (size_t)pl->nseg, hipMemcpyHostToDevice, hst));
+            prep_qlat_launch<T>(hst, stage, (const int32_t *)pl->sh->row_of_pos.p, (T *)S.qlat.p + (size_t)slot * S.slot_qlat, n, pl->nseg_pad, cnt, c0, cnt);
+            HIP_TRY(hipGetLastError());
+            HIP_TRY(hipEventRecord(S.ev_fgroup[(size_t)slot * (size_t)S.fgroups + (size_t)i], hst));
+        }
     } else if (pl->nseg > 0) {
         HIP_TRY(hipMemcpyAsync(pl->in_qlat.p, qlat, bytes, hipMemcpyHostToDevice, hst));
-        const int32_t n = (int32_t)pl->nseg;
-        hipLaunchKernelGGL((k_prep_qlat<T>), dim3((n + 63) / 64, (unsigned)((S.nq + 31) / 32)), dim3(kBlock), 0, hst, (const T *)pl->in_qlat.p,
-                           (const int32_t *)pl->sh->row_of_pos.p, (T *)S.qlat.p + (size_t)slot * S.slot_qlat, n, pl->nseg_pad, (int32_t)S.nq);
-    }
-    if (S.slot_da > 0) {
-        const size_t n = S.slot_da, o = (size_t)slot * S.slot_da;
-        HIP_TRY(hipMemcpyAsync((uint8_t *)S.da_mode.p + o, day.da_mode, n, hipMemcpyHostToDevice, hst));
-        HIP_TRY(hipMemcpyAsync((T *)S.da_a.p + o, day.da_a, n * sizeof(T), hipMemcpyHostToDevice, hst));
-        HIP_TRY(hipMemcpyAsync((T *)S.da_w.p + o, day.da_w, n * sizeof(T), hipMemcpyHostToDevice, hst));
-        HIP_TRY(hipMemsetAsync((T *)S.tab[P_NUDGE].base + o, 0, n * sizeof(T), hst));
-        T *const q0o = (T *)S.da_q0.p + (size_t)slot * (size_t)S.ngage;
-        if (day.da_q0) HIP_TRY(hipMemcpyAsync(q0o, day.da_q0, (size_t)S.ngage * sizeof(T), hipMemcpyHostToDevice, hst));
-        else HIP_TRY(hipMemsetAsync(q0o, 0xff, (size_t)S.ngage * sizeof(T), hst));
-    }
-    if (S.rda) {
-        float *const img = (float *)((char *)S.rda_stage.p + (size_t)slot * S.slot_rda);
-        stream_rda_image(pl, S, *day.reservoir_da, img);
-        HIP_TRY(hipMemcpyAsync((char *)S.rda_tab.p + (size_t)slot * S.slot_rda, img, S.slot_rda, hipMemcpyHostToDevice, hst));
-    }
-    if (int rc = S.mk_bnd.order(hst)) return rc;
-    S.mk_bnd.settle();
-    if (tp.nboundary > 0 && boundary_q_dev) {
-        T *q = (T *)S.tm.p + (size_t)slot * S.slot_tm;
-        if (d > 0) {
-            const T *qp = (const T *)S.tm.p + (size_t)((d - 1) % S.slots) * S.slot_tm + (size_t)S.nsteps * np;
-            HIP_TRY(hipMemcpyAsync(q, qp, (size_t)tp.nboundary * sizeof(T), hipMemcpyDeviceToDevice, hst));
-        }
-        hipLaunchKernelGGL((k_stream_boundary<T>), dim3(blocks_for(tp.nboundary * (int64_t)S.nsteps)), dim3(kBlock), 0, hst,
-                           (const T *)boundary_q_dev, q, (int32_t)tp.nboundary, S.nsteps, pl->nseg_pad);
+        prep_qlat_launch<T>(hst, (const T *)pl->in_qlat.p, (const int32_t *)pl->sh->row_of_pos.p, (T *)S.qlat.p + (size_t)slot * S.slot_qlat,
+                            (int32_t)pl->nseg, pl->nseg_pad, (int32_t)S.nq, 0, (int32_t)S.nq);
     }
     HIP_TRY(hipGetLastError());
     HIP_TRY(hipEventRecord(S.ev_forcing[(size_t)slot], hst));
-    HIP_TRY(hipStreamWaitEvent(pl->wstream, S.ev_forcing[(size_t)slot], 0));
-    HIP_TRY(hipStreamWaitEvent(pl->stream, S.ev_forcing[(size_t)slot], 0));
+    if (ng > 1) {
+        if (int rc = stream_forcing_wait(pl, S, d, 0, d + 1)) return rc;
+    } else {
+        HIP_TRY(hipStreamWaitEvent(pl->wstream, S.ev_forcing[(size_t)slot], 0));
+        HIP_TRY(hipStreamWaitEvent(pl->stream, S.ev_forcing[(size_t)slot], 0));
+    }
     if (S.cou && S.cou_days > 0) HIP_TRY(hipStreamWaitEvent(pl->wstream, S.ev_cou, 0));
     if (S.dex_K > 0 && S.dex_days > 0) HIP_TRY(hipStreamWaitEvent(pl->wstream, S.ev_dex, 0));
     S.days_pushed = d + 1;
@@ -1423,6 +1492,8 @@
     return 0;
 }
 
+int trmc_stream_forcing_group(int nsteps, int64_t nq, int tile_steps, int groups, int tile) { return stream_forcing_group(nsteps, nq, tile_steps, groups, tile); }
+
 int trmc_stream_info(const trmc_plan *pl, int32_t *slots, int32_t *tiles_per_day, int32_t *lag_max, int32_t *wide_levels,
                      int32_t *cluster_levels, int64_t *days_pushed, int64_t *days_complete, int64_t *launches)
 {
diff --git a/t-route_amd/csrc/trmc.hip b/t-route_amd/csrc/trmc.hip
--- a/t-route_amd/csrc/trmc.hip
+++ b/t-route_amd/csrc/trmc.hip
@@ -206,6 +206,7 @@
         int32_t stream_split = 0;
         int32_t hot_wave_rows = 0;
         int32_t velocity_on_demand = 0;
+        int32_t forcing_groups = 0;
         bool sequence = false;
         bool flow_overlap = false;
         int32_t flow_lean = 0;
```
